# bigai-nlco/VideoTGB

Measured on AMD Instinct MI355X. Metric: clips/sec end-to-end VideoQA (96->8 frames), higher is better.
Workload: dtype bf16; 1 GPU; InstructBLIP-Vicuna-7B + TGB, T=96->8 of 32 frames, 224x224, greedy 16 new tokens (BASELINE.json configs[2]); inputs=resident in HBM when the timed region starts, global_batch=124, parallelism=clip-parallel x1 (no data-path collective), streams=1, weights=seeded N(0,0.02) random init

## Files before the change

include/vtgb.h:

```cpp
#ifndef VTGB_H
#define VTGB_H

#include <stddef.h>
#include <stdint.h>

#ifdef __cplusplus
extern "C" {
#endif

typedef struct ihipStream_t* vtgb_stream_t;

#define VTGB_VERSION 601

#define VTGB_OK 0
#define VTGB_EINVAL (-1)
#define VTGB_EWORKSPACE (-2)
#define VTGB_EHIP (-3)
#define VTGB_EUNSUPPORTED (-4)

#define VTGB_F32 0
#define VTGB_BF16 1
#define VTGB_BF16X3 2
#define VTGB_F16C8 3

// ... 40 lines not shown
} vtgb_preprocess_args;
int vtgb_preprocess_frames(const vtgb_preprocess_args* a, vtgb_stream_t stream);

typedef struct {
    const int64_t* input_ids;
    const int64_t* input_atts;
    const int64_t* output_ids;
    const int64_t* output_atts;
    int64_t* llm_ids;
    int64_t* llm_atts;
    int64_t* input_len;
    int64_t* labels;
    int64_t pad_id;
    int32_t B, Li, Lo, prefix_len;
} vtgb_concat_text_io_args;
int vtgb_concat_text_io(const vtgb_concat_text_io_args* a, vtgb_stream_t stream);

typedef struct {
    int32_t dtype, B, S, V;
    const void* logits;
    const int64_t* labels;
    float* lse;
    float* row_loss;
    float* loss;
    const float* grad_out;
    void* dlogits;
} vtgb_shifted_ce_args;
int vtgb_shifted_ce_forward(const vtgb_shifted_ce_args* a, vtgb_stream_t stream);
int vtgb_shifted_ce_backward(const vtgb_shifted_ce_args* a, vtgb_stream_t stream);

#define VTGB_VIT_NW_GLOBAL 6
#define VTGB_VIT_NW_LAYER 18
typedef struct {
    int32_t dtype, n_frames, image, patch, hidden, heads, mlp, layers;
    float eps;
    const float* pixel_values;
    const void* const* weights;
    float* out_f32;
    void* out_act;
    void* workspace;
    size_t workspace_bytes;
} vtgb_vit_args;
int32_t vtgb_vit_patch_kpad(int32_t dtype, int32_t patch);
size_t vtgb_vit_workspace_bytes(const vtgb_vit_args* a);
int vtgb_vit_forward(const vtgb_vit_args* a, vtgb_stream_t stream);

#define VTGB_QF_NW_GLOBAL 4
#define VTGB_QF_NW_LAYER 32
typedef struct {
    int32_t dtype, n_frames, n_query, n_text, hidden, heads, ffn, layers, cross_freq;
    int32_t enc_tokens, enc_hidden, has_text;
    float eps;
    const void* image_embeds;
    const float* query_tokens;
    const int64_t* text_ids;
    const int64_t* text_mask;
    const int64_t* image_mask;
    const void* const* weights;
    float* out_f32;
    void* workspace;
    size_t workspace_bytes;
} vtgb_qformer_args;
size_t vtgb_qformer_workspace_bytes(const vtgb_qformer_args* a);
int vtgb_qformer_forward(const vtgb_qformer_args* a, vtgb_stream_t stream);

#define VTGB_POOL_MEAN 0
#define VTGB_POOL_CONCAT 1
typedef struct {
    int32_t dtype, n_clips, n_query, hidden, out_dim, mode;
    const float* query_out;
    const int32_t* widths;
    const void* proj_w;
    const float* proj_b;
    float* out;
    void* workspace;
    size_t workspace_bytes;
} vtgb_pool_project_args;
size_t vtgb_pool_project_workspace_bytes(const vtgb_pool_project_args* a);
int vtgb_pool_project(const vtgb_pool_project_args* a, vtgb_stream_t stream);

#define VTGB_TGB_NW_GLOBAL 17
#define VTGB_TGB_NW_LAYER 26
#define VTGB_TGB_MODE_TEXT 0
#define VTGB_TGB_MODE_FUSION 1
#define VTGB_TGB_MODE_MULTIMODAL 2
typedef struct {
    int32_t dtype, B, L, n_text, hidden, heads, ffn, layers, fusion_layer, mode, image, patch;
    float eps;
    const float* of;
    const int64_t* of_mask;
    const int64_t* text_ids;
    const int64_t* text_mask;
    const void* const* weights;
    float* seq_out;
    float* logits;
    void* workspace;
    size_t workspace_bytes;
} vtgb_tgb_args;
size_t vtgb_tgb_workspace_bytes(const vtgb_tgb_args* a);
int vtgb_tgb_forward(const vtgb_tgb_args* a, vtgb_stream_t stream);

typedef struct {
    int32_t dtype, B, L, n_text, hidden, heads, ffn, layers, fusion_layer, mode, image, patch;
    float eps;
    const float* of;
    const int64_t* of_mask;
    const int64_t* text_ids;
    const int64_t* text_mask;
    const void* const* weights;
    float* trunk;
    void* trunk_act;
    float* seq_out;
    float* logits;
    void* workspace;
    size_t workspace_bytes;
} vtgb_tgb_split_args;
size_t vtgb_tgb_trunk_workspace_bytes(const vtgb_tgb_split_args* a);
int vtgb_tgb_trunk(const vtgb_tgb_split_args* a, vtgb_stream_t stream);
size_t vtgb_tgb_resume_workspace_bytes(const vtgb_tgb_split_args* a);
int vtgb_tgb_resume(const vtgb_tgb_split_args* a, vtgb_stream_t stream);

#define VTGB_EPI_STORE 0
#define VTGB_EPI_GELU 1
#define VTGB_EPI_RESID_F32 2
#define VTGB_EPI_STORE_F32 3
typedef struct {
    int32_t dtype, M, N, K, epilogue;
    const void* A;
    int64_t lda;
    const void* W;
    int64_t ldw;
    const float* bias;
    const float* resid;
    void* out;
    int64_t ldo;
} vtgb_gemm_args;
int vtgb_gemm(const vtgb_gemm_args* a, vtgb_stream_t stream);

typedef struct {
    int32_t dtype, batch, heads, head_dim, s_q, s_kv;
    const void* q;
    const void* k;
    const void* v;
    int64_t q_tok_stride, kv_tok_stride;
    int64_t q_batch_stride, kv_batch_stride;
    const float* key_mask;
    const float* rope_q;
    const float* rope_k;
    float scale;
    void* out;
    int64_t out_tok_stride, out_batch_stride;
    int32_t causal;
} vtgb_attention_args;
int vtgb_attention(const vtgb_attention_args* a, vtgb_stream_t stream);

typedef struct {
    int32_t batch, heads, kv_heads, head_dim, s_q, s_kv;
    const void* q;
    const void* k;
    const void* v;
    int64_t q_tok_stride, kv_tok_stride;
    int64_t q_batch_stride, kv_batch_stride;
    const float* key_mask;
    float scale;
    int32_t causal;
    void* out;
    int64_t out_tok_stride, out_batch_stride;
} vtgb_attention_tiled_args;
int vtgb_attention_tiled(const vtgb_attention_tiled_args* a, vtgb_stream_t stream);

typedef struct {
    int32_t batch, heads, kv_heads, head_dim, s_q;
    int32_t q0;
    int32_t tmax;
    float scale;
    const void* q;
    const void* kc;
    const void* vc;
    const float* ks;
    const float* vs;
    const uint8_t* key_valid;
    int64_t q_tok_stride, q_batch_stride;
    void* out;
    int64_t out_tok_stride, out_batch_stride;
} vtgb_attention_cached_args;
int vtgb_attention_cached(const vtgb_attention_cached_args* a, vtgb_stream_t stream);

typedef struct {
    int32_t dtype, M, D;
    float eps;
    const float* x;
    const float* gamma;
    const float* beta;
    float* out_f32;
    void* out_act;
} vtgb_layernorm_args;
int vtgb_layernorm(const vtgb_layernorm_args* a, vtgb_stream_t stream);

#define VTGB_RAFT_NW 30
typedef struct {
    int32_t dtype, n_pairs, H8, W8, iters;
    const float* net;
    const float* inp;
    const void* corr[4];
    const void* const* weights;
    float* flow_up;
    void* workspace;
    size_t workspace_bytes;
    int32_t corr_f16;
    const float* cnet_nhwc;
    const float* flow_init;
} vtgb_raft_update_args;
size_t vtgb_raft_update_workspace_bytes(const vtgb_raft_update_args* a);
int vtgb_raft_update(const vtgb_raft_update_args* a, vtgb_stream_t stream);

int vtgb_pair_pack(int32_t fmt, const float* x, void* out, int64_t M, int32_t C, int32_t ld_pair, vtgb_stream_t stream);
typedef struct {
    int32_t M, N, H, W, KH, KW, C1;
    const void* a;
    const void* a2;
    const void* weights;
    const int32_t* scale;
    const float* bias;
    int32_t act;
    int32_t out_fmt;
    void* out;
    int32_t ld_out;
} vtgb_pair_conv_args;
int vtgb_pair_conv(const vtgb_pair_conv_args* a, vtgb_stream_t stream);
typedef struct {
    vtgb_pair_conv_args conv;
    const void* resid;
    int32_t ld_resid;
    const float* tail_w;
    float* tail_out;
    float* out_f32;
    int32_t ld_f32;
} vtgb_pair_conv_ex_args;
int vtgb_pair_conv_ex(const vtgb_pair_conv_ex_args* a, vtgb_stream_t stream);

typedef struct {
    int32_t n_pairs, H8, W8;
    int32_t variant;
    const float* corr[4];
    const float* flow;
    const void* weights;
    const int32_t* scale;
    const float* bias;
    void* out;
    int32_t* occupancy;
} vtgb_raft_lookup_convc1_args;
int vtgb_raft_lookup_convc1(const vtgb_raft_lookup_convc1_args* a, vtgb_stream_t stream);

typedef struct {
    int32_t fmt;
    int32_t n_images, H8, W8;
    int32_t half;
    int32_t stage;
    const void* h;
    void* h_q;
    const void* x;
    void* rh;
    float* z;
    const float* start_zr;
    const float* start_q;
    const void* w_zr;
    const void* w_q;
    const int32_t* scale_zr;
    const int32_t* scale_q;
} vtgb_raft_gru_half_args;
int vtgb_raft_gru_half(const vtgb_raft_gru_half_args* a, vtgb_stream_t stream);

#define VTGB_CONV_OUT_F32 0
#define VTGB_CONV_OUT_PAIR_BF16 1
#define VTGB_CONV_OUT_PAIR_F16C8 2
#define VTGB_CONV_OUT_BF16 3
typedef struct {
    int32_t dtype;
    int32_t out_kind;
    int32_t site;
    int32_t n_images, H, W;
    int32_t KH, KW, stride;
    int32_t Hi, Wi;
    int32_t C1, C2;
    int32_t N;
    int32_t act;
    int32_t post_relu;
    float out_scale;
    const void* a;
    const void* a2;
    const void* weights;
    const float* bias;
    void* out;
    int64_t ld_out;
    float* moments;
    float* stats_part;
    int64_t stats_part_floats;
    const void* resid;
    int64_t ld_resid;
    const void* tail_w;
    float* tail_out;
} vtgb_conv_launch_args;
int vtgb_conv_launch(const vtgb_conv_launch_args* a, vtgb_stream_t stream);

typedef struct {
    int32_t dtype, n_pairs, H8, W8, dim;
    int32_t pairs_per_clip, frames_per_clip, first_off, second_off, n_images;
    float scale;
    const float* fmap;
    void* levels[4];
    void* workspace;
    size_t workspace_bytes;
} vtgb_raft_corr_args;
size_t vtgb_raft_corr_workspace_bytes(const vtgb_raft_corr_args* a);
int vtgb_raft_corr(const vtgb_raft_corr_args* a, vtgb_stream_t stream);

#define VTGB_RAFT_ENC_NW 40
typedef struct {
    int32_t dtype, n_images, H, W, norm;
    const float* images;
    const void* const* weights;
    float* out;
    void* workspace;
    size_t workspace_bytes;
} vtgb_raft_encoder_args;
size_t vtgb_raft_encoder_workspace_bytes(const vtgb_raft_encoder_args* a);
int vtgb_raft_encoder(const vtgb_raft_encoder_args* a, vtgb_stream_t stream);

int vtgb_llm_rmsnorm(int dtype, void* x, const void* delta, const void* w, void* h, int64_t rows, int32_t H, float eps,
                     vtgb_stream_t stream);
int vtgb_llm_rope_cache(int dtype, const void* qkv, void* q_out, void* kc, void* vc, const void* cos_t, const void* sin_t,
                        const int64_t* pos, int32_t B, int32_t nq, int32_t nkv, int32_t hd, int32_t tmax, vtgb_stream_t stream);
int vtgb_llm_rope_cache_prefill(int dtype, void* qkv, void* kc, void* vc, const void* cos_t, const void* sin_t, int32_t B, int32_t S, int32_t nq,
                                int32_t nkv, int32_t hd, int32_t tmax, vtgb_stream_t stream);
int vtgb_llm_decode_attention(int dtype, const void* q, const void* kc, const void* vc, void* out, const int64_t* pos, int32_t B,
                              int32_t nq, int32_t nkv, int32_t hd, int32_t tmax, float scale, vtgb_stream_t stream);
int vtgb_llm_silu_mul(int dtype, const void* gu, void* act, int64_t rows, int32_t I, vtgb_stream_t stream);

typedef struct {
    int32_t dtype, rows, heads, head_dim, rows_per_batch, n_keys, t_pad;
    float scale;
    const void* q;   int64_t q_row;
    const void* k;   const void* v;   int64_t kv_batch, kv_head, kv_tok;
    const void* bias; int64_t bias_pos, bias_head;
    const int64_t* pos;
    void* out;       int64_t o_row;
} vtgb_llm_attn_rows_args;
int vtgb_llm_attention_rows(const vtgb_llm_attn_rows_args* a, vtgb_stream_t stream);
int vtgb_llm_gated_act(int dtype, const void* gu, void* act, int64_t rows, int32_t I, int32_t kind, int32_t gated, vtgb_stream_t stream);

typedef struct {
    int32_t M, N, K, n_splits;
    const void* x; int64_t ldx;
    const void* w; int64_t ldw;
    void* out; int64_t ldo;
    int32_t out_dtype;
    int32_t w_tiled;
    void* workspace;
    size_t workspace_bytes;
    int32_t defer_reduce;
} vtgb_gemm_skinny_args;
int32_t vtgb_gemm_skinny_splits(const vtgb_gemm_skinny_args* a);
int vtgb_llm_rmsnorm_parts(int dtype, void* x, const float* part, int32_t n_splits, const void* w, void* h, int64_t rows, int32_t H, float eps,
                           vtgb_stream_t stream);
int vtgb_llm_rope_cache_parts(int dtype, const float* part, int32_t n_splits, void* q_out, void* kc, void* vc, const void* cos_t, const void* sin_t,
                              const int64_t* pos, int32_t B, int32_t nq, int32_t nkv, int32_t hd, int32_t tmax, vtgb_stream_t stream);

int vtgb_llm_rope_cache_pos(int dtype, const void* qkv, void* q_out, void* kc, void* vc, const void* cos_t, const void* sin_t,
                            const int64_t* pos, const int64_t* rope_off, int32_t B, int32_t nq, int32_t nkv, int32_t hd, int32_t tmax,
                            vtgb_stream_t stream);
int vtgb_llm_rope_cache_parts_pos(int dtype, const float* part, int32_t n_splits, void* q_out, void* kc, void* vc, const void* cos_t,
                                  const void* sin_t, const int64_t* pos, const int64_t* rope_off, int32_t B, int32_t nq, int32_t nkv, int32_t hd,
                                  int32_t tmax, vtgb_stream_t stream);
int vtgb_llm_rope_cache_prefill_pos(int dtype, void* qkv, void* kc, void* vc, const void* cos_t, const void* sin_t, const int64_t* pos_ids,
                                    int32_t B, int32_t S, int32_t nq, int32_t nkv, int32_t hd, int32_t tmax, vtgb_stream_t stream);
int vtgb_llm_decode_attention_masked(int dtype, const void* q, const void* kc, const void* vc, void* out, const int64_t* pos,
                                     const uint8_t* key_valid, int32_t B, int32_t nq, int32_t nkv, int32_t hd, int32_t tmax, float scale,
                                     vtgb_stream_t stream);
int vtgb_llm_attention_rows_masked(const vtgb_llm_attn_rows_args* a, const uint8_t* key_valid, int64_t key_valid_batch_stride,
                                   vtgb_stream_t stream);

int64_t vtgb_llm_decode_attention_split_workspace_bytes(int32_t B, int32_t nq, int32_t hd, int32_t tmax);
int vtgb_llm_decode_attention_split(int dtype, const void* q, const void* kc, const void* vc, void* out, const int64_t* pos,
                                    const uint8_t* key_valid , void* workspace, int32_t B, int32_t nq, int32_t nkv, int32_t hd,
                                    int32_t tmax, float scale, vtgb_stream_t stream);

typedef struct {
    int32_t dtype;
    int32_t B, nq, nkv, hd, tmax;
    int32_t n_splits;
    const void* qkv;
    const float* part;
    void* q_out;
    uint8_t* kc8; uint8_t* vc8;
    float* ks; float* vs;
    const void* cos_t; const void* sin_t;
    const int64_t* pos;
    const int64_t* rope_off;
} vtgb_llm_rope_cache_fp8_args;
int vtgb_llm_rope_cache_fp8(const vtgb_llm_rope_cache_fp8_args* a, vtgb_stream_t stream);
int vtgb_llm_rope_cache_prefill_fp8(int dtype, void* qkv, uint8_t* kc8, uint8_t* vc8, float* ks, float* vs, const void* cos_t, const void* sin_t,
                                    const int64_t* pos_ids , int32_t B, int32_t S, int32_t nq, int32_t nkv, int32_t hd, int32_t tmax,
                                    vtgb_stream_t stream);
int vtgb_llm_decode_attention_split_fp8(int dtype, const void* q, const uint8_t* kc8, const uint8_t* vc8, const float* ks, const float* vs, void* out,
                                        const int64_t* pos, const uint8_t* key_valid , void* workspace, int32_t B, int32_t nq,
                                        int32_t nkv, int32_t hd, int32_t tmax, float scale, vtgb_stream_t stream);

typedef struct {
    int32_t dtype;
    int32_t R, K, nq, nkv, hd, tmax_p, tmax_g;
    float scale;
    const void* q;
    const void* kp; const void* vp;
    const void* kg; const void* vg;
    const int32_t* src_row;
    void* out;
    const int64_t* n_prompt;
    const int64_t* pos;
    const uint8_t* key_valid;
    void* workspace;
} vtgb_llm_decode_attention_beam_args;
int vtgb_llm_decode_attention_beam(const vtgb_llm_decode_attention_beam_args* a, vtgb_stream_t stream);
typedef struct {
    int32_t dtype;
    int32_t R, K, nq, nkv, hd, tmax_p, tmax_g;
    float scale;
    const void* q;
    const uint8_t* kp8; const uint8_t* vp8;
    const float* kps; const float* vps;
    const uint8_t* kg8; const uint8_t* vg8;
    const float* kgs; const float* vgs;
    const int32_t* src_row;
    void* out;
    const int64_t* n_prompt;
    const int64_t* pos;
    const uint8_t* key_valid;
    void* workspace;
} vtgb_llm_decode_attention_beam_fp8_args;
int vtgb_llm_decode_attention_beam_fp8(const vtgb_llm_decode_attention_beam_fp8_args* a, vtgb_stream_t stream);
typedef struct {
    int32_t dtype;
    int32_t R, K, V, N;
    int32_t eos;
    int32_t min_new;
    float penalty;
    const void* logits;
    const int64_t* seq;
    const int64_t* step;
    const float* running;
    float* cand_score;
    int32_t* cand_idx;
    void* workspace;
    size_t workspace_bytes;
} vtgb_llm_beam_candidates_args;
int vtgb_llm_beam_candidates(const vtgb_llm_beam_candidates_args* a, vtgb_stream_t stream);

#define VTGB_LLM_ATTN_ROWS_BEAM_MAX_T 1920
int vtgb_llm_attention_rows_beam(const vtgb_llm_attn_rows_args* a, const int32_t* src_row, int64_t src_row_stride, int32_t cache_rows,
                                 vtgb_stream_t stream);

#define VTGB_LORA_MAX_SEGMENTS 4
#define VTGB_LORA_MAX_RANK 64
typedef struct {
    const float* A;
    const float* B;
    int32_t r, n, col0;
    float scaling;
} vtgb_llm_lora_seg;
typedef struct {
    int32_t dtype;
    int32_t K, n_cols, n_seg;
    int64_t rows, ldx, ldy;
    const void* x;
    void* y;
    vtgb_llm_lora_seg seg[VTGB_LORA_MAX_SEGMENTS];
} vtgb_llm_lora_args;
int vtgb_llm_lora(const vtgb_llm_lora_args* a, vtgb_stream_t stream);

size_t vtgb_pack_skinny_weight_bytes(int32_t N, int32_t K);
int vtgb_pack_skinny_weight(const void* w, int64_t ldw, int32_t N, int32_t K, void* dst, vtgb_stream_t stream);
size_t vtgb_gemm_skinny_workspace_bytes(const vtgb_gemm_skinny_args* a);
int vtgb_gemm_skinny(const vtgb_gemm_skinny_args* a, vtgb_stream_t stream);

size_t vtgb_pack_skinny_weight_fp8_bytes(int32_t N, int32_t K);
int vtgb_pack_skinny_weight_fp8(const void* w, int64_t ldw, int32_t N, int32_t K, void* dst, float* scale_out, vtgb_stream_t stream);
int vtgb_gemm_skinny_fp8(const vtgb_gemm_skinny_args* a, const float* w_scale, vtgb_stream_t stream);

int vtgb_gemm_skinny_bias(const vtgb_gemm_skinny_args* a, const float* w_scale , const float* bias ,
                          vtgb_stream_t stream);

size_t vtgb_pack_skinny_weight_mxfp4_bytes(int32_t N, int32_t K);
int vtgb_pack_skinny_weight_mxfp4(const void* w, int64_t ldw, int32_t N, int32_t K, void* dst, vtgb_stream_t stream);
int vtgb_gemm_skinny_mxfp4(const vtgb_gemm_skinny_args* a, const float* bias , vtgb_stream_t stream);

typedef struct {
    int32_t batch, heads, head_dim, s_q, s_kv;
    const float* q;
    const float* k;
    const float* v;
    int64_t q_tok, kv_tok, q_batch, kv_batch;
    const float* key_mask;
    const float* drop;
    float scale;
    float* out;
    int64_t o_tok, o_batch;
    float* lse;
    const float* dout;
    float* dq;
    float* dk;
    float* dv;
    float* delta;
} vtgb_attn_train_args;
int vtgb_attn_train_forward(const vtgb_attn_train_args* a, vtgb_stream_t stream);
int vtgb_attn_train_backward(const vtgb_attn_train_args* a, vtgb_stream_t stream);

typedef struct {
    int32_t compute, M, N, K;
    const void* a;
    int64_t lda;
    int32_t a_dtype, a_kmajor;
    const void* b;
    int64_t ldb;
    int32_t b_dtype, b_kmajor;
    const float* bias;
    float* out;
    int64_t ldo;
    void* workspace;
    size_t workspace_bytes;
} vtgb_gemm_train_args;
size_t vtgb_gemm_train_workspace_bytes(const vtgb_gemm_train_args* a);
int vtgb_gemm_train(const vtgb_gemm_train_args* a, vtgb_stream_t stream);
int32_t vtgb_col_sum_parts(int32_t M);
int vtgb_col_sum_f32(const float* x, int64_t ldx, int32_t M, int32_t N, float* out, float* partial, vtgb_stream_t stream);
typedef struct {
    int32_t rows, D;
    float eps;
    const float* x;
    const float* mask;
    const float* resid;
    const float* gamma;
    const float* beta;
    float* sum;
    float* y;
    float* mean;
    float* rstd;
    const float* dy;
    float* ds;
    float* dx;
    float* dgamma;
    float* dbeta;
    float* partial;
} vtgb_layernorm_train_args;
int32_t vtgb_layernorm_train_partials(int32_t rows);
int vtgb_layernorm_train_forward(const vtgb_layernorm_train_args* a, vtgb_stream_t stream);
int vtgb_layernorm_train_backward(const vtgb_layernorm_train_args* a, vtgb_stream_t stream);
int vtgb_gelu_forward(const float* x, float* y, int64_t n, vtgb_stream_t stream);
int vtgb_gelu_backward(const float* x, const float* dy, float* dx, int64_t n, vtgb_stream_t stream);

#define VTGB_COMM_ID_BYTES 128
typedef struct vtgb_comm vtgb_comm;
int vtgb_comm_unique_id(void* id_out );
int vtgb_comm_init(vtgb_comm** comm, const void* unique_id , int32_t rank, int32_t world);
int vtgb_comm_destroy(vtgb_comm* comm);
int vtgb_allreduce_f32(vtgb_comm* comm, float* buf, size_t count, int32_t average, vtgb_stream_t stream);

#define VTGB_PROF_GEMM 0
#define VTGB_PROF_ATTN 1
#define VTGB_PROF_CONV 2
void vtgb_prof_enable(int on);
void vtgb_prof_reset(void);
int vtgb_prof_summary(int kind, int64_t* launches, double* ms, double* flops);
int vtgb_prof_executed_flops(int kind, double* flops);

#ifdef __cplusplus
}
#endif
#endif
```

videotgb_amd/_lib.py:

```python
from __future__ import annotations

import ctypes as C
import os

import torch

HERE = os.path.dirname(os.path.abspath(__file__))
LIB_PATH = os.environ.get("VTGB_LIB") or os.path.join(HERE, "libvtgb.so")

F32, BF16 = 0, 1
BF16X3 = 2
F16C8 = 3
MAP_A, MAP_B = 0, 1
POOL_MEAN, POOL_CONCAT = 0, 1
TGB_MODE = {"text": 0, "vision": 0, "fusion": 1, "multi_modal": 2}
EPI_STORE, EPI_GELU, EPI_RESID_F32, EPI_STORE_F32 = 0, 1, 2, 3
VIT_NW_GLOBAL, VIT_NW_LAYER = 6, 18
QF_NW_GLOBAL, QF_NW_LAYER = 4, 32
TGB_NW_GLOBAL, TGB_NW_LAYER = 17, 26

EXPORTS = [
    "vtgb_version", "vtgb_last_error", "vtgb_pack_bf16", "vtgb_span_select", "vtgb_span_to_frames",
    "vtgb_gather_frames", "vtgb_vit_patch_kpad", "vtgb_vit_workspace_bytes", "vtgb_vit_forward",
    "vtgb_qformer_workspace_bytes", "vtgb_qformer_forward", "vtgb_pool_project_workspace_bytes",
    "vtgb_pool_project", "vtgb_tgb_workspace_bytes", "vtgb_tgb_forward", "vtgb_tgb_trunk_workspace_bytes", "vtgb_tgb_trunk",
    "vtgb_tgb_resume_workspace_bytes", "vtgb_tgb_resume", "vtgb_gemm", "vtgb_attention",
    "vtgb_layernorm", "vtgb_prof_enable", "vtgb_prof_reset", "vtgb_prof_summary", "vtgb_prof_executed_flops",
    "vtgb_llm_rmsnorm", "vtgb_llm_rope_cache", "vtgb_llm_rope_cache_prefill", "vtgb_llm_decode_attention", "vtgb_llm_silu_mul",
    "vtgb_llm_attention_rows", "vtgb_llm_gated_act", "vtgb_llm_rmsnorm_parts", "vtgb_llm_rope_cache_parts", "vtgb_gemm_skinny_splits",
    "vtgb_llm_rope_cache_pos", "vtgb_llm_rope_cache_parts_pos", "vtgb_llm_rope_cache_prefill_pos", "vtgb_llm_decode_attention_masked",
    "vtgb_llm_attention_rows_masked",
    "vtgb_gemm_skinny_workspace_bytes", "vtgb_gemm_skinny", "vtgb_pack_skinny_weight_bytes", "vtgb_pack_skinny_weight",
    "vtgb_pack_skinny_weight_fp8_bytes", "vtgb_pack_skinny_weight_fp8", "vtgb_gemm_skinny_fp8", "vtgb_gemm_skinny_bias",
    "vtgb_raft_update_workspace_bytes", "vtgb_raft_update", "vtgb_raft_encoder_workspace_bytes", "vtgb_raft_encoder",
    "vtgb_raft_corr_workspace_bytes", "vtgb_raft_corr", "vtgb_preprocess_frames", "vtgb_concat_text_io", "vtgb_shifted_ce_forward", "vtgb_shifted_ce_backward",
    "vtgb_comm_unique_id", "vtgb_comm_init", "vtgb_comm_destroy", "vtgb_allreduce_f32",
    "vtgb_attn_train_forward", "vtgb_attn_train_backward",
    "vtgb_gemm_train", "vtgb_gemm_train_workspace_bytes", "vtgb_col_sum_parts", "vtgb_col_sum_f32", "vtgb_layernorm_train_partials", "vtgb_layernorm_train_forward", "vtgb_layernorm_train_backward",
    "vtgb_gelu_forward", "vtgb_gelu_backward",
    "vtgb_pair_pack", "vtgb_pair_conv", "vtgb_pair_conv_ex", "vtgb_attention_tiled",
    "vtgb_llm_decode_attention_split_workspace_bytes", "vtgb_llm_decode_attention_split",
    "vtgb_llm_decode_attention_split_fp8", "vtgb_llm_rope_cache_fp8", "vtgb_llm_rope_cache_prefill_fp8",
    "vtgb_raft_lookup_convc1", "vtgb_raft_gru_half", "vtgb_llm_lora", "vtgb_conv_launch", "vtgb_attention_cached",
    "vtgb_llm_decode_attention_beam", "vtgb_llm_beam_candidates", "vtgb_llm_attention_rows_beam", "vtgb_llm_decode_attention_beam_fp8",
    "vtgb_pack_skinny_weight_mxfp4_bytes", "vtgb_pack_skinny_weight_mxfp4", "vtgb_gemm_skinny_mxfp4",
]
COMM_ID_BYTES = 128

i32, i64, f32, vp, sz = C.c_int32, C.c_int64, C.c_float, C.c_void_p, C.c_size_t


class AttnTrainArgs(C.Structure):
    _fields_ = [("batch", i32), ("heads", i32), ("head_dim", i32), ("s_q", i32), ("s_kv", i32), ("q", vp), ("k", vp), ("v", vp),
                ("q_tok", i64), ("kv_tok", i64), ("q_batch", i64), ("kv_batch", i64), ("key_mask", vp), ("drop", vp), ("scale", f32),
                ("out", vp), ("o_tok", i64), ("o_batch", i64), ("lse", vp), ("dout", vp), ("dq", vp), ("dk", vp), ("dv", vp), ("delta", vp)]


class GemmTrainArgs(C.Structure):
    _fields_ = [("compute", i32), ("M", i32), ("N", i32), ("K", i32), ("a", vp), ("lda", i64), ("a_dtype", i32), ("a_kmajor", i32),
                ("b", vp), ("ldb", i64), ("b_dtype", i32), ("b_kmajor", i32), ("bias", vp), ("out", vp), ("ldo", i64), ("workspace", vp), ("workspace_bytes", sz)]


class LayerNormTrainArgs(C.Structure):
    _fields_ = [("rows", i32), ("D", i32), ("eps", f32), ("x", vp), ("mask", vp), ("resid", vp), ("gamma", vp), ("beta", vp), ("sum", vp),
                ("y", vp), ("mean", vp), ("rstd", vp), ("dy", vp), ("ds", vp), ("dx", vp), ("dgamma", vp), ("dbeta", vp), ("partial", vp)]


class VtgbError(RuntimeError):
    pass


class SpanSelectArgs(C.Structure):
    _fields_ = [("logits", vp), ("noise", vp), ("idx", vp), ("B", i32), ("L", i32), ("draws", i32), ("tau", f32)]


class SpanToFramesArgs(C.Structure):
    _fields_ = [("sel", vp), ("V", vp), ("frame_idx", vp), ("B", i32), ("draws", i32), ("V_all", i32), ("N", i32),
                ("nframe", i32), ("variant", i32)]


class GatherFramesArgs(C.Structure):
    _fields_ = [("pixel_values", vp), ("frame_idx", vp), ("out", vp), ("B", i32), ("N", i32), ("nframe", i32),
                ("frame_elems", i64)]


class PreprocessArgs(C.Structure):
    _fields_ = [("raw", vp), ("frame_idx", vp), ("out", vp), ("T", i32), ("H0", i32), ("W0", i32), ("n_out", i32), ("size", i32),
                ("mean", f32 * 3), ("std", f32 * 3)]


class ConcatTextIoArgs(C.Structure):
    _fields_ = [("input_ids", vp), ("input_atts", vp), ("output_ids", vp), ("output_atts", vp), ("llm_ids", vp), ("llm_atts", vp),
                ("input_len", vp), ("labels", vp), ("pad_id", i64), ("B", i32), ("Li", i32), ("Lo", i32), ("prefix_len", i32)]


class ShiftedCeArgs(C.Structure):
    _fields_ = [("dtype", i32), ("B", i32), ("S", i32), ("V", i32), ("logits", vp), ("labels", vp), ("lse", vp), ("row_loss", vp),
                ("loss", vp), ("grad_out", vp), ("dlogits", vp)]


class VitArgs(C.Structure):
    _fields_ = [("dtype", i32), ("n_frames", i32), ("image", i32), ("patch", i32), ("hidden", i32), ("heads", i32),
                ("mlp", i32), ("layers", i32), ("eps", f32), ("pixel_values", vp), ("weights", C.POINTER(vp)),
                ("out_f32", vp), ("out_act", vp), ("workspace", vp), ("workspace_bytes", sz)]


class QFormerArgs(C.Structure):
    _fields_ = [("dtype", i32), ("n_frames", i32), ("n_query", i32), ("n_text", i32), ("hidden", i32), ("heads", i32),
                ("ffn", i32), ("layers", i32), ("cross_freq", i32), ("enc_tokens", i32), ("enc_hidden", i32),
                ("has_text", i32), ("eps", f32), ("image_embeds", vp), ("query_tokens", vp), ("text_ids", vp),
                ("text_mask", vp), ("image_mask", vp), ("weights", C.POINTER(vp)), ("out_f32", vp), ("workspace", vp),
                ("workspace_bytes", sz)]


class PoolProjectArgs(C.Structure):
    _fields_ = [("dtype", i32), ("n_clips", i32), ("n_query", i32), ("hidden", i32), ("out_dim", i32), ("mode", i32),
                ("query_out", vp), ("widths", C.POINTER(i32)), ("proj_w", vp), ("proj_b", vp), ("out", vp),
                ("workspace", vp), ("workspace_bytes", sz)]


class TgbArgs(C.Structure):
    _fields_ = [("dtype", i32), ("B", i32), ("L", i32), ("n_text", i32), ("hidden", i32), ("heads", i32), ("ffn", i32),
                ("layers", i32), ("fusion_layer", i32), ("mode", i32), ("image", i32), ("patch", i32), ("eps", f32),
                ("of", vp), ("of_mask", vp), ("text_ids", vp), ("text_mask", vp), ("weights", C.POINTER(vp)),
                ("seq_out", vp), ("logits", vp), ("workspace", vp), ("workspace_bytes", sz)]


class TgbSplitArgs(C.Structure):
    _fields_ = [("dtype", i32), ("B", i32), ("L", i32), ("n_text", i32), ("hidden", i32), ("heads", i32), ("ffn", i32),
                ("layers", i32), ("fusion_layer", i32), ("mode", i32), ("image", i32), ("patch", i32), ("eps", f32),
                ("of", vp), ("of_mask", vp), ("text_ids", vp), ("text_mask", vp), ("weights", C.POINTER(vp)),
                ("trunk", vp), ("trunk_act", vp), ("seq_out", vp), ("logits", vp), ("workspace", vp), ("workspace_bytes", sz)]


class RaftUpdateArgs(C.Structure):
    _fields_ = [("dtype", i32), ("n_pairs", i32), ("H8", i32), ("W8", i32), ("iters", i32), ("net", vp), ("inp", vp), ("corr", vp * 4),
                ("weights", C.POINTER(vp)), ("flow_up", vp), ("workspace", vp), ("workspace_bytes", sz), ("corr_f16", i32), ("cnet_nhwc", vp),
                ("flow_init", vp)]


class PairConvArgs(C.Structure):
    _fields_ = [("M", i32), ("N", i32), ("H", i32), ("W", i32), ("KH", i32), ("KW", i32), ("C1", i32), ("a", vp), ("a2", vp), ("weights", vp), ("scale", vp),
                ("bias", vp), ("act", i32), ("out_fmt", i32), ("out", vp), ("ld_out", i32)]


class PairConvExArgs(C.Structure):
    _fields_ = [("conv", PairConvArgs), ("resid", vp), ("ld_resid", i32), ("tail_w", vp), ("tail_out", vp), ("out_f32", vp), ("ld_f32", i32)]


class RaftLookupConvc1Args(C.Structure):
    _fields_ = [("n_pairs", i32), ("H8", i32), ("W8", i32), ("variant", i32), ("corr", vp * 4), ("flow", vp), ("weights", vp), ("scale", vp), ("bias", vp),
                ("out", vp), ("occupancy", C.POINTER(i32))]


class RaftGruHalfArgs(C.Structure):
    _fields_ = [("fmt", i32), ("n_images", i32), ("H8", i32), ("W8", i32), ("half", i32), ("stage", i32), ("h", vp), ("h_q", vp), ("x", vp), ("rh", vp), ("z", vp),
                ("start_zr", vp), ("start_q", vp), ("w_zr", vp), ("w_q", vp), ("scale_zr", vp), ("scale_q", vp)]


CONV_OUT_F32, CONV_OUT_PAIR_BF16, CONV_OUT_PAIR_F16C8, CONV_OUT_BF16 = 0, 1, 2, 3
CONV_SITE_ENCODER, CONV_SITE_UPDATE = 0, 1


class ConvLaunchArgs(C.Structure):
    _fields_ = [("dtype", i32), ("out_kind", i32), ("site", i32), ("n_images", i32), ("H", i32), ("W", i32), ("KH", i32), ("KW", i32), ("stride", i32),
                ("Hi", i32), ("Wi", i32), ("C1", i32), ("C2", i32), ("N", i32), ("act", i32), ("post_relu", i32), ("out_scale", f32), ("a", vp), ("a2", vp),
                ("weights", vp), ("bias", vp), ("out", vp), ("ld_out", i64), ("moments", vp), ("stats_part", vp), ("stats_part_floats", i64), ("resid", vp),
                ("ld_resid", i64), ("tail_w", vp), ("tail_out", vp)]


class RaftCorrArgs(C.Structure):
    _fields_ = [("dtype", i32), ("n_pairs", i32), ("H8", i32), ("W8", i32), ("dim", i32), ("pairs_per_clip", i32), ("frames_per_clip", i32),
                ("first_off", i32), ("second_off", i32), ("n_images", i32), ("scale", f32), ("fmap", vp), ("levels", vp * 4),
                ("workspace", vp), ("workspace_bytes", sz)]


class RaftEncoderArgs(C.Structure):
    _fields_ = [("dtype", i32), ("n_images", i32), ("H", i32), ("W", i32), ("norm", i32), ("images", vp), ("weights", C.POINTER(vp)), ("out", vp),
                ("workspace", vp), ("workspace_bytes", sz)]


class GemmSkinnyArgs(C.Structure):
    _fields_ = [("M", i32), ("N", i32), ("K", i32), ("n_splits", i32), ("x", vp), ("ldx", i64), ("w", vp), ("ldw", i64), ("out", vp), ("ldo", i64),
                ("out_dtype", i32), ("w_tiled", i32), ("workspace", vp), ("workspace_bytes", sz), ("defer_reduce", i32)]


class LlmLoraSeg(C.Structure):
    _fields_ = [("A", vp), ("B", vp), ("r", i32), ("n", i32), ("col0", i32), ("scaling", f32)]


LORA_MAX_SEGMENTS, LORA_MAX_RANK = 4, 64


class LlmLoraArgs(C.Structure):
    _fields_ = [("dtype", i32), ("K", i32), ("n_cols", i32), ("n_seg", i32), ("rows", i64), ("ldx", i64), ("ldy", i64), ("x", vp), ("y", vp),
                ("seg", LlmLoraSeg * LORA_MAX_SEGMENTS)]


class LlmRopeCacheFp8Args(C.Structure):
    _fields_ = [("dtype", i32), ("B", i32), ("nq", i32), ("nkv", i32), ("hd", i32), ("tmax", i32), ("n_splits", i32), ("qkv", vp), ("part", vp),
                ("q_out", vp), ("kc8", vp), ("vc8", vp), ("ks", vp), ("vs", vp), ("cos_t", vp), ("sin_t", vp), ("pos", vp), ("rope_off", vp)]


class LlmDecodeAttentionBeamArgs(C.Structure):
    _fields_ = [("dtype", i32), ("R", i32), ("K", i32), ("nq", i32), ("nkv", i32), ("hd", i32), ("tmax_p", i32), ("tmax_g", i32), ("scale", f32),
                ("q", vp), ("kp", vp), ("vp", vp), ("kg", vp), ("vg", vp), ("src_row", vp), ("out", vp), ("n_prompt", vp), ("pos", vp),
                ("key_valid", vp), ("workspace", vp)]


class LlmDecodeAttentionBeamFp8Args(C.Structure):
    _fields_ = [("dtype", i32), ("R", i32), ("K", i32), ("nq", i32), ("nkv", i32), ("hd", i32), ("tmax_p", i32), ("tmax_g", i32), ("scale", f32),
                ("q", vp), ("kp8", vp), ("vp8", vp), ("kps", vp), ("vps", vp), ("kg8", vp), ("vg8", vp), ("kgs", vp), ("vgs", vp), ("src_row", vp),
                ("out", vp), ("n_prompt", vp), ("pos", vp), ("key_valid", vp), ("workspace", vp)]


class LlmBeamCandidatesArgs(C.Structure):
    _fields_ = [("dtype", i32), ("R", i32), ("K", i32), ("V", i32), ("N", i32), ("eos", i32), ("min_new", i32), ("penalty", f32), ("logits", vp),
                ("seq", vp), ("step", vp), ("running", vp), ("cand_score", vp), ("cand_idx", vp), ("workspace", vp), ("workspace_bytes", sz)]


class GemmArgs(C.Structure):
    _fields_ = [("dtype", i32), ("M", i32), ("N", i32), ("K", i32), ("epilogue", i32), ("A", vp), ("lda", i64),
                ("W", vp), ("ldw", i64), ("bias", vp), ("resid", vp), ("out", vp), ("ldo", i64)]


class AttentionArgs(C.Structure):
    _fields_ = [("dtype", i32), ("batch", i32), ("heads", i32), ("head_dim", i32), ("s_q", i32), ("s_kv", i32),
                ("q", vp), ("k", vp), ("v", vp), ("q_tok_stride", i64), ("kv_tok_stride", i64), ("q_batch_stride", i64),
                ("kv_batch_stride", i64), ("key_mask", vp), ("rope_q", vp), ("rope_k", vp), ("scale", f32), ("out", vp),
                ("out_tok_stride", i64), ("out_batch_stride", i64), ("causal", i32)]


class AttentionTiledArgs(C.Structure):
    _fields_ = [("batch", i32), ("heads", i32), ("kv_heads", i32), ("head_dim", i32), ("s_q", i32), ("s_kv", i32),
                ("q", vp), ("k", vp), ("v", vp), ("q_tok_stride", i64), ("kv_tok_stride", i64), ("q_batch_stride", i64),
                ("kv_batch_stride", i64), ("key_mask", vp), ("scale", f32), ("causal", i32), ("out", vp),
                ("out_tok_stride", i64), ("out_batch_stride", i64)]


class AttentionCachedArgs(C.Structure):
    _fields_ = [("batch", i32), ("heads", i32), ("kv_heads", i32), ("head_dim", i32), ("s_q", i32), ("q0", i32), ("tmax", i32), ("scale", f32),
                ("q", vp), ("kc", vp), ("vc", vp), ("ks", vp), ("vs", vp), ("key_valid", vp), ("q_tok_stride", i64), ("q_batch_stride", i64),
                ("out", vp), ("out_tok_stride", i64), ("out_batch_stride", i64)]


class LlmAttnRowsArgs(C.Structure):
    _fields_ = [("dtype", i32), ("rows", i32), ("heads", i32), ("head_dim", i32), ("rows_per_batch", i32), ("n_keys", i32), ("t_pad", i32),
                ("scale", f32), ("q", vp), ("q_row", i64), ("k", vp), ("v", vp), ("kv_batch", i64), ("kv_head", i64), ("kv_tok", i64),
                ("bias", vp), ("bias_pos", i64), ("bias_head", i64), ("pos", vp), ("out", vp), ("o_row", i64)]


class LayerNormArgs(C.Structure):
    _fields_ = [("dtype", i32), ("M", i32), ("D", i32), ("eps", f32), ("x", vp), ("gamma", vp), ("beta", vp),
                ("out_f32", vp), ("out_act", vp)]


_lib = None


def lib() -> C.CDLL:
    global _lib
    if _lib is not None:
        return _lib
    if not os.path.exists(LIB_PATH):
        raise VtgbError(f"{LIB_PATH} is missing: build it with `python -m videotgb_amd.build` "
                        "(there is no CPU fallback for the hot path)")
    L = C.CDLL(LIB_PATH)
    L.vtgb_version.restype = C.c_int
    L.vtgb_last_error.restype = C.c_char_p
    L.vtgb_pack_bf16.argtypes = [vp, vp, i64, i64, i64, vp]
    L.vtgb_vit_patch_kpad.argtypes = [i32, i32]
    L.vtgb_vit_patch_kpad.restype = i32
    for name, st in (("span_select", SpanSelectArgs), ("span_to_frames", SpanToFramesArgs),
                     ("gather_frames", GatherFramesArgs), ("vit_forward", VitArgs), ("qformer_forward", QFormerArgs),
                     ("pool_project", PoolProjectArgs), ("tgb_forward", TgbArgs), ("gemm", GemmArgs),
                     ("attention", AttentionArgs), ("attention_tiled", AttentionTiledArgs), ("attention_cached", AttentionCachedArgs),
                     ("layernorm", LayerNormArgs)):
        fn = getattr(L, "vtgb_" + name)
        fn.argtypes = [C.POINTER(st), vp]
        fn.restype = C.c_int
    for name, st in (("vit", VitArgs), ("qformer", QFormerArgs), ("pool_project", PoolProjectArgs), ("tgb", TgbArgs),
                     ("tgb_trunk", TgbSplitArgs), ("tgb_resume", TgbSplitArgs)):
        fn = getattr(L, f"vtgb_{name}_workspace_bytes")
        fn.argtypes = [C.POINTER(st)]
        fn.restype = sz
    for name in ("tgb_trunk", "tgb_resume"):
        fn = getattr(L, "vtgb_" + name)
        fn.argtypes = [C.POINTER(TgbSplitArgs), vp]
        fn.restype = C.c_int
    L.vtgb_pair_pack.argtypes = [i32, vp, vp, i64, i32, i32, vp]
    L.vtgb_pair_pack.restype = C.c_int
    L.vtgb_pair_conv.argtypes = [C.POINTER(PairConvArgs), vp]
    L.vtgb_pair_conv.restype = C.c_int
    L.vtgb_pair_conv_ex.argtypes = [C.POINTER(PairConvExArgs), vp]
    L.vtgb_pair_conv_ex.restype = C.c_int
    L.vtgb_raft_lookup_convc1.argtypes = [C.POINTER(RaftLookupConvc1Args), vp]
    L.vtgb_raft_lookup_convc1.restype = C.c_int
    L.vtgb_raft_gru_half.argtypes = [C.POINTER(RaftGruHalfArgs), vp]
    L.vtgb_raft_gru_half.restype = C.c_int
    L.vtgb_conv_launch.argtypes = [C.POINTER(ConvLaunchArgs), vp]
    L.vtgb_conv_launch.restype = C.c_int
    L.vtgb_raft_update.argtypes = [C.POINTER(RaftUpdateArgs), vp]
    L.vtgb_raft_update.restype = C.c_int
    L.vtgb_raft_update_workspace_bytes.argtypes = [C.POINTER(RaftUpdateArgs)]
    L.vtgb_raft_update_workspace_bytes.restype = sz
    L.vtgb_raft_encoder.argtypes = [C.POINTER(RaftEncoderArgs), vp]
    L.vtgb_raft_encoder.restype = C.c_int
    L.vtgb_raft_encoder_workspace_bytes.argtypes = [C.POINTER(RaftEncoderArgs)]
    L.vtgb_raft_encoder_workspace_bytes.restype = sz
    L.vtgb_raft_corr.argtypes = [C.POINTER(RaftCorrArgs), vp]
    L.vtgb_raft_corr.restype = C.c_int
    L.vtgb_raft_corr_workspace_bytes.argtypes = [C.POINTER(RaftCorrArgs)]
    L.vtgb_raft_corr_workspace_bytes.restype = sz
    L.vtgb_llm_rmsnorm.argtypes = [C.c_int, vp, vp, vp, vp, i64, i32, f32, vp]
    L.vtgb_llm_rope_cache.argtypes = [C.c_int, vp, vp, vp, vp, vp, vp, vp, i32, i32, i32, i32, i32, vp]
    L.vtgb_llm_rope_cache_prefill.argtypes = [C.c_int, vp, vp, vp, vp, vp, i32, i32, i32, i32, i32, i32, vp]
    L.vtgb_llm_decode_attention.argtypes = [C.c_int, vp, vp, vp, vp, vp, i32, i32, i32, i32, i32, f32, vp]
    L.vtgb_llm_silu_mul.argtypes = [C.c_int, vp, vp, i64, i32, vp]
    L.vtgb_llm_attention_rows.argtypes = [C.POINTER(LlmAttnRowsArgs), vp]
    L.vtgb_llm_attention_rows.restype = C.c_int
    L.vtgb_llm_gated_act.argtypes = [C.c_int, vp, vp, i64, i32, i32, i32, vp]
    L.vtgb_llm_gated_act.restype = C.c_int
    L.vtgb_llm_rmsnorm_parts.argtypes = [C.c_int, vp, vp, i32, vp, vp, i64, i32, f32, vp]
    L.vtgb_llm_rmsnorm_parts.restype = C.c_int
    L.vtgb_llm_rope_cache_parts.argtypes = [C.c_int, vp, i32, vp, vp, vp, vp, vp, vp, i32, i32, i32, i32, i32, vp]
    L.vtgb_llm_rope_cache_parts.restype = C.c_int
    L.vtgb_llm_rope_cache_pos.argtypes = [C.c_int, vp, vp, vp, vp, vp, vp, vp, vp, i32, i32, i32, i32, i32, vp]
    L.vtgb_llm_rope_cache_parts_pos.argtypes = [C.c_int, vp, i32, vp, vp, vp, vp, vp, vp, vp, i32, i32, i32, i32, i32, vp]
    L.vtgb_llm_rope_cache_prefill_pos.argtypes = [C.c_int, vp, vp, vp, vp, vp, vp, i32, i32, i32, i32, i32, i32, vp]
    L.vtgb_llm_decode_attention_masked.argtypes = [C.c_int, vp, vp, vp, vp, vp, vp, i32, i32, i32, i32, i32, f32, vp]
    L.vtgb_llm_attention_rows_masked.argtypes = [C.POINTER(LlmAttnRowsArgs), vp, i64, vp]
    for fn in (L.vtgb_llm_rope_cache_pos, L.vtgb_llm_rope_cache_parts_pos, L.vtgb_llm_rope_cache_prefill_pos, L.vtgb_llm_decode_attention_masked,
               L.vtgb_llm_attention_rows_masked):
        fn.restype = C.c_int
    L.vtgb_llm_decode_attention_split_workspace_bytes.argtypes = [i32, i32, i32, i32]
    L.vtgb_llm_decode_attention_split_workspace_bytes.restype = i64
    L.vtgb_llm_decode_attention_split.argtypes = [C.c_int, vp, vp, vp, vp, vp, vp, vp, i32, i32, i32, i32, i32, f32, vp]
    L.vtgb_llm_decode_attention_split.restype = C.c_int
    L.vtgb_llm_decode_attention_split_fp8.argtypes = [C.c_int, vp, vp, vp, vp, vp, vp, vp, vp, vp, i32, i32, i32, i32, i32, f32, vp]
    L.vtgb_llm_decode_attention_split_fp8.restype = C.c_int
    L.vtgb_llm_rope_cache_fp8.argtypes = [C.POINTER(LlmRopeCacheFp8Args), vp]
    L.vtgb_llm_rope_cache_fp8.restype = C.c_int
    L.vtgb_llm_decode_attention_beam.argtypes = [C.POINTER(LlmDecodeAttentionBeamArgs), vp]
    L.vtgb_llm_decode_attention_beam.restype = C.c_int
    L.vtgb_llm_decode_attention_beam_fp8.argtypes = [C.POINTER(LlmDecodeAttentionBeamFp8Args), vp]
    L.vtgb_llm_decode_attention_beam_fp8.restype = C.c_int
    L.vtgb_llm_beam_candidates.argtypes = [C.POINTER(LlmBeamCandidatesArgs), vp]
    L.vtgb_llm_beam_candidates.restype = C.c_int
    L.vtgb_llm_attention_rows_beam.argtypes = [C.POINTER(LlmAttnRowsArgs), vp, i64, i32, vp]
    L.vtgb_llm_attention_rows_beam.restype = C.c_int
    L.vtgb_llm_lora.argtypes = [C.POINTER(LlmLoraArgs), vp]
    L.vtgb_llm_lora.restype = C.c_int
    L.vtgb_llm_rope_cache_prefill_fp8.argtypes = [C.c_int, vp, vp, vp, vp, vp, vp, vp, vp, i32, i32, i32, i32, i32, i32, vp]
    L.vtgb_llm_rope_cache_prefill_fp8.restype = C.c_int
    L.vtgb_gemm_skinny_splits.argtypes = [C.POINTER(GemmSkinnyArgs)]
    L.vtgb_gemm_skinny_splits.restype = i32
    L.vtgb_gemm_skinny.argtypes = [C.POINTER(GemmSkinnyArgs), vp]
    L.vtgb_gemm_skinny.restype = C.c_int
    L.vtgb_gemm_skinny_workspace_bytes.argtypes = [C.POINTER(GemmSkinnyArgs)]
    L.vtgb_gemm_skinny_workspace_bytes.restype = sz
    L.vtgb_pack_skinny_weight_bytes.argtypes = [i32, i32]
    L.vtgb_pack_skinny_weight_bytes.restype = sz
    L.vtgb_pack_skinny_weight.argtypes = [vp, i64, i32, i32, vp, vp]
    L.vtgb_pack_skinny_weight.restype = C.c_int
    L.vtgb_pack_skinny_weight_fp8_bytes.argtypes = [i32, i32]
    L.vtgb_pack_skinny_weight_fp8_bytes.restype = sz
    L.vtgb_pack_skinny_weight_fp8.argtypes = [vp, i64, i32, i32, vp, vp, vp]
    L.vtgb_pack_skinny_weight_fp8.restype = C.c_int
    L.vtgb_gemm_skinny_fp8.argtypes = [C.POINTER(GemmSkinnyArgs), vp, vp]
    L.vtgb_gemm_skinny_fp8.restype = C.c_int
    L.vtgb_gemm_skinny_bias.argtypes = [C.POINTER(GemmSkinnyArgs), vp, vp, vp]
    L.vtgb_gemm_skinny_bias.restype = C.c_int
    L.vtgb_pack_skinny_weight_mxfp4_bytes.argtypes = [i32, i32]
    L.vtgb_pack_skinny_weight_mxfp4_bytes.restype = sz
    L.vtgb_pack_skinny_weight_mxfp4.argtypes = [vp, i64, i32, i32, vp, vp]
    L.vtgb_pack_skinny_weight_mxfp4.restype = C.c_int
    L.vtgb_gemm_skinny_mxfp4.argtypes = [C.POINTER(GemmSkinnyArgs), vp, vp]
    L.vtgb_gemm_skinny_mxfp4.restype = C.c_int
    for fn in (L.vtgb_attn_train_forward, L.vtgb_attn_train_backward):
        fn.argtypes = [C.POINTER(AttnTrainArgs), vp]
        fn.restype = C.c_int
    L.vtgb_gemm_train.argtypes = [C.POINTER(GemmTrainArgs), vp]
    L.vtgb_gemm_train_workspace_bytes.argtypes = [C.POINTER(GemmTrainArgs)]
    L.vtgb_gemm_train_workspace_bytes.restype = sz
    L.vtgb_col_sum_f32.argtypes = [vp, i64, i32, i32, vp, vp, vp]
    L.vtgb_col_sum_parts.argtypes = [i32]
    L.vtgb_col_sum_parts.restype = i32
    L.vtgb_layernorm_train_partials.argtypes = [i32]
    L.vtgb_layernorm_train_partials.restype = i32
    for fn in (L.vtgb_layernorm_train_forward, L.vtgb_layernorm_train_backward):
        fn.argtypes = [C.POINTER(LayerNormTrainArgs), vp]
    L.vtgb_gelu_forward.argtypes = [vp, vp, i64, vp]
    L.vtgb_gelu_backward.argtypes = [vp, vp, vp, i64, vp]
    for fn in (L.vtgb_gemm_train, L.vtgb_col_sum_f32, L.vtgb_layernorm_train_forward, L.vtgb_layernorm_train_backward, L.vtgb_gelu_forward,
               L.vtgb_gelu_backward):
        fn.restype = C.c_int
    L.vtgb_comm_unique_id.argtypes = [vp]
    L.vtgb_comm_init.argtypes = [C.POINTER(vp), vp, i32, i32]
    L.vtgb_comm_destroy.argtypes = [vp]
    L.vtgb_allreduce_f32.argtypes = [vp, vp, sz, i32, vp]
    for fn in (L.vtgb_comm_unique_id, L.vtgb_comm_init, L.vtgb_comm_destroy, L.vtgb_allreduce_f32):
        fn.restype = C.c_int
    L.vtgb_prof_enable.argtypes = [C.c_int]
    L.vtgb_prof_enable.restype = None
    L.vtgb_prof_reset.restype = None
    L.vtgb_prof_summary.argtypes = [C.c_int, C.POINTER(i64), C.POINTER(C.c_double), C.POINTER(C.c_double)]
    L.vtgb_prof_summary.restype = C.c_int
    L.vtgb_prof_executed_flops.argtypes = [C.c_int, C.POINTER(C.c_double)]
    L.vtgb_prof_executed_flops.restype = C.c_int
    _lib = L
    return L


def prof_summary(kind: int):
    n, ms, fl = i64(0), C.c_double(0), C.c_double(0)
    check(lib().vtgb_prof_summary(kind, C.byref(n), C.byref(ms), C.byref(fl)))
    return n.value, ms.value, fl.value


def prof_executed_flops(kind: int) -> float:
    f = C.c_double(0)
    check(lib().vtgb_prof_executed_flops(kind, C.byref(f)))
    return f.value


_ERR = {-1: ValueError, -2: VtgbError, -3: VtgbError, -4: NotImplementedError}


def check(rc: int) -> None:
    if rc != 0:
        msg = lib().vtgb_last_error().decode("utf-8", "replace")
        raise _ERR.get(rc, VtgbError)(f"libvtgb: {msg} (code {rc})")
```

videotgb_amd/csrc/common.h:

```cpp
#pragma once
#include <hip/hip_runtime.h>
#include <stdint.h>
#include <stdio.h>

#include "vtgb.h"

typedef __bf16 bf16_t;
typedef __attribute__((ext_vector_type(8))) __bf16 bf16x8;
typedef __attribute__((ext_vector_type(4))) __bf16 bf16x4;
typedef __attribute__((ext_vector_type(4))) float f32x4;

#if defined(__HIPCC__)
__device__ __forceinline__ float bf16_round(float v) {
    unsigned u = __float_as_uint(v);
    if ((u & 0x7F800000u) != 0x7F800000u) u += 0x7FFFu + ((u >> 16) & 1u);
    return __uint_as_float(u & 0xFFFF0000u);
}
#endif

void vtgb_set_error(const char* fmt, ...);

#define VTGB_REQUIRE(cond, code, ...)  \
    do {                               \
        if (!(cond)) {                 \
            vtgb_set_error(__VA_ARGS__); \
            return (code);             \
        }                              \
    } while (0)

#define VTGB_HIP(expr)                                                              \
    do {                                                                            \
        hipError_t _e = (expr);                                                     \
        if (_e != hipSuccess) {                                                     \
            vtgb_set_error("%s failed: %s (%s:%d)", #expr, hipGetErrorString(_e), __FILE__, __LINE__); \
            return VTGB_EHIP;                                                       \
        }                                                                           \
    } while (0)

#define VTGB_TRY(expr)        \
    do {                      \
        int _r = (expr);      \
        if (_r != VTGB_OK) return _r; \
    } while (0)

struct RowMap {
    int32_t seg_rows;
    int64_t seg_stride;
    int64_t seg_off;
};
static inline RowMap rowmap_identity() { return RowMap{0, 0, 0}; }
static inline RowMap rowmap(int seg_rows, int64_t seg_stride, int64_t seg_off) {
    return RowMap{seg_rows, seg_stride, seg_off};
}
__host__ __device__ static inline int64_t map_row(const RowMap& m, int64_t r) {
    if (m.seg_rows == 0) return r;
    const int32_t r32 = (int32_t)r, seg = r32 / m.seg_rows;
    return (int64_t)seg * m.seg_stride + m.seg_off + (r32 - seg * m.seg_rows);
}

static inline size_t align_up(size_t x, size_t a) { return (x + a - 1) / a * a; }

#include <atomic>
struct DeviceOnce {
    std::atomic<uint64_t> done{0};
    static uint64_t bit() {
        int dev = 0;
        (void)hipGetDevice(&dev);
        return 1ull << (dev & 63);
    }
    bool need() const { return !(done.load(std::memory_order_acquire) & bit()); }
    void mark() { done.fetch_or(bit(), std::memory_order_acq_rel); }
};
#define VTGB_FUNC_LDS_ONCE(flag, kernel, bytes)                                                                              \
    do {                                                                                                                     \
        if ((flag).need()) {                                                                                                 \
            VTGB_HIP(hipFuncSetAttribute(reinterpret_cast<const void*>(kernel), hipFuncAttributeMaxDynamicSharedMemorySize, (int)(bytes))); \
            (flag).mark();                                                                                                   \
        }                                                                                                                    \
    } while (0)
static inline size_t dtype_size(int dtype) { return dtype == VTGB_BF16 ? 2 : 4; }

struct Workspace {
    char* base;
    size_t size, used;
    bool dry;
    Workspace(void* p, size_t n) : base((char*)p), size(n), used(0), dry(p == nullptr) {}
    void* take(size_t bytes) {
        size_t off = align_up(used, 256);
        used = off + bytes;
        return dry ? nullptr : (void*)(base + off);
    }
    bool ok() const { return dry || used <= size; }
};

struct GemmDesc {
    int dtype, M, N, K, epi;
    const void* A;
    int64_t lda;
    RowMap a_map;
    const void* W;
    int64_t ldw;
    const float* bias;
    const float* resid;
    int64_t ldr;
    RowMap r_map;
    void* out;
    int64_t ldo;
    RowMap o_map;
    int act;
    float out_scale;
    int conv_H, conv_W, conv_KH, conv_KW, conv_Cin, conv_split;
    int conv_stride, conv_Hi, conv_Wi;
    const void* A2;
    int64_t lda2;
    const void* zero_page;
    const void* aux;
    int64_t ldaux;
    void* out2;
    int64_t ldo2;
    float* col_stats;
    int stats_rows;
    int gate_from;
    const void* resid_bf16;
    int64_t ldrb;
    int post_relu;
    const void* init_bf16;
    int64_t ldinit;
    int frag_out, init_frag;
    uint32_t div_hw_mul, div_hw_sh, div_w_mul, div_w_sh;
    double algo_flops;
    const void* tail_w;
    float* tail_out;
    int64_t ldtail;
    int conv_wrap, conv_wrap2;
    int split_lo;
    void* ln_xb;
    int64_t ldxb;
    float* ln_part;
    const float* ln_stats;
    const float* ln_cs;
    const float* ln_c;
    int h8_run;
    const int* h8_scale;
    int h8_out_bf16;
    int split_f16c8;
};
int launch_conv_h8(const GemmDesc& d, hipStream_t s);
int launch_ln_fold_stats(const float* part, int nblk, int D, float eps, float* stats, int64_t M, hipStream_t s);
int launch_ln_fold_prepare(const float* x, int64_t ldx, int D, void* xb, float* part, int64_t M, hipStream_t s);
#define VTGB_EPI_GRU 4
#define VTGB_EPI_SPLIT 5
#define VTGB_EPI_X3ZR 6
#define VTGB_EPI_X3Q 7
int launch_gemm(const GemmDesc& d, hipStream_t s);
int launch_conv_gemm(const GemmDesc& d, hipStream_t s);

struct AttnDesc {
    int dtype, batch, heads, head_dim, s_q, s_kv;
    const void *q, *k, *v;
    int64_t q_tok, kv_tok, q_batch, kv_batch;
    const float* key_mask;
    const float* rope_q;
    const float* rope_k;
    float scale;
    void* out;
    int64_t o_tok, o_batch;
    int causal = 0;
};
int launch_attention(const AttnDesc& d, hipStream_t s);

bool stem7x7_supported(int H, int W);
int launch_stem7x7(const float* img, const void* w, const float* bias, float* out_f32, float* stats, float* stats_part, void* out_bf16, int n_img, int H, int W,
                   int relu, hipStream_t s);
size_t conv64_stats_part_floats(int n_img);
int launch_stats_finish_tiles(const float* part, float* stats, int n_img, int HW, int N, int64_t M, hipStream_t s);
int launch_stats_finish_parts(const float* part, float* stats, int n_img, int parts, int C, hipStream_t s);
int cu_count();

bool conv3x3_c64_supported(int H, int W);
int launch_conv3x3_c64(const void* in, const void* w, const float* bias, float* out_f32, float* stats, float* stats_part, void* out_bf16, const void* resid,
                       int n_img, int H, int W, int relu, int post_relu, hipStream_t s);

struct LnDesc {
    int dtype, M, D;
    float eps;
    const float* x;
    int64_t ldx;
    RowMap x_map;
    const float* gamma;
    const float* beta;
    float* out_f32;
    void* out_act;
    int64_t ldo;
    RowMap o_map;
};
int launch_layernorm(const LnDesc& d, hipStream_t s);

int launch_im2col(int dtype, const float* pix, void* out, int n_img, int ch, int image, int patch, int kpad, hipStream_t s);
int launch_vit_cls_rows(const float* cls, const float* pos, float* x, int n_frames, int tokens, int hidden, hipStream_t s);
int launch_cast_act(int dtype, const float* src, void* dst, int64_t n, hipStream_t s);
int launch_mask_to_additive(const int64_t* mask, float* out, int64_t n, float neg, hipStream_t s);
int launch_fill_f32(float* dst, float v, int64_t n, hipStream_t s);
int launch_qformer_embed(const float* query, const int64_t* ids, const float* wemb, const float* pemb, float* x,
                         int n_frames, int n_query, int n_text, int hidden, hipStream_t s);
int launch_tgb_text_embed(const int64_t* ids, const float* wemb, const float* temb, float* x, int64_t rows, int hidden,
                          hipStream_t s);
int launch_flow_reduce(const float* of, const float* fcw, float* red, int n_img, int image, int patch, hipStream_t s);
int launch_flow_assemble(const float* conv, const float* proj_b, const float* fcw, const float* fcb, const float* bos,
                         const float* eos, const float* pos, const int64_t* of_mask, float* x, int B, int L,
                         int hidden, int n_patches, hipStream_t s);
int launch_mean_pool_uniform(const float* q, float* out, int n_clips, int width, int64_t row_elems, hipStream_t s);
int launch_pack_bf16(const float* src, void* dst, int64_t rows, int64_t cols, int64_t cols_pad, hipStream_t s);
int launch_mrc_head(const float* x, const float* w, const float* b, float* logits, int B, int L, int hidden, hipStream_t s);

struct CorrPyr { const void* lvl[4]; int h[4], w[4]; };

struct ProfScope {
    int slot;
    hipStream_t s;
    ProfScope(int kind, double flops, hipStream_t stream, double executed_flops = -1.0);
    ~ProfScope();
};
```

videotgb_amd/csrc/conv64.hip:

```cpp
#include "common.h"

namespace {

constexpr int C64_R = 8, C64_RS = 128;
constexpr int C64_ROW_BYTES = C64_RS * 128;
constexpr int C64_LDS = C64_R * C64_ROW_BYTES + 8 * 32 * 2 * 4 + 64 * 4;
typedef __attribute__((address_space(3))) void* c64_lptr_t;

struct Conv64Params {
    const bf16_t* in;
    const bf16_t* w;
    const float* bias;
    float* out_f32;
    float* stats;
    float* stats_part;
    bf16_t* out_bf16;
    const bf16_t* resid;
    int n_img, H, W, relu, post_relu;
    int parts, rows_per_part;
};

template <int MODE>
__global__ __launch_bounds__(512) void conv3x3_c64_kernel(const Conv64Params p) {
#if defined(__HIP_DEVICE_COMPILE__)
    extern __shared__ __attribute__((aligned(16))) char ring[];
    float* const xch = reinterpret_cast<float*>(ring + C64_R * C64_ROW_BYTES);
    const int tid = threadIdx.x, lane = tid & 63, fr = lane & 15, fg = lane >> 4;
    const int wave = __builtin_amdgcn_readfirstlane(tid >> 6);
    const int wm = wave & 3, wn = wave >> 2;
    const int H = p.H, W = p.W;

    bf16x8 wf[9][2][2];
#pragma unroll
    for (int t = 0; t < 9; t++)
#pragma unroll
        for (int ks = 0; ks < 2; ks++)
#pragma unroll
            for (int i = 0; i < 2; i++)
                wf[t][ks][i] = *reinterpret_cast<const bf16x8*>(p.w + (wn * 32 + i * 16 + fr) * 576 + t * 64 + ks * 32 + fg * 8);
    float* const bias_s = xch + 8 * 32 * 2;
    if (tid < 64) bias_s[tid] = p.bias[tid];

    unsigned dma_off[2];
#pragma unroll
    for (int q = 0; q < 2; q++) {
        const int slot = (wave * 2 + q) * 8 + (lane >> 3), x = slot - 1, c = (lane & 7) ^ ((slot >> 1) & 7);
        dma_off[q] = (x >= 0 && x < W) ? (unsigned)(x * 64 + c * 8) * 2u : 0x80000000u;
    }
    unsigned x_off[3];
    int px[2];
#pragma unroll
    for (int j = 0; j < 2; j++) px[j] = wm * 32 + j * 16 + fr;
#pragma unroll
    for (int kx = 0; kx < 3; kx++) x_off[kx] = (unsigned)((px[0] + kx) * 128 + ((fg ^ (((px[0] + kx) >> 1) & 7)) << 4));

    typedef __attribute__((__vector_size__(4 * sizeof(unsigned)))) unsigned u32x4_t;
    typedef __attribute__((__vector_size__(2 * sizeof(unsigned)))) unsigned u32x2_t;
    constexpr unsigned OOB = 0x80000000u;
    constexpr int ES = MODE == 0 ? 4 : 2;
    unsigned o_off[2][2];
#pragma unroll
    for (int i = 0; i < 2; i++)
#pragma unroll
        for (int j = 0; j < 2; j++) o_off[i][j] = px[j] < W ? (unsigned)(px[j] * 64 + wn * 32 + i * 16 + fg * 4) * ES : OOB;

    const int n_units = p.n_img * p.parts;
    for (int unit = blockIdx.x; unit < n_units; unit += gridDim.x) {
        const int img = unit / p.parts, y0 = (unit - img * p.parts) * p.rows_per_part;
        if (y0 >= H) continue;
        const int y1 = y0 + p.rows_per_part < H ? y0 + p.rows_per_part : H;
        const bf16_t* const ibase = p.in + (int64_t)img * H * W * 64;
        const auto rsrc = __builtin_amdgcn_make_buffer_rsrc(const_cast<bf16_t*>(ibase), 0, H * W * 128, 0x00020000);
        const auto orsrc = __builtin_amdgcn_make_buffer_rsrc(MODE == 0 ? (void*)(p.out_f32 + (int64_t)img * H * W * 64) : (void*)(p.out_bf16 + (int64_t)img * H * W * 64), 0,
                                                             H * W * 64 * ES, 0x00020000);
        const auto rrsrc = __builtin_amdgcn_make_buffer_rsrc(const_cast<bf16_t*>(p.resid ? p.resid + (int64_t)img * H * W * 64 : ibase), 0, H * W * 128, 0x00020000);
#define C64_ISSUE(yy)                                                                                                          \
        {                                                                                                                      \
            const int so_ = ((yy) >= 0 && (yy) < H) ? (yy) * W * 128 : 0x7FFFFF00;        \
            char* const dst_ = ring + ((yy) & (C64_R - 1)) * C64_ROW_BYTES + (wave * 2) * 1024;                                \
            __builtin_amdgcn_raw_ptr_buffer_load_lds(rsrc, (c64_lptr_t)dst_, 16, dma_off[0], so_, 0, 0);                       \
            __builtin_amdgcn_raw_ptr_buffer_load_lds(rsrc, (c64_lptr_t)(dst_ + 1024), 16, dma_off[1], so_, 0, 0);              \
        }
        __builtin_amdgcn_s_waitcnt(0x0F70);
        __builtin_amdgcn_s_barrier();
        C64_ISSUE(y0 - 1)
        C64_ISSUE(y0)
        C64_ISSUE(y0 + 1)
        C64_ISSUE(y0 + 2)
        f32x4 s1[2] = {f32x4{0.f, 0.f, 0.f, 0.f}, f32x4{0.f, 0.f, 0.f, 0.f}}, s2[2] = {s1[0], s1[0]};
        for (int y = y0; y < y1; y += 2) {
            if (y == y0) __builtin_amdgcn_s_waitcnt(0x0F70);
            else __builtin_amdgcn_s_waitcnt(0x0F78);
            __builtin_amdgcn_s_barrier();
            bf16x4 rres[2][2][2];
            if constexpr (MODE == 1) {
                if (p.resid) {
#pragma unroll
                    for (int o = 0; o < 2; o++)
#pragma unroll
                        for (int i = 0; i < 2; i++)
#pragma unroll
                            for (int j = 0; j < 2; j++) {
                                const unsigned off = (y + o < y1 && o_off[i][j] != OOB) ? o_off[i][j] + (unsigned)((y + o) * W * 64 * 2) : OOB;
                                rres[o][i][j] = __builtin_bit_cast(bf16x4, __builtin_amdgcn_raw_buffer_load_b64(rrsrc, off, 0, 0));
                            }
                }
            }
            C64_ISSUE(y + 3)
            C64_ISSUE(y + 4)
            f32x4 acc[2][2][2];
#pragma unroll
            for (int o = 0; o < 2; o++)
#pragma unroll
                for (int i = 0; i < 2; i++)
#pragma unroll
                    for (int j = 0; j < 2; j++) acc[o][i][j] = f32x4{0.f, 0.f, 0.f, 0.f};
#pragma unroll
            for (int rr = 0; rr < 4; rr++) {
                const char* const rowp = ring + ((y + rr - 1) & (C64_R - 1)) * C64_ROW_BYTES;
#pragma unroll
                for (int kx = 0; kx < 3; kx++)
#pragma unroll
                    for (int ks = 0; ks < 2; ks++) {
                        const bf16x8 x0 = *reinterpret_cast<const bf16x8*>(rowp + (x_off[kx] ^ (ks * 64)));
                        const bf16x8 x1 = *reinterpret_cast<const bf16x8*>(rowp + (x_off[kx] ^ (ks * 64)) + 2048);
#pragma unroll
                        for (int o = 0; o < 2; o++) {
                            const int ky = rr - o;
                            if (ky < 0 || ky > 2) continue;
#pragma unroll
                            for (int i = 0; i < 2; i++) {
                                acc[o][i][0] = __builtin_amdgcn_mfma_f32_16x16x32_bf16(wf[ky * 3 + kx][ks][i], x0, acc[o][i][0], 0, 0, 0);
                                acc[o][i][1] = __builtin_amdgcn_mfma_f32_16x16x32_bf16(wf[ky * 3 + kx][ks][i], x1, acc[o][i][1], 0, 0, 0);
                            }
                        }
                    }
            }
            f32x4 b4[2];
#pragma unroll
            for (int i = 0; i < 2; i++) b4[i] = *reinterpret_cast<const f32x4*>(bias_s + wn * 32 + i * 16 + fg * 4);
#pragma unroll
            for (int o = 0; o < 2; o++) {
                const bool row_ok = y + o < y1;
#pragma unroll
                for (int i = 0; i < 2; i++)
#pragma unroll
                    for (int j = 0; j < 2; j++) {
                        const bool ok = row_ok && o_off[i][j] != OOB;
                        const unsigned off = ok ? o_off[i][j] + (unsigned)((y + o) * W * 64 * ES) : OOB;
                        f32x4 v = acc[o][i][j] + b4[i];
                        if constexpr (MODE == 0) {
                            __builtin_amdgcn_raw_buffer_store_b128(__builtin_bit_cast(u32x4_t, v), orsrc, off, 0, 0);
                            const f32x4 vz = {ok ? v[0] : 0.f, ok ? v[1] : 0.f, ok ? v[2] : 0.f, ok ? v[3] : 0.f};
                            s1[i] += vz;
                            s2[i] += vz * vz;
                        } else {
                            if (p.relu) v = f32x4{fmaxf(v[0], 0.f), fmaxf(v[1], 0.f), fmaxf(v[2], 0.f), fmaxf(v[3], 0.f)};
                            if (p.resid) {
                                const bf16x4 r = rres[o][i][j];
                                v += f32x4{(float)r[0], (float)r[1], (float)r[2], (float)r[3]};
                            }
                            if (p.post_relu) v = f32x4{fmaxf(v[0], 0.f), fmaxf(v[1], 0.f), fmaxf(v[2], 0.f), fmaxf(v[3], 0.f)};
                            const bf16x4 pk = {(bf16_t)v[0], (bf16_t)v[1], (bf16_t)v[2], (bf16_t)v[3]};
                            __builtin_amdgcn_raw_buffer_store_b64(__builtin_bit_cast(u32x2_t, pk), orsrc, off, 0, 0);
                        }
                    }
            }
        }
#undef C64_ISSUE
        if constexpr (MODE == 0) {
#pragma unroll
            for (int i = 0; i < 2; i++)
#pragma unroll
                for (int e = 0; e < 4; e++) {
                    float a_ = s1[i][e], b_ = s2[i][e];
#pragma unroll
                    for (int off = 1; off < 16; off <<= 1) { a_ += __shfl_xor(a_, off); b_ += __shfl_xor(b_, off); }
                    s1[i][e] = a_; s2[i][e] = b_;
                }
            __builtin_amdgcn_s_waitcnt(0xC07F);
            __builtin_amdgcn_s_barrier();
            if (fr == 0) {
#pragma unroll
                for (int i = 0; i < 2; i++)
#pragma unroll
                    for (int e = 0; e < 4; e++) {
                        xch[(wave * 32 + i * 16 + fg * 4 + e) * 2] = s1[i][e];
                        xch[(wave * 32 + i * 16 + fg * 4 + e) * 2 + 1] = s2[i][e];
                    }
            }
            __syncthreads();
            if (tid < 128) {
                const int ch = tid >> 1, which = tid & 1, wn_ = ch >> 5, c32 = ch & 31;
                float t = 0.f;
#pragma unroll
                for (int m_ = 0; m_ < 4; m_++) t += xch[((wn_ * 4 + m_) * 32 + c32) * 2 + which];
                if (p.parts == 1) p.stats[((int64_t)img * 64 + ch) * 2 + which] = t;
                else p.stats_part[((int64_t)unit * 64 + ch) * 2 + which] = t;
            }
        }
    }
#endif
}


constexpr int ST_R = 5;
struct StemParams {
    const float* img;
    const bf16_t* w;
    const float* bias;
    float* out_f32;
    float* stats;
    float* stats_part;
    bf16_t* out_bf16;
    int n_img, H, W, relu;
    int parts, rows_per_part;
};

template <int MODE>
__global__ __launch_bounds__(512) void stem7x7_kernel(const StemParams p) {
#if defined(__HIP_DEVICE_COMPILE__)
    extern __shared__ __attribute__((aligned(16))) char ring[];
    const int tid = threadIdx.x, lane = tid & 63, fr = lane & 15, fg = lane >> 4;
    const int wave = __builtin_amdgcn_readfirstlane(tid >> 6);
    const int wm = wave & 3, wn = wave >> 2;
    const int H = p.H, W = p.W, H2 = H >> 1, W2 = W >> 1;
    const int row_bytes = W2 * 256;
    float* const xch = reinterpret_cast<float*>(ring + ST_R * row_bytes);
    float* const bias_s = xch + 8 * 32 * 2;
    if (tid < 64) bias_s[tid] = p.bias[tid];
    for (int i = tid; i < ST_R * W2 * 4; i += 512) {
        const int pxl = i >> 2, X = pxl % W2, c = 6 + (i & 1) + ((i & 2) << 2);
        *reinterpret_cast<uint4*>(ring + pxl * 256 + ((c ^ (X & 15)) << 4)) = make_uint4(0, 0, 0, 0);
    }
    bf16x8 wf[16][2];
#pragma unroll
    for (int s_ = 0; s_ < 16; s_++)
#pragma unroll
        for (int i = 0; i < 2; i++) wf[s_][i] = *reinterpret_cast<const bf16x8*>(p.w + (wn * 32 + i * 16 + fr) * 512 + s_ * 32 + fg * 8);
    const bool builder = tid < W2 * 4;
    const int bX = tid >> 2, bdX = tid & 3, bcol = 2 * (bX + bdX - 2);
    const bool bcol_ok = builder && bcol >= 0 && bcol + 1 < W;
    const int bcol_c = bcol < 0 ? 0 : bcol + 1 < W ? bcol : W - 2;
    unsigned b_off[3];
#pragma unroll
    for (int q = 0; q < 3; q++) {
        const int off = bdX * 24 + q * 8;
        b_off[q] = (unsigned)(bX * 256 + (((off >> 4) ^ (bX & 15)) << 4) + (off & 8));
    }
    int px[2];
    unsigned x_off[2];
#pragma unroll
    for (int j = 0; j < 2; j++) {
        px[j] = wm * 32 + j * 16 + fr;
        const int pc = px[j] < W2 ? px[j] : 0;
        x_off[j] = (unsigned)(pc * 256 + ((fg ^ (pc & 15)) << 4));
    }
    typedef __attribute__((__vector_size__(4 * sizeof(unsigned)))) unsigned u32x4_t;
    typedef __attribute__((__vector_size__(2 * sizeof(unsigned)))) unsigned u32x2_t;
    constexpr unsigned OOB = 0x80000000u;
    constexpr int ES = MODE == 0 ? 4 : 2;
    unsigned o_off[2][2];
#pragma unroll
    for (int i = 0; i < 2; i++)
#pragma unroll
        for (int j = 0; j < 2; j++) o_off[i][j] = px[j] < W2 ? (unsigned)(px[j] * 64 + wn * 32 + i * 16 + fg * 4) * ES : OOB;

    const int n_units = p.n_img * p.parts;
    for (int unit = blockIdx.x; unit < n_units; unit += gridDim.x) {
        const int img = unit / p.parts, y0 = (unit - img * p.parts) * p.rows_per_part;
        if (y0 >= H2) continue;
        const int y1 = y0 + p.rows_per_part < H2 ? y0 + p.rows_per_part : H2;
        const float* const ibase = p.img + (int64_t)img * 3 * H * W;
        const auto orsrc = __builtin_amdgcn_make_buffer_rsrc(MODE == 0 ? (void*)(p.out_f32 + (int64_t)img * H2 * W2 * 64) : (void*)(p.out_bf16 + (int64_t)img * H2 * W2 * 64),
                                                             0, H2 * W2 * 64 * ES, 0x00020000);
        float2 ld[6];
#define ST_LOAD(Yp)       \
        {                                                                                                    \
            const int yc_ = (Yp) < 0 ? 0 : (Yp) >= H2 ? H2 - 1 : (Yp);                                       \
            _Pragma("unroll") for (int py = 0; py < 2; py++)                                                 \
                _Pragma("unroll") for (int c = 0; c < 3; c++)                                                \
                    ld[py * 3 + c] = *reinterpret_cast<const float2*>(ibase + ((int64_t)c * H + 2 * yc_ + py) * W + bcol_c); \
        }
#define ST_WRITE(Yp)                                                                                         \
        if (builder) {                                                                                       \
            const bool in_ = bcol_ok && (Yp) >= 0 && (Yp) < H2;                                              \
            bf16_t hi[12], lo[12];                                                                           \
            _Pragma("unroll") for (int py = 0; py < 2; py++)                                                 \
                _Pragma("unroll") for (int c = 0; c < 3; c++) {                                              \
                    const float d0 = in_ ? ld[py * 3 + c].x - 127.5f : 0.f, d1 = in_ ? ld[py * 3 + c].y - 127.5f : 0.f; \
                    const float h0_ = bf16_round(d0), h1_ = bf16_round(d1);                                  \
                    hi[py * 6 + c] = (bf16_t)h0_; lo[py * 6 + c] = (bf16_t)(d0 - h0_);                       \
                    hi[py * 6 + 3 + c] = (bf16_t)h1_; lo[py * 6 + 3 + c] = (bf16_t)(d1 - h1_);               \
                }                                                                                            \
            char* const rb_ = ring + ((((Yp) % ST_R) + ST_R) % ST_R) * row_bytes;                            \
            _Pragma("unroll") for (int q = 0; q < 3; q++) {                                                  \
                *reinterpret_cast<bf16x4*>(rb_ + b_off[q]) = bf16x4{hi[q * 4], hi[q * 4 + 1], hi[q * 4 + 2], hi[q * 4 + 3]}; \
                *reinterpret_cast<bf16x4*>(rb_ + (b_off[q] ^ 128)) = bf16x4{lo[q * 4], lo[q * 4 + 1], lo[q * 4 + 2], lo[q * 4 + 3]}; \
            }                                                                                                \
        }
        __syncthreads();
        for (int yy = y0 - 2; yy <= y0 + 1; yy++) {
            ST_LOAD(yy)
            ST_WRITE(yy)
        }
        f32x4 s1[2] = {f32x4{0.f, 0.f, 0.f, 0.f}, f32x4{0.f, 0.f, 0.f, 0.f}}, s2[2] = {s1[0], s1[0]};
        for (int y = y0; y < y1; y++) {
            __builtin_amdgcn_sched_barrier(0);
            __builtin_amdgcn_s_waitcnt(0xC07F);
            __builtin_amdgcn_s_barrier();
            __builtin_amdgcn_sched_barrier(0);
            ST_LOAD(y + 2)
            f32x4 acc[2][2];
#pragma unroll
            for (int i = 0; i < 2; i++)
#pragma unroll
                for (int j = 0; j < 2; j++) acc[i][j] = f32x4{0.f, 0.f, 0.f, 0.f};
#pragma unroll
            for (int tY = 0; tY < 4; tY++) {
                const char* const rowp = ring + ((y + tY - 2 + ST_R) % ST_R) * row_bytes;
#pragma unroll
                for (int hl = 0; hl < 2; hl++)
#pragma unroll
                    for (int half = 0; half < 2; half++) {
                        const int s_ = hl * 8 + tY * 2 + half;
                        const unsigned cx = (unsigned)((hl * 8 + half * 4) << 4);
                        const bf16x8 x0 = *reinterpret_cast<const bf16x8*>(rowp + (x_off[0] ^ cx));
                        const bf16x8 x1 = *reinterpret_cast<const bf16x8*>(rowp + (x_off[1] ^ cx));
#pragma unroll
                        for (int i = 0; i < 2; i++) {
                            acc[i][0] = __builtin_amdgcn_mfma_f32_16x16x32_bf16(wf[s_][i], x0, acc[i][0], 0, 0, 0);
                            acc[i][1] = __builtin_amdgcn_mfma_f32_16x16x32_bf16(wf[s_][i], x1, acc[i][1], 0, 0, 0);
                        }
                    }
            }
            f32x4 b4[2];
#pragma unroll
            for (int i = 0; i < 2; i++) b4[i] = *reinterpret_cast<const f32x4*>(bias_s + wn * 32 + i * 16 + fg * 4);
#pragma unroll
            for (int i = 0; i < 2; i++)
#pragma unroll
                for (int j = 0; j < 2; j++) {
                    const bool ok = o_off[i][j] != OOB;
                    const unsigned off = ok ? o_off[i][j] + (unsigned)(y * W2 * 64 * ES) : OOB;
                    f32x4 v = acc[i][j] + b4[i];
                    if constexpr (MODE == 0) {
                        __builtin_amdgcn_raw_buffer_store_b128(__builtin_bit_cast(u32x4_t, v), orsrc, off, 0, 0);
                        const f32x4 vz = {ok ? v[0] : 0.f, ok ? v[1] : 0.f, ok ? v[2] : 0.f, ok ? v[3] : 0.f};
                        s1[i] += vz;
                        s2[i] += vz * vz;
                    } else {
                        if (p.relu) v = f32x4{fmaxf(v[0], 0.f), fmaxf(v[1], 0.f), fmaxf(v[2], 0.f), fmaxf(v[3], 0.f)};
                        const bf16x4 pk = {(bf16_t)v[0], (bf16_t)v[1], (bf16_t)v[2], (bf16_t)v[3]};
                        __builtin_amdgcn_raw_buffer_store_b64(__builtin_bit_cast(u32x2_t, pk), orsrc, off, 0, 0);
                    }
                }
            ST_WRITE(y + 2)
        }
#undef ST_LOAD
#undef ST_WRITE
        if constexpr (MODE == 0) {
#pragma unroll
            for (int i = 0; i < 2; i++)
#pragma unroll
                for (int e = 0; e < 4; e++) {
                    float a_ = s1[i][e], b_ = s2[i][e];
#pragma unroll
                    for (int off = 1; off < 16; off <<= 1) { a_ += __shfl_xor(a_, off); b_ += __shfl_xor(b_, off); }
                    s1[i][e] = a_; s2[i][e] = b_;
                }
            __syncthreads();
            if (fr == 0) {
#pragma unroll
                for (int i = 0; i < 2; i++)
#pragma unroll
                    for (int e = 0; e < 4; e++) {
                        xch[(wave * 32 + i * 16 + fg * 4 + e) * 2] = s1[i][e];
                        xch[(wave * 32 + i * 16 + fg * 4 + e) * 2 + 1] = s2[i][e];
                    }
            }
            __syncthreads();
            if (tid < 128) {
                const int ch = tid >> 1, which = tid & 1, wn_ = ch >> 5, c32 = ch & 31;
                float t = 0.f;
#pragma unroll
                for (int m_ = 0; m_ < 4; m_++) t += xch[((wn_ * 4 + m_) * 32 + c32) * 2 + which];
                if (p.parts == 1) p.stats[((int64_t)img * 64 + ch) * 2 + which] = t;
                else p.stats_part[((int64_t)unit * 64 + ch) * 2 + which] = t;
            }
        }
    }
#endif
}

}

bool conv3x3_c64_supported(int H, int W) { return W >= 16 && W <= C64_RS - 2 && H >= 1; }

size_t conv64_stats_part_floats(int n_img) { return ((size_t)n_img + 4 * (size_t)cu_count()) * 2 * 64 * 2; }

int launch_conv3x3_c64(const void* in, const void* w, const float* bias, float* out_f32, float* stats, float* stats_part, void* out_bf16, const void* resid,
                       int n_img, int H, int W, int relu, int post_relu, hipStream_t s) {
    VTGB_REQUIRE(conv3x3_c64_supported(H, W), VTGB_EUNSUPPORTED, "conv3x3_c64: W=%d outside [16, %d]", W, C64_RS - 2);
    VTGB_REQUIRE((int64_t)H * W * 128 < 0x7FFFFF00ll, VTGB_EUNSUPPORTED, "conv3x3_c64: image too large");
    Conv64Params p;
    p.in = (const bf16_t*)in; p.w = (const bf16_t*)w; p.bias = bias; p.out_f32 = out_f32; p.stats = stats; p.stats_part = stats_part; p.out_bf16 = (bf16_t*)out_bf16;
    p.resid = (const bf16_t*)resid; p.n_img = n_img; p.H = H; p.W = W; p.relu = relu; p.post_relu = post_relu;
    int parts = 1;
    while ((int64_t)n_img * parts < 4 * cu_count() && H / (parts * 2) >= 8) parts *= 2;
    p.rows_per_part = 2 * ((H + 2 * parts - 1) / (2 * parts));
    p.parts = (H + p.rows_per_part - 1) / p.rows_per_part;
    const int64_t units = (int64_t)n_img * p.parts;
    const int grid = units < cu_count() ? (int)units : cu_count();
    if (out_f32 && p.parts > 1) VTGB_REQUIRE(stats_part && (size_t)units * 128 <= conv64_stats_part_floats(n_img), VTGB_EINVAL, "conv3x3_c64: partial-moment scratch missing");
    const double flops = 2.0 * n_img * H * W * 64.0 * 576.0;
    ProfScope prof(VTGB_PROF_CONV, flops, s, flops);
    static DeviceOnce a0, a1;
    if (out_f32) {
        VTGB_REQUIRE(stats, VTGB_EINVAL, "conv3x3_c64: fp32 output needs the moments buffer");
        VTGB_FUNC_LDS_ONCE(a0, conv3x3_c64_kernel<0>, C64_LDS);
        hipLaunchKernelGGL(conv3x3_c64_kernel<0>, dim3(grid), dim3(512), C64_LDS, s, p);
        if (p.parts > 1) VTGB_TRY(launch_stats_finish_parts(stats_part, stats, n_img, p.parts, 64, s));
    } else {
        VTGB_FUNC_LDS_ONCE(a1, conv3x3_c64_kernel<1>, C64_LDS);
        hipLaunchKernelGGL(conv3x3_c64_kernel<1>, dim3(grid), dim3(512), C64_LDS, s, p);
    }
    VTGB_HIP(hipGetLastError());
    return VTGB_OK;
}

bool stem7x7_supported(int H, int W) { return (H % 2) == 0 && (W % 2) == 0 && W / 2 >= 16 && W / 2 <= 112 && H / 2 >= 4; }

int launch_stem7x7(const float* img, const void* w, const float* bias, float* out_f32, float* stats, float* stats_part, void* out_bf16, int n_img, int H, int W,
                   int relu, hipStream_t s) {
    VTGB_REQUIRE(stem7x7_supported(H, W), VTGB_EUNSUPPORTED, "stem7x7: %d x %d unsupported", H, W);
    const int H2 = H / 2, W2 = W / 2;
    StemParams p;
    p.img = img; p.w = (const bf16_t*)w; p.bias = bias; p.out_f32 = out_f32; p.stats = stats; p.stats_part = stats_part; p.out_bf16 = (bf16_t*)out_bf16;
    p.n_img = n_img; p.H = H; p.W = W; p.relu = relu;
    int parts = 1;
    while ((int64_t)n_img * parts < 4 * cu_count() && H2 / (parts * 2) >= 14) parts *= 2;
    p.rows_per_part = (H2 + parts - 1) / parts;
    p.parts = (H2 + p.rows_per_part - 1) / p.rows_per_part;
    const int64_t units = (int64_t)n_img * p.parts;
    const int grid = units < cu_count() ? (int)units : cu_count();
    if (out_f32 && p.parts > 1) VTGB_REQUIRE(stats_part && (size_t)units * 128 <= conv64_stats_part_floats(n_img), VTGB_EINVAL, "stem7x7: partial-moment scratch missing");
    const int lds = ST_R * W2 * 256 + 8 * 32 * 2 * 4 + 64 * 4;
    const double flops = 2.0 * n_img * H2 * W2 * 64.0 * 147.0, exec = 2.0 * n_img * H2 * W2 * 64.0 * 512.0;
    ProfScope prof(VTGB_PROF_CONV, flops, s, exec);
    static DeviceOnce a0, a1;
    if (out_f32) {
        VTGB_REQUIRE(stats, VTGB_EINVAL, "stem7x7: fp32 output needs the moments buffer");
        VTGB_FUNC_LDS_ONCE(a0, stem7x7_kernel<0>, ST_R * 112 * 256 + 8 * 32 * 2 * 4 + 64 * 4);
        hipLaunchKernelGGL(stem7x7_kernel<0>, dim3(grid), dim3(512), lds, s, p);
        if (p.parts > 1) VTGB_TRY(launch_stats_finish_parts(stats_part, stats, n_img, p.parts, 64, s));
    } else {
        VTGB_FUNC_LDS_ONCE(a1, stem7x7_kernel<1>, ST_R * 112 * 256 + 8 * 32 * 2 * 4 + 64 * 4);
        hipLaunchKernelGGL(stem7x7_kernel<1>, dim3(grid), dim3(512), lds, s, p);
    }
    VTGB_HIP(hipGetLastError());
    return VTGB_OK;
}
```

videotgb_amd/csrc/pair_h8.h:

```cpp
#pragma once
#include "common.h"

typedef unsigned h8_u32x2 __attribute__((__vector_size__(2 * sizeof(unsigned))));
typedef _Float16 h8_f16x2 __attribute__((ext_vector_type(2)));
constexpr float H8_LO_SCALE = 2048.0f;
constexpr float H8_MAX = 57344.0f;

#if defined(__HIPCC__)
__device__ __forceinline__ void h8_split4(f32x4 v, h8_u32x2& hi, h8_u32x2& lo) {
#pragma unroll
    for (int e = 0; e < 4; e++) v[e] = __builtin_amdgcn_fmed3f(v[e], -H8_MAX, H8_MAX);
    const h8_f16x2 h01 = {(_Float16)v[0], (_Float16)v[1]}, h23 = {(_Float16)v[2], (_Float16)v[3]};
    const float r0 = (v[0] - (float)h01[0]) * H8_LO_SCALE, r1 = (v[1] - (float)h01[1]) * H8_LO_SCALE;
    const float r2 = (v[2] - (float)h23[0]) * H8_LO_SCALE, r3 = (v[3] - (float)h23[1]) * H8_LO_SCALE;
    hi[0] = __builtin_bit_cast(unsigned, h01);
    hi[1] = __builtin_bit_cast(unsigned, h23);
    int l0 = __builtin_amdgcn_cvt_pk_bf8_f32(r0, r1, 0, false);
    l0 = __builtin_amdgcn_cvt_pk_bf8_f32(r2, r3, l0, true);
    int l1 = __builtin_amdgcn_cvt_pk_bf8_f32(v[0], v[1], 0, false);
    l1 = __builtin_amdgcn_cvt_pk_bf8_f32(v[2], v[3], l1, true);
    lo[0] = (unsigned)l0;
    lo[1] = (unsigned)l1;
}
__device__ __forceinline__ f32x4 h8_join4(const h8_u32x2 hi, const h8_u32x2 lo) {
    typedef _Float16 h8_f16x4 __attribute__((ext_vector_type(4)));
    const f32x4 hv = __builtin_convertvector(__builtin_bit_cast(h8_f16x4, hi), f32x4);
    const int l0 = (int)lo[0];
    const f32x4 lv = {__builtin_amdgcn_cvt_f32_bf8(l0, 0), __builtin_amdgcn_cvt_f32_bf8(l0, 1), __builtin_amdgcn_cvt_f32_bf8(l0, 2), __builtin_amdgcn_cvt_f32_bf8(l0, 3)};
    return lv * (1.0f / H8_LO_SCALE) + hv;
}
__device__ __forceinline__ void h8_split1(float v, unsigned short& hi, unsigned char& lo_r, unsigned char& lo_v) {
    v = __builtin_amdgcn_fmed3f(v, -H8_MAX, H8_MAX);
    const _Float16 h = (_Float16)v;
    hi = __builtin_bit_cast(unsigned short, h);
    const int l = __builtin_amdgcn_cvt_pk_bf8_f32((v - (float)h) * H8_LO_SCALE, v, 0, false);
    lo_r = (unsigned char)(l & 255);
    lo_v = (unsigned char)((l >> 8) & 255);
}
__device__ __forceinline__ int h8_lo_off(int c) { return (c >> 2) * 8 + (c & 3); }
#endif
```

videotgb_amd/csrc/raft_enc.hip:

```cpp
#include <math.h>
#include <string.h>

#include "common.h"
#include "conv_descs.h"

template <typename T>
__global__ __launch_bounds__(256) void raft_stem_pack_kernel(const float* __restrict__ img, T* __restrict__ out, T* __restrict__ pad_page,
                                                             int64_t n_px, int H, int W) {
    constexpr bool PAIR = sizeof(T) == 2;
    constexpr int CP = PAIR ? 128 : 64;
    const int64_t i = (int64_t)blockIdx.x * blockDim.x + threadIdx.x;
    if (i < 64) pad_page[i] = (T)0.f;
    if (i >= n_px * 4) return;
    const int64_t px_i = i >> 2;
    const int dX = (int)(i & 3), W2 = W >> 1, H2 = H >> 1;
    const int X = (int)(px_i % W2), Y = (int)((px_i / W2) % H2);
    const int64_t n = px_i / ((int64_t)W2 * H2);
    T v[12], l[12];
#pragma unroll
    for (int py = 0; py < 2; py++)
#pragma unroll
        for (int pxx = 0; pxx < 2; pxx++) {
            const int col = 2 * (X + dX - 2) + pxx, row = 2 * Y + py;
            const bool ok = (unsigned)col < (unsigned)W;
#pragma unroll
            for (int c = 0; c < 3; c++) {
                const int e = py * 6 + pxx * 3 + c;
                const float raw = ok ? img[((n * 3 + c) * H + row) * W + col] : 0.f;
                if constexpr (PAIR) {
                    const float d = ok ? raw - 127.5f : 0.f;
                    const float hf = bf16_round(d);
                    v[e] = (T)hf;
                    l[e] = (T)(d - hf);
                } else {
                    v[e] = (T)(ok ? 2.0f * (raw / 255.0f) - 1.0f : 0.f);
                }
            }
        }
    typedef T T4 __attribute__((ext_vector_type(4)));
    T* o = out + px_i * CP + dX * 12;
#pragma unroll
    for (int q = 0; q < 3; q++) *reinterpret_cast<T4*>(o + q * 4) = T4{v[q * 4], v[q * 4 + 1], v[q * 4 + 2], v[q * 4 + 3]};
    if constexpr (PAIR) {
#pragma unroll
        for (int q = 0; q < 3; q++) *reinterpret_cast<T4*>(o + 64 + q * 4) = T4{l[q * 4], l[q * 4 + 1], l[q * 4 + 2], l[q * 4 + 3]};
    }
    if (dX == 3) {
        const T4 z = {(T)0.f, (T)0.f, (T)0.f, (T)0.f};
#pragma unroll
        for (int q = 0; q < 4; q++) {
            *reinterpret_cast<T4*>(out + px_i * CP + 48 + q * 4) = z;
            if constexpr (PAIR) *reinterpret_cast<T4*>(out + px_i * CP + 112 + q * 4) = z;
        }
    }
}

__global__ __launch_bounds__(256) void inorm_stats_kernel(const float* __restrict__ x, float* __restrict__ part, int HW, int C, int ldx) {
    __shared__ float s1[256], s2[256];
    const int n = blockIdx.x, tid = threadIdx.x;
    const int c4 = C >> 2, cq = tid % c4, lane_p = tid / c4, np = 256 / c4;
    const int per = (HW + gridDim.y - 1) / gridDim.y, p0 = blockIdx.y * per, p1 = min(HW, p0 + per);
    float a[4] = {0.f, 0.f, 0.f, 0.f}, q[4] = {0.f, 0.f, 0.f, 0.f};
    if (lane_p < np) {
        const float* base = x + (int64_t)n * HW * ldx + cq * 4;
        for (int p = p0 + lane_p; p < p1; p += np) {
            const float4 v = *reinterpret_cast<const float4*>(base + (int64_t)p * ldx);
            a[0] += v.x; a[1] += v.y; a[2] += v.z; a[3] += v.w;
            q[0] = fmaf(v.x, v.x, q[0]); q[1] = fmaf(v.y, v.y, q[1]); q[2] = fmaf(v.z, v.z, q[2]); q[3] = fmaf(v.w, v.w, q[3]);
        }
    }
    for (int e = 0; e < 4; e++) {
        __syncthreads();
        s1[tid] = a[e]; s2[tid] = q[e];
        __syncthreads();
        if (tid < c4) {
            float sa = 0.f, sq = 0.f;
            for (int l = 0; l < np; l++) { sa += s1[l * c4 + tid]; sq += s2[l * c4 + tid]; }
            float* st = part + (((int64_t)n * gridDim.y + blockIdx.y) * C + tid * 4 + e) * 2;
            st[0] = sa;
            st[1] = sq;
        }
    }
}

__global__ void stats_finish_parts_kernel(const float* __restrict__ part, float* __restrict__ stats, int64_t total, int parts, int C2) {
    const int64_t i = (int64_t)blockIdx.x * blockDim.x + threadIdx.x;
    if (i >= total) return;
    const int64_t img = i / C2;
    const int cw = (int)(i - img * C2);
    float t = 0.f;
    for (int pt = 0; pt < parts; pt++) t += part[(img * parts + pt) * C2 + cw];
    stats[i] = t;
}
int launch_stats_finish_parts(const float* part, float* stats, int n_img, int parts, int C, hipStream_t s) {
    const int64_t total = (int64_t)n_img * C * 2;
    hipLaunchKernelGGL(stats_finish_parts_kernel, dim3((unsigned)((total + 255) / 256)), dim3(256), 0, s, part, stats, total, parts, C * 2);
    VTGB_HIP(hipGetLastError());
    return VTGB_OK;
}
__global__ void stats_finish_tiles_kernel(const float* __restrict__ part, float* __restrict__ stats, int n_img, int HW, int N, int64_t M) {
    const int64_t i = (int64_t)blockIdx.x * blockDim.x + threadIdx.x;
    if (i >= (int64_t)n_img * N) return;
    const int img = (int)(i / N), n = (int)(i - (int64_t)img * N);
    const int64_t r0 = (int64_t)img * HW, r1 = r0 + HW;
    const int t0 = (int)(r0 >> 8), t1 = (int)((r1 - 1) >> 8);
    float sa = 0.f, sq = 0.f;
    for (int t = t0; t <= t1; t++) {
        const float4 v = *reinterpret_cast<const float4*>(part + ((int64_t)t * N + n) * 4);
        const int img_a = (int)(((int64_t)t << 8) / HW);
        if (img_a == img) { sa += v.x; sq += v.y; }
        else { sa += v.z; sq += v.w; }
    }
    stats[i * 2] = sa;
    stats[i * 2 + 1] = sq;
}
int launch_stats_finish_tiles(const float* part, float* stats, int n_img, int HW, int N, int64_t M, hipStream_t s) {
    VTGB_REQUIRE(HW >= 256, VTGB_EINVAL, "stats_finish_tiles: images of >= 256 rows");
    const int64_t total = (int64_t)n_img * N;
    hipLaunchKernelGGL(stats_finish_tiles_kernel, dim3((unsigned)((total + 255) / 256)), dim3(256), 0, s, part, stats, n_img, HW, N, M);
    VTGB_HIP(hipGetLastError());
    return VTGB_OK;
}

constexpr int NA_PASS = 4;
template <typename T>
__global__ __launch_bounds__(256) void norm_apply_kernel(const float* __restrict__ x, const float* __restrict__ stats, const T* __restrict__ resid,
                                                         T* __restrict__ out, int HW, int C, int Cpad, int ldx, int relu_inner, int relu_outer) {
    typedef T T4 __attribute__((ext_vector_type(4)));
    const int sh = Cpad == 64 ? 4 : 5, cp4 = 1 << sh, ppb = 256 >> sh;
    const int tid = threadIdx.x, c = (tid & (cp4 - 1)) * 4, pl = tid >> sh;
    const int n = blockIdx.y, p0 = blockIdx.x * (NA_PASS * ppb) + pl;
    const int64_t m0 = (int64_t)n * HW;
    float mean[4] = {0.f, 0.f, 0.f, 0.f}, rstd[4] = {1.f, 1.f, 1.f, 1.f};
    const bool live = c < C;
    if (live && stats) {
        const float inv = 1.0f / (float)HW;
        const float4 s01 = *reinterpret_cast<const float4*>(stats + ((int64_t)n * C + c) * 2);
        const float4 s23 = *reinterpret_cast<const float4*>(stats + ((int64_t)n * C + c) * 2 + 4);
        const float sm[4] = {s01.x, s01.z, s23.x, s23.z}, sq[4] = {s01.y, s01.w, s23.y, s23.w};
#pragma unroll
        for (int e = 0; e < 4; e++) {
            mean[e] = sm[e] * inv;
            rstd[e] = rsqrtf(fmaxf(sq[e] * inv - mean[e] * mean[e], 0.f) + 1e-5f);
        }
    }
    float4 xv[NA_PASS];
    T4 rv[NA_PASS];
#pragma unroll
    for (int j = 0; j < NA_PASS; j++) {
        const int px = p0 + j * ppb;
        const int pc = px < HW ? px : HW - 1;
        xv[j] = live ? *reinterpret_cast<const float4*>(x + (m0 + pc) * ldx + c) : make_float4(0.f, 0.f, 0.f, 0.f);
        if (resid && live) rv[j] = *reinterpret_cast<const T4*>(resid + (m0 + pc) * Cpad + c);
    }
#pragma unroll
    for (int j = 0; j < NA_PASS; j++) {
        const int px = p0 + j * ppb;
        float v[4] = {xv[j].x, xv[j].y, xv[j].z, xv[j].w};
        if (live) {
            if (stats) {
#pragma unroll
                for (int e = 0; e < 4; e++) v[e] = (v[e] - mean[e]) * rstd[e];
            }
            if (relu_inner) {
#pragma unroll
                for (int e = 0; e < 4; e++) v[e] = fmaxf(v[e], 0.f);
            }
            if (resid) {
#pragma unroll
                for (int e = 0; e < 4; e++) v[e] += (float)rv[j][e];
            }
            if (relu_outer) {
#pragma unroll
                for (int e = 0; e < 4; e++) v[e] = fmaxf(v[e], 0.f);
            }
        }
        const T4 o = {(T)v[0], (T)v[1], (T)v[2], (T)v[3]};
        if (px < HW) *reinterpret_cast<T4*>(out + (m0 + px) * Cpad + c) = o;
    }
}

int launch_x3_pair_pass(const float* x, int64_t ldx, const float* stats, int HW, const void* resid, int64_t ldr, int r_lo, void* out, int64_t ldo, int o_lo,
                        int C, int Cpad, int relu_in, int relu_out, int64_t M, hipStream_t s, int h8 = 0, int resid_h8 = 0);

static int enc_impl(const vtgb_raft_encoder_args* a, Workspace& ws, hipStream_t s) {
    VTGB_REQUIRE(a, VTGB_EINVAL, "raft_encoder: NULL args");
    VTGB_REQUIRE(a->n_images > 0 && a->H >= 64 && a->W >= 64 && (a->H % 8) == 0 && (a->W % 8) == 0 && (a->norm == 0 || a->norm == 1), VTGB_EINVAL,
                 "raft_encoder: bad dims n=%d H=%d W=%d", a->n_images, a->H, a->W);
    VTGB_REQUIRE(a->dtype == VTGB_BF16 || a->dtype == VTGB_F32 || a->dtype == VTGB_BF16X3 || a->dtype == VTGB_F16C8, VTGB_EINVAL, "raft_encoder: bad dtype %d", a->dtype);
    const bool h8l1 = a->dtype == VTGB_F16C8;
    const int n = a->n_images, dt = h8l1 ? VTGB_BF16X3 : a->dtype;
    const bool x3 = dt == VTGB_BF16X3;
    const size_t es = x3 ? 4 : dtype_size(dt);
    const int H2 = a->H / 2, W2 = a->W / 2, H4 = a->H / 4, W4 = a->W / 4, H8 = a->H / 8, W8 = a->W / 8;
    const int64_t M2 = (int64_t)n * H2 * W2, M4 = (int64_t)n * H4 * W4, M8 = (int64_t)n * H8 * W8;
    VTGB_REQUIRE(M2 < (1ll << 31), VTGB_EUNSUPPORTED, "raft_encoder: too many pixels per call (chunk the images)");
    float* cf = (float*)ws.take(M2 * 64 * 4);
    float* cf2 = (float*)ws.take(M4 * 128 * 4);
    void* act0 = ws.take(M2 * 64 * es);
    char* act12 = (char*)ws.take(2 * M2 * 64 * es);
    void* act1 = act12;
    void* act2 = act12 + (ws.dry ? 0 : M2 * 64 * es);
    float* stats = (float*)ws.take((int64_t)n * 128 * 2 * 4);
    float* stats2 = (float*)ws.take((int64_t)n * 128 * 2 * 4);
    size_t part_floats = (size_t)(M2 / 256 + 2) * 128 * 4;
    if (conv64_stats_part_floats(n) > part_floats) part_floats = conv64_stats_part_floats(n);
    if ((size_t)n * 16 * 128 * 2 > part_floats) part_floats = (size_t)n * 16 * 128 * 2;
    float* spart = (float*)ws.take(part_floats * 4);
    void* zero = ws.take(256);
    void* pad_page = ws.take(256);
    if (ws.dry) return VTGB_OK;
    VTGB_REQUIRE(ws.ok(), VTGB_EWORKSPACE, "raft_encoder: workspace %zu < %zu bytes", ws.size, ws.used);
    VTGB_REQUIRE(a->images && a->weights && a->out, VTGB_EINVAL, "raft_encoder: NULL operand");
    const void* const* w = a->weights;
    auto F = [](const void* p) { return (const float*)p; };
    const bool inorm = a->norm == 0;
    VTGB_HIP(hipMemsetAsync(zero, 0, 256, s));

    auto norm = [&](const float* x, int64_t M, int HW, int C, int Cpad, int ldx, const void* resid, void* out, int relu_in, int relu_out,
                    float* st, bool fused, int out_h8 = 0, int resid_h8 = 0) -> int {
        if (inorm && !fused) {
            const int splits = HW >= 4096 ? 16 : HW >= 1024 ? 4 : 1;
            hipLaunchKernelGGL(inorm_stats_kernel, dim3(n, splits), dim3(256), 0, s, x, spart, HW, C, ldx);
            VTGB_TRY(launch_stats_finish_parts(spart, st, n, splits, C, s));
        }
        if (x3)
            return launch_x3_pair_pass(x, ldx, inorm ? st : nullptr, HW, resid, 2 * Cpad, Cpad, out, 2 * Cpad, Cpad, C, Cpad, relu_in, relu_out, M, s, out_h8, resid_h8);
        VTGB_REQUIRE(Cpad == 64 || Cpad == 128, VTGB_EUNSUPPORTED, "raft_encoder: normalisation pass over %d padded channels", Cpad);
        const int ppb = 256 / (Cpad / 4);
        VTGB_REQUIRE(M / HW <= 65535, VTGB_EUNSUPPORTED, "raft_encoder: %lld images per call exceed the normalisation pass's grid (chunk the images)", (long long)(M / HW));
        const dim3 grid((unsigned)((HW + NA_PASS * ppb - 1) / (NA_PASS * ppb)), (unsigned)(M / HW));
        if (dt == VTGB_BF16)
            hipLaunchKernelGGL(norm_apply_kernel<bf16_t>, grid, dim3(256), 0, s, x, inorm ? st : nullptr, (const bf16_t*)resid, (bf16_t*)out, HW, C, Cpad, ldx,
                               relu_in, relu_out);
        else
            hipLaunchKernelGGL(norm_apply_kernel<float>, grid, dim3(256), 0, s, x, inorm ? st : nullptr, (const float*)resid, (float*)out, HW, C, Cpad, ldx,
                               relu_in, relu_out);
        VTGB_HIP(hipGetLastError());
        return VTGB_OK;
    };
    auto stats_for = [&](float* st, int HW, int C) -> float* {
        if (!inorm || HW < 256 || dt == VTGB_F32) return nullptr;
        return spart;
    };
    auto conv_stats = [&](const GemmDesc& d, float* st) -> int {
        VTGB_TRY(launch_conv_gemm(d, s));
        if (d.col_stats) VTGB_TRY(launch_stats_finish_tiles(d.col_stats, st, n, d.stats_rows, d.N, d.M, s));
        return VTGB_OK;
    };
#ifdef VTGB_DEBUG_HOOKS
    static const bool stem_on = !(getenv("VTGB_STEM64") && getenv("VTGB_STEM64")[0] == '0');
#else
    constexpr bool stem_on = true;
#endif
    if (stem_on && dt == VTGB_BF16 && stem7x7_supported(a->H, a->W)) {
        if (inorm) {
            VTGB_TRY(launch_stem7x7(a->images, w[0], F(w[1]), cf, stats, spart, nullptr, n, a->H, a->W, 0, s));
            VTGB_TRY(norm(cf, M2, H2 * W2, 64, 64, 64, nullptr, act0, 1, 0, stats, true));
        } else {
            VTGB_TRY(launch_stem7x7(a->images, w[0], F(w[1]), nullptr, nullptr, nullptr, act0, n, a->H, a->W, 1, s));
        }
    } else {
        if (dt != VTGB_F32)
            hipLaunchKernelGGL(raft_stem_pack_kernel<bf16_t>, dim3((unsigned)((M2 * 4 + 255) / 256)), dim3(256), 0, s, a->images, (bf16_t*)act1, (bf16_t*)pad_page, M2,
                               a->H, a->W);
        else
            hipLaunchKernelGGL(raft_stem_pack_kernel<float>, dim3((unsigned)((M2 * 4 + 255) / 256)), dim3(256), 0, s, a->images, (float*)act1, (float*)pad_page, M2,
                               a->H, a->W);
        {
            float* sf = stats_for(stats, H2 * W2, 64);
            const int cp = dt == VTGB_BF16 ? 128 : 64;
            GemmDesc d = enc_stem_conv(dt, (int)M2, 64, H2, W2, cp, act1, w[0], F(w[1]), cf, 64, pad_page, sf);
            if (x3) d.algo_flops = 2.0 * (double)M2 * 64 * 147;
            if (!inorm && !x3) { d.epi = VTGB_EPI_STORE; d.act = 1; d.out = act0; }
            VTGB_TRY(conv_stats(d, stats));
            if (inorm || x3) VTGB_TRY(norm(cf, M2, H2 * W2, 64, 64, 64, nullptr, act0, 1, 0, stats, sf != nullptr, h8l1));
        }
    }
    struct Stage { int C, Cpad, stride, Ho, Wo; };
    const Stage st[6] = {{64, 64, 1, H2, W2}, {64, 64, 1, H2, W2}, {96, 128, 2, H4, W4}, {96, 128, 1, H4, W4}, {128, 128, 2, H8, W8}, {128, 128, 1, H8, W8}};
    void* x = act0;
    void* t1 = act1;
    void* t2 = act2;
    int Cin_pad = 64, Hi = H2, Wi = W2;
    auto conv_bn = [&](int64_t Mo, const Stage& g, int K, int Cin, int stride, int Hi_, int Wi_, const void* A, const void* Wt, const float* bias,
                       int relu, const void* resid, int post_relu, void* out) -> int {
        GemmDesc d = enc_conv(dt, (int)Mo, g.Cpad, g.Ho, g.Wo, K, Cin, stride, Hi_, Wi_, A, Wt, bias, nullptr, g.Cpad, zero, nullptr);
        d.epi = VTGB_EPI_STORE; d.act = relu; d.out = out;
        d.resid_bf16 = resid; d.ldrb = g.Cpad; d.post_relu = post_relu;
        return launch_conv_gemm(d, s);
    };
    for (int b = 0; b < 6; b++) {
        const Stage& g = st[b];
        const void* const* bw = w + 2 + 6 * b;
        const int64_t Mo = (int64_t)n * g.Ho * g.Wo;
        const int HWo = g.Ho * g.Wo;
        if (g.stride != 1) VTGB_REQUIRE(bw[4] && bw[5], VTGB_EINVAL, "raft_encoder: block %d lacks its downsample weights", b);
        void* outb;
#ifdef VTGB_DEBUG_HOOKS
        static const bool c64_on = !(getenv("VTGB_CONV64") && getenv("VTGB_CONV64")[0] == '0');
#else
        constexpr bool c64_on = true;
#endif
        const bool c64 = c64_on && dt == VTGB_BF16 && g.C == 64 && g.Cpad == 64 && Cin_pad == 64 && g.stride == 1 && conv3x3_c64_supported(g.Ho, g.Wo);
        if (c64 && !inorm) {
            VTGB_TRY(launch_conv3x3_c64(x, bw[0], F(bw[1]), nullptr, nullptr, nullptr, t1, nullptr, n, g.Ho, g.Wo, 1, 0, s));
            outb = t2;
            VTGB_TRY(launch_conv3x3_c64(t1, bw[2], F(bw[3]), nullptr, nullptr, nullptr, outb, x, n, g.Ho, g.Wo, 1, 1, s));
        } else if (c64) {
            VTGB_TRY(launch_conv3x3_c64(x, bw[0], F(bw[1]), cf, stats, spart, nullptr, nullptr, n, g.Ho, g.Wo, 0, 0, s));
            VTGB_TRY(norm(cf, Mo, HWo, g.C, g.Cpad, g.Cpad, nullptr, t1, 1, 0, stats, true));
            VTGB_TRY(launch_conv3x3_c64(t1, bw[2], F(bw[3]), cf, stats, spart, nullptr, nullptr, n, g.Ho, g.Wo, 0, 0, s));
            outb = t1;
            VTGB_TRY(norm(cf, Mo, HWo, g.C, g.Cpad, g.Cpad, x, outb, 1, 1, stats, true));
        } else if (!inorm && !x3) {
            VTGB_TRY(conv_bn(Mo, g, 3, Cin_pad, g.stride, Hi, Wi, x, bw[0], F(bw[1]), 1, nullptr, 0, t1));
            const void* res = x;
            outb = t2;
            if (g.stride != 1) {
                VTGB_TRY(conv_bn(Mo, g, 1, Cin_pad, g.stride, Hi, Wi, x, bw[4], F(bw[5]), 0, nullptr, 0, t2));
                res = t2;
                outb = x;
            }
            VTGB_TRY(conv_bn(Mo, g, 3, g.Cpad, 1, g.Ho, g.Wo, t1, bw[2], F(bw[3]), 1, res, 1, outb));
        } else if (h8l1) {
            VTGB_REQUIRE(w[40], VTGB_EINVAL, "raft_encoder: weights[40] (the f16c8 convolutions' scale bytes) is NULL at VTGB_F16C8");
            const int C2 = 2 * g.Cpad;
            const bool s2 = g.stride != 1;
            auto conv_h8 = [&](const void* A, const void* Wt, const float* bias, float* col_stats, int si) -> int {
                GemmDesc d;
                memset(&d, 0, sizeof(d));
                d.dtype = VTGB_BF16; d.M = (int)Mo; d.N = g.C; d.K = 9 * C2; d.epi = VTGB_EPI_STORE_F32;
                d.A = A; d.lda = C2; d.W = Wt; d.ldw = d.K; d.bias = bias; d.out = cf; d.ldo = g.Cpad;
                d.conv_H = g.Ho; d.conv_W = g.Wo; d.conv_KH = 3; d.conv_KW = 3; d.conv_Cin = C2; d.conv_split = C2; d.zero_page = zero;
                d.col_stats = col_stats; d.stats_rows = HWo;
                d.h8_run = 9 * (g.Cpad / 64); d.h8_scale = (const int*)w[40] + si;
                d.algo_flops = 2.0 * Mo * (double)g.C * (9 * g.C);
                VTGB_TRY(launch_conv_h8(d, s));
                if (col_stats) VTGB_TRY(launch_stats_finish_tiles(col_stats, stats, n, HWo, g.C, Mo, s));
                return VTGB_OK;
            };
            auto conv_pair = [&](const void* A, const void* Wt, const float* bias, int si, const void* resid, void* out, int out_bf16) -> int {
                GemmDesc d;
                memset(&d, 0, sizeof(d));
                d.dtype = VTGB_BF16; d.M = (int)Mo; d.N = g.Cpad; d.K = 9 * C2; d.epi = VTGB_EPI_SPLIT; d.act = 1;
                d.A = A; d.lda = C2; d.W = Wt; d.ldw = d.K; d.bias = bias; d.out = out; d.ldo = C2; d.split_lo = g.Cpad;
                d.conv_H = g.Ho; d.conv_W = g.Wo; d.conv_KH = 3; d.conv_KW = 3; d.conv_Cin = C2; d.conv_split = C2; d.zero_page = zero;
                d.resid_bf16 = resid; d.ldrb = C2; d.post_relu = resid != nullptr;
                d.h8_run = 9 * (g.Cpad / 64); d.h8_scale = (const int*)w[40] + si; d.h8_out_bf16 = out_bf16;
                d.algo_flops = 2.0 * Mo * (double)g.C * (9 * g.C);
                return launch_conv_h8(d, s);
            };
            const int out_h8 = (b & 1) == 0;
            if (!inorm) {
                auto split_conv = [&](int K, const void* Wt, const float* bias, int relu, void* out) -> int {
                    GemmDesc d = enc_conv(dt, (int)Mo, g.Cpad, g.Ho, g.Wo, K, Cin_pad, g.stride, Hi, Wi, x, Wt, bias, nullptr, C2, zero, nullptr);
                    d.epi = VTGB_EPI_SPLIT; d.act = relu; d.out = out; d.split_lo = g.Cpad; d.split_f16c8 = 1;
                    d.algo_flops = 2.0 * Mo * (double)g.C * (K * K * Cin_pad);
                    return launch_conv_gemm(d, s);
                };
                if (s2) VTGB_TRY(split_conv(3, bw[0], F(bw[1]), 1, t1));
                else VTGB_TRY(conv_pair(x, bw[0], F(bw[1]), 2 * b, nullptr, t1, 0));
                const void* res = x;
                outb = t2;
                if (s2) {
                    VTGB_TRY(split_conv(1, bw[4], F(bw[5]), 0, t2));
                    res = t2;
                    outb = x;
                }
                VTGB_TRY(conv_pair(t1, bw[2], F(bw[3]), 2 * b + 1, res, outb, !out_h8));
            } else {
                float* sf = stats_for(stats, HWo, g.C);
                if (s2) VTGB_TRY(conv_stats(enc_conv(dt, (int)Mo, g.C, g.Ho, g.Wo, 3, Cin_pad, g.stride, Hi, Wi, x, bw[0], F(bw[1]), cf, g.Cpad, zero, sf), stats));
                else VTGB_TRY(conv_h8(x, bw[0], F(bw[1]), sf, 2 * b));
                VTGB_TRY(norm(cf, Mo, HWo, g.C, g.Cpad, g.Cpad, nullptr, t1, 1, 0, stats, sf != nullptr, 1));
                sf = stats_for(stats, HWo, g.C);
                VTGB_TRY(conv_h8(t1, bw[2], F(bw[3]), sf, 2 * b + 1));
                const void* res = x;
                if (s2) {
                    float* sf2 = stats_for(stats2, HWo, g.C);
                    VTGB_TRY(conv_stats(enc_conv(dt, (int)Mo, g.C, g.Ho, g.Wo, 1, Cin_pad, g.stride, Hi, Wi, x, bw[4], F(bw[5]), cf2, g.Cpad, zero, sf2), stats2));
                    VTGB_TRY(norm(cf2, Mo, HWo, g.C, g.Cpad, g.Cpad, nullptr, t2, 0, 0, stats2, sf2 != nullptr));
                    res = t2;
                }
                outb = t1;
                VTGB_TRY(norm(cf, Mo, HWo, g.C, g.Cpad, g.Cpad, res, outb, 1, 1, stats, sf != nullptr, out_h8, !s2));
            }
        } else if (x3 && !inorm && g.Cpad == 128) {
            auto split_conv = [&](int K, int Cin, int stride, int Hi_, int Wi_, const void* A, const void* Wt, const float* bias, int relu, void* out) -> int {
                GemmDesc d = enc_conv(dt, (int)Mo, g.Cpad, g.Ho, g.Wo, K, Cin, stride, Hi_, Wi_, A, Wt, bias, nullptr, 2 * g.Cpad, zero, nullptr);
                d.epi = VTGB_EPI_SPLIT; d.act = relu; d.out = out; d.split_lo = g.Cpad;
                d.algo_flops = 2.0 * Mo * (double)g.C * (K * K * Cin);
                return launch_conv_gemm(d, s);
            };
            VTGB_TRY(split_conv(3, Cin_pad, g.stride, Hi, Wi, x, bw[0], F(bw[1]), 1, t1));
            VTGB_TRY(launch_conv_gemm(enc_conv(dt, (int)Mo, g.C, g.Ho, g.Wo, 3, g.Cpad, 1, g.Ho, g.Wo, t1, bw[2], F(bw[3]), cf, g.Cpad, zero, nullptr), s));
            const void* res = x;
            outb = t1;
            if (g.stride != 1) {
                VTGB_TRY(split_conv(1, Cin_pad, g.stride, Hi, Wi, x, bw[4], F(bw[5]), 0, t2));
                res = t2;
            }
            VTGB_TRY(norm(cf, Mo, HWo, g.C, g.Cpad, g.Cpad, res, outb, 1, 1, stats, false));
        } else {
            float* sf = stats_for(stats, HWo, g.C);
            VTGB_TRY(conv_stats(enc_conv(dt, (int)Mo, g.C, g.Ho, g.Wo, 3, Cin_pad, g.stride, Hi, Wi, x, bw[0], F(bw[1]), cf, g.Cpad, zero, sf), stats));
            VTGB_TRY(norm(cf, Mo, HWo, g.C, g.Cpad, g.Cpad, nullptr, t1, 1, 0, stats, sf != nullptr));
            sf = stats_for(stats, HWo, g.C);
            VTGB_TRY(conv_stats(enc_conv(dt, (int)Mo, g.C, g.Ho, g.Wo, 3, g.Cpad, 1, g.Ho, g.Wo, t1, bw[2], F(bw[3]), cf, g.Cpad, zero, sf), stats));
            const void* res = x;
            if (g.stride != 1) {
                float* sf2 = stats_for(stats2, HWo, g.C);
                VTGB_TRY(conv_stats(enc_conv(dt, (int)Mo, g.C, g.Ho, g.Wo, 1, Cin_pad, g.stride, Hi, Wi, x, bw[4], F(bw[5]), cf2, g.Cpad, zero, sf2), stats2));
                VTGB_TRY(norm(cf2, Mo, HWo, g.C, g.Cpad, g.Cpad, nullptr, t2, 0, 0, stats2, sf2 != nullptr));
                res = t2;
            }
            outb = t1;
            VTGB_TRY(norm(cf, Mo, HWo, g.C, g.Cpad, g.Cpad, res, outb, 1, 1, stats, sf != nullptr));
        }
        void* all3[3] = {x, t1, t2};
        void* rest[2];
        int k = 0;
        for (int i = 0; i < 3; i++) if (all3[i] != outb) rest[k++] = all3[i];
        x = outb; t1 = rest[0]; t2 = rest[1];
        Cin_pad = g.Cpad; Hi = g.Ho; Wi = g.Wo;
    }
    {
        GemmDesc d;
        memset(&d, 0, sizeof(d));
        d.dtype = dt; d.M = (int)M8; d.N = 256; d.K = 128; d.epi = VTGB_EPI_STORE_F32;
        d.A = x; d.lda = 128; d.W = w[38]; d.ldw = 128; d.bias = F(w[39]); d.out = a->out; d.ldo = 256;
        if (x3) d = enc_conv(dt, (int)M8, 256, H8, W8, 1, 128, 1, H8, W8, x, w[38], F(w[39]), a->out, 256, zero, nullptr);
        VTGB_TRY(launch_conv_gemm(d, s));
    }
    return VTGB_OK;
}

extern "C" size_t vtgb_raft_encoder_workspace_bytes(const vtgb_raft_encoder_args* a) {
    Workspace ws(nullptr, 0);
    if (enc_impl(a, ws, nullptr) != VTGB_OK) return 0;
    return align_up(ws.used, 256);
}
extern "C" int vtgb_raft_encoder(const vtgb_raft_encoder_args* a, vtgb_stream_t stream) {
    VTGB_REQUIRE(a && a->workspace, VTGB_EWORKSPACE, "raft_encoder: workspace is NULL");
    Workspace ws(a->workspace, a->workspace_bytes);
    return enc_impl(a, ws, stream);
}
```

videotgb_amd/csrc/raft_x3.hip:

```cpp
#include <math.h>
#include <string.h>

#include "common.h"
#include "conv_descs.h"
#include "pair_h8.h"

int raft_launch_lookup_pair(const CorrPyr& pyr, const float* flow, void* out_pair, int64_t M, int H8, int W8, int h8, hipStream_t s);
int raft_lkc1_h8_variant();
int raft_lkc1_h8_pack(const void* w, void* packed, int variant, hipStream_t s);
size_t raft_lkc1_h8_pack_bytes();
int raft_launch_lookup_convc1_h8(const CorrPyr& pyr, const float* flow, const void* wpk, const int* scale, const float* bias, void* c1, int64_t M, int H8, int W8,
                                 int variant, int* occupancy, hipStream_t s);
int raft_launch_flow_head2(const float* P2, const float* bias, float* flow, int n_pairs, int H8, int W8, hipStream_t s);
int raft_launch_upsample(const float* flow, const float* mask, float* flow_up, int n_pairs, int H8, int W8, hipStream_t s);

__device__ __forceinline__ void pair_split4(const f32x4 v, bf16x4& hi, bf16x4& lo) {
#pragma unroll
    for (int e = 0; e < 4; e++) {
        const float hf = bf16_round(v[e]);
        hi[e] = (bf16_t)hf;
        lo[e] = (bf16_t)(v[e] - hf);
    }
}
__device__ __forceinline__ f32x4 pair_join4(const bf16x4 hi, const bf16x4 lo) {
    return f32x4{(float)hi[0] + (float)lo[0], (float)hi[1] + (float)lo[1], (float)hi[2] + (float)lo[2], (float)hi[3] + (float)lo[3]};
}
__device__ __forceinline__ float tanh_f(float x) { return 1.0f - 2.0f * __frcp_rn(__expf(2.0f * x) + 1.0f); }

struct PairPass {
    const float* x; int64_t ldx;
    const float* stats; int HW;
    const bf16_t* resid; int64_t ldr; int r_lo;
    bf16_t* out; int64_t ldo; int o_lo;
    int C, Cpad, relu_in, relu_out;
    int64_t M;
    int h8;
    int resid_h8;
};
__global__ __launch_bounds__(256) void x3_pair_pass_kernel(const PairPass p) {
    const int g = p.Cpad >> 2;
    const int64_t i = (int64_t)blockIdx.x * 256 + threadIdx.x;
    if (i >= p.M * g) return;
    const int64_t m = i / g;
    const int c = (int)(i - m * g) * 4;
    f32x4 v = {0.f, 0.f, 0.f, 0.f};
    if (c < p.C) {
        v = *reinterpret_cast<const f32x4*>(p.x + m * p.ldx + c);
        if (p.stats) {
            const int64_t n = m / p.HW;
            const float inv = 1.0f / (float)p.HW;
            const f32x4 s01 = *reinterpret_cast<const f32x4*>(p.stats + (n * p.C + c) * 2), s23 = *reinterpret_cast<const f32x4*>(p.stats + (n * p.C + c) * 2 + 4);
            const float sm[4] = {s01[0], s01[2], s23[0], s23[2]}, sq[4] = {s01[1], s01[3], s23[1], s23[3]};
#pragma unroll
            for (int e = 0; e < 4; e++) {
                const float mean = sm[e] * inv;
                const float rstd = rsqrtf(fmaxf(sq[e] * inv - mean * mean, 0.f) + 1e-5f);
                v[e] = (v[e] - mean) * rstd;
            }
        }
        if (p.relu_in) {
#pragma unroll
            for (int e = 0; e < 4; e++) v[e] = fmaxf(v[e], 0.f);
        }
        if (p.resid) {
            const bf16_t* r = p.resid + m * p.ldr + c;
            if (p.resid_h8) v += h8_join4(*reinterpret_cast<const h8_u32x2*>(r), *reinterpret_cast<const h8_u32x2*>(r + p.r_lo));
            else v += pair_join4(*reinterpret_cast<const bf16x4*>(r), *reinterpret_cast<const bf16x4*>(r + p.r_lo));
        }
        if (p.relu_out) {
#pragma unroll
            for (int e = 0; e < 4; e++) v[e] = fmaxf(v[e], 0.f);
        }
    }
    bf16_t* o = p.out + m * p.ldo + c;
    if (p.h8) {
        h8_u32x2 hu, lu;
        h8_split4(v, hu, lu);
        *reinterpret_cast<h8_u32x2*>(o) = hu;
        *reinterpret_cast<h8_u32x2*>(o + p.o_lo) = lu;
        return;
    }
    bf16x4 hi, lo;
    pair_split4(v, hi, lo);
    *reinterpret_cast<bf16x4*>(o) = hi;
    *reinterpret_cast<bf16x4*>(o + p.o_lo) = lo;
}
int launch_x3_pair_pass(const float* x, int64_t ldx, const float* stats, int HW, const void* resid, int64_t ldr, int r_lo, void* out, int64_t ldo, int o_lo,
                        int C, int Cpad, int relu_in, int relu_out, int64_t M, hipStream_t s, int h8, int resid_h8) {
    VTGB_REQUIRE((C & 3) == 0 && (Cpad & 3) == 0 && (ldx & 3) == 0 && (ldo & 3) == 0 && (o_lo & 3) == 0 && (ldr & 3) == 0 && (r_lo & 3) == 0, VTGB_EINVAL,
                 "pair pass: 4-aligned rows");
    PairPass p{x, ldx, stats, HW, (const bf16_t*)resid, ldr, r_lo, (bf16_t*)out, ldo, o_lo, C, Cpad, relu_in, relu_out, M, h8, resid_h8};
    const int64_t n = M * (Cpad >> 2);
    hipLaunchKernelGGL(x3_pair_pass_kernel, dim3((unsigned)((n + 255) / 256)), dim3(256), 0, s, p);
    VTGB_HIP(hipGetLastError());
    return VTGB_OK;
}

__device__ __forceinline__ void x3_put_flow(bf16_t* __restrict__ X, int64_t m, int i, float f, int h8) {
    if (h8) {
        unsigned short hi; unsigned char lr, lv;
        h8_split1(f, hi, lr, lv);
        reinterpret_cast<unsigned short*>(X)[m * 256 + 126 + i] = hi;
        unsigned char* lo = reinterpret_cast<unsigned char*>(X) + m * 512 + 256 + h8_lo_off(126 + i);
        lo[0] = lr; lo[4] = lv;
    } else {
        const float fh = bf16_round(f);
        X[m * 256 + 126 + i] = (bf16_t)fh;
        X[m * 256 + 254 + i] = (bf16_t)(f - fh);
    }
}

__global__ __launch_bounds__(256) void x3_init_kernel(const float* __restrict__ net, const float* __restrict__ inp, const float* __restrict__ cnet,
                                                      bf16_t* __restrict__ hb, bf16_t* __restrict__ INP, bf16_t* __restrict__ X, float* __restrict__ flow,
                                                      const float* __restrict__ flow_init, int64_t M, int HW, int h8) {
    const int64_t i = (int64_t)blockIdx.x * 256 + threadIdx.x;
    if (i >= M * 32) return;
    const int64_t m = i >> 5;
    const int c = (int)(i & 31) * 4;
    f32x4 hv, iv;
    if (cnet) {
        const f32x4 nv = *reinterpret_cast<const f32x4*>(cnet + m * 256 + c);
        iv = *reinterpret_cast<const f32x4*>(cnet + m * 256 + 128 + c);
#pragma unroll
        for (int e = 0; e < 4; e++) { hv[e] = tanh_f(nv[e]); iv[e] = fmaxf(iv[e], 0.f); }
    } else {
        const int64_t n = m / HW, pp = m - n * HW;
#pragma unroll
        for (int e = 0; e < 4; e++) { hv[e] = net[(n * 128 + c + e) * HW + pp]; iv[e] = inp[(n * 128 + c + e) * HW + pp]; }
    }
    bf16x4 hi, lo;
    if (h8) {
        h8_u32x2 hu, lu;
        h8_split4(hv, hu, lu);
        *reinterpret_cast<h8_u32x2*>(hb + m * 256 + c) = hu;
        *reinterpret_cast<h8_u32x2*>(hb + m * 256 + 128 + c) = lu;
    } else {
        pair_split4(hv, hi, lo);
        *reinterpret_cast<bf16x4*>(hb + m * 256 + c) = hi;
        *reinterpret_cast<bf16x4*>(hb + m * 256 + 128 + c) = lo;
    }
    pair_split4(iv, hi, lo);
    *reinterpret_cast<bf16x4*>(INP + m * 256 + c) = hi;
    *reinterpret_cast<bf16x4*>(INP + m * 256 + 128 + c) = lo;
    if (c == 0) {
        float f0 = 0.f, f1 = 0.f;
        if (flow_init) {
            const int64_t n = m / HW, pp = m - n * HW;
            f0 = flow_init[(n * 2) * HW + pp];
            f1 = flow_init[(n * 2 + 1) * HW + pp];
        }
        flow[m * 2] = f0;
        flow[m * 2 + 1] = f1;
        x3_put_flow(X, m, 0, f0, h8);
        x3_put_flow(X, m, 1, f1, h8);
    }
}

constexpr int CF1_PX = 64, CF1_LDW = 65, CF1_KS = 25;
__global__ __launch_bounds__(256) void x3_convf1_kernel(const float* __restrict__ flow, const float* __restrict__ wt, const float* __restrict__ b,
                                                        bf16_t* __restrict__ f1, bf16_t* __restrict__ X, int64_t M, int H8, int W8, int h8) {
    __shared__ float win[4 * CF1_KS][CF1_LDW];
    const int tid = threadIdx.x, HW = H8 * W8;
    const int lane = tid & 63, wave = __builtin_amdgcn_readfirstlane(tid >> 6);
    const int fr = lane & 15, fg = lane >> 4;
    const int64_t n_tiles = (M + CF1_PX - 1) / CF1_PX;
    float wa[CF1_KS][2];
#pragma unroll
    for (int s_ = 0; s_ < CF1_KS; s_++) {
        const int k = 4 * s_ + fg;
#pragma unroll
        for (int i = 0; i < 2; i++) wa[s_][i] = k < 98 ? wt[k * 128 + wave * 32 + i * 16 + fr] : 0.f;
    }
    f32x4 bias4[2];
#pragma unroll
    for (int i = 0; i < 2; i++) bias4[i] = *reinterpret_cast<const f32x4*>(b + wave * 32 + i * 16 + fg * 4);
    for (int64_t tile = blockIdx.x; tile < n_tiles; tile += gridDim.x) {
    const int64_t m0 = tile * CF1_PX;
    {
        const int px = tid & 63, part = tid >> 6;
        const int64_t m = m0 + px;
        const bool live = m < M;
        const int p0 = __builtin_amdgcn_readfirstlane((int)(m0 % HW));
        int pix = p0 + px;
        pix = pix >= HW ? pix - HW : pix;
        const int y0 = pix / W8, x0 = pix - y0 * W8;
        const auto frs = __builtin_amdgcn_make_buffer_rsrc(const_cast<float*>(flow), 0, (int)(M * 8), 0x00020000);
        typedef unsigned cf1_u32x2 __attribute__((__vector_size__(2 * sizeof(unsigned))));
        cf1_u32x2 v[13];
#pragma unroll
        for (int i = 0; i < 13; i++) {
            const int t = part + 4 * i, tt = t < 49 ? t : 48;
            const int ky = tt / 7, kx = tt - ky * 7, y = y0 + ky - 3, x = x0 + kx - 3;
            const bool ok = live && t < 49 && (unsigned)y < (unsigned)H8 && (unsigned)x < (unsigned)W8;
            const unsigned off = ok ? (unsigned)((int)m + (ky - 3) * W8 + (kx - 3)) * 8u : 0xFFFFFFF0u;
            v[i] = __builtin_amdgcn_raw_buffer_load_b64(frs, off, 0, 0);
        }
#pragma unroll
        for (int i = 0; i < 13; i++) {
            const int t = part + 4 * i;
            if (t < 49) {
                win[t][px] = __uint_as_float(v[i][0]);
                win[49 + t][px] = __uint_as_float(v[i][1]);
            }
        }
        if (tid < 2 * CF1_PX) win[98 + (tid >> 6)][tid & 63] = 0.f;
    }
    f32x4 acc[2][4];
#pragma unroll
    for (int i = 0; i < 2; i++)
#pragma unroll
        for (int j = 0; j < 4; j++) acc[i][j] = bias4[i];
    __syncthreads();
#pragma unroll
    for (int s_ = 0; s_ < CF1_KS; s_++) {
        float xb[4];
#pragma unroll
        for (int j = 0; j < 4; j++) xb[j] = win[4 * s_ + fg][j * 16 + fr];
#pragma unroll
        for (int i = 0; i < 2; i++)
#pragma unroll
            for (int j = 0; j < 4; j++) acc[i][j] = __builtin_amdgcn_mfma_f32_16x16x4f32(wa[s_][i], xb[j], acc[i][j], 0, 0, 0);
    }
#pragma unroll
    for (int j = 0; j < 4; j++) {
        const int64_t m = m0 + j * 16 + fr;
        if (m >= M) continue;
#pragma unroll
        for (int i = 0; i < 2; i++) {
            f32x4 v = acc[i][j];
#pragma unroll
            for (int e = 0; e < 4; e++) v[e] = fmaxf(v[e], 0.f);
            bf16_t* o = f1 + m * 256 + wave * 32 + i * 16 + fg * 4;
            if (h8) {
                h8_u32x2 hu, lu;
                h8_split4(v, hu, lu);
                *reinterpret_cast<h8_u32x2*>(o) = hu;
                *reinterpret_cast<h8_u32x2*>(o + 128) = lu;
            } else {
                bf16x4 hi, lo;
                pair_split4(v, hi, lo);
                *reinterpret_cast<bf16x4*>(o) = hi;
                *reinterpret_cast<bf16x4*>(o + 128) = lo;
            }
        }
    }
    if (tid < 2 * CF1_PX) {
        const int64_t m = m0 + (tid >> 1);
        if (m < M) x3_put_flow(X, m, tid & 1, flow[m * 2 + (tid & 1)], h8);
    }
    __syncthreads();
    }
}

static GemmDesc h8_conv(int M, int N, int H, int W, int KH, int KW, const void* A, int C1, const void* A2, int C2, const void* Wt, const float* bias, int epi,
                        int act, void* out, int64_t ldo, int split_lo, const void* zero, const int* scale, int out_bf16 = 0) {
    GemmDesc d;
    memset(&d, 0, sizeof(d));
    const int Cin = 2 * (C1 + C2);
    d.dtype = VTGB_BF16; d.M = M; d.N = N; d.K = KH * KW * Cin; d.epi = epi; d.act = act;
    d.A = A; d.lda = 2 * C1; d.A2 = A2; d.lda2 = 2 * C2; d.W = Wt; d.ldw = d.K; d.bias = bias; d.out = out; d.ldo = ldo; d.split_lo = split_lo;
    d.conv_H = H; d.conv_W = W; d.conv_KH = KH; d.conv_KW = KW; d.conv_Cin = Cin; d.conv_split = 2 * C1;
    d.zero_page = zero;
    d.h8_run = KH * KW * (C1 / 64); d.h8_scale = scale; d.h8_out_bf16 = out_bf16;
    d.algo_flops = 2.0 * M * (double)N * (KH * KW * (C1 + C2));
    return d;
}

struct GruHalf {
    int M, H8, W8, half, h8;
    const void* h; void* hq; const void* X; void* RH; float* Z;
    const float* start_zr; const float* start_q;
    const void* w_zr; const void* w_q;
    const int* s_zr; const int* s_q;
    const void* zero;
};
static int x3_gru_half(const GruHalf& g, int stage, hipStream_t s) {
    const int kh = g.half == 0 ? 1 : 5, kw = g.half == 0 ? 5 : 1;
    auto conv = [&](int N, const void* A, const void* Wt, const int* scale, int epi, void* out, int64_t ldo) {
        return g.h8 ? h8_conv(g.M, N, g.H8, g.W8, kh, kw, A, 128, g.X, 128, Wt, nullptr, epi, 0, out, ldo, 128, g.zero, scale)
                    : x3_conv(g.M, N, g.H8, g.W8, kh, kw, A, 128, g.X, 128, Wt, nullptr, epi, 0, out, ldo, 128, g.zero);
    };
    auto run = [&](const GemmDesc& d) { return g.h8 ? launch_conv_h8(d, s) : launch_conv_gemm(d, s); };
    if (stage != 1) {
        GemmDesc zr = conv(256, g.h, g.w_zr, g.s_zr, VTGB_EPI_X3ZR, g.Z, 128);
        zr.resid = g.start_zr; zr.ldr = 256; zr.aux = g.h; zr.ldaux = 256; zr.out2 = g.RH; zr.ldo2 = 256;
        zr.algo_flops = 2.0 * g.M * 256.0 * (5 * 384);
        VTGB_TRY(run(zr));
    }
    if (stage != 0) {
        GemmDesc q = conv(128, g.RH, g.w_q, g.s_q, VTGB_EPI_X3Q, g.hq, 256);
        q.resid = g.start_q; q.ldr = 128; q.aux = g.Z; q.ldaux = 128;
        q.algo_flops = 2.0 * g.M * 128.0 * (5 * 384);
        VTGB_TRY(run(q));
    }
    return VTGB_OK;
}

int raft_x3_impl(const vtgb_raft_update_args* a, Workspace& ws, hipStream_t s) {
    VTGB_REQUIRE(a->n_pairs > 0 && a->H8 >= 8 && a->W8 >= 8 && a->iters > 0, VTGB_EINVAL, "raft_update: bad dims n=%d H8=%d W8=%d iters=%d", a->n_pairs, a->H8,
                 a->W8, a->iters);
    const int H8 = a->H8, W8 = a->W8, HW = H8 * W8;
    const int64_t M = (int64_t)a->n_pairs * HW;
    VTGB_REQUIRE(M < (1ll << 28), VTGB_EUNSUPPORTED, "raft_update: too many pixels (the flow field is addressed through one 32-bit buffer range)");
    bf16_t* hb = (bf16_t*)ws.take(M * 256 * 2);
    bf16_t* X = (bf16_t*)ws.take(M * 256 * 2);
    bf16_t* INP = (bf16_t*)ws.take(M * 256 * 2);
    float* ZRI[2] = {(float*)ws.take(M * 256 * 4), (float*)ws.take(M * 256 * 4)};
    float* QI[2] = {(float*)ws.take(M * 128 * 4), (float*)ws.take(M * 128 * 4)};
    const int h8 = a->dtype == VTGB_F16C8;
    bf16_t* corrf = h8 ? nullptr : (bf16_t*)ws.take(M * 768 * 2);
    bf16_t* c1 = (bf16_t*)ws.take(M * 512 * 2);
    bf16_t* CF = (bf16_t*)ws.take(M * 512 * 2);
    bf16_t* f1 = (bf16_t*)ws.take(M * 256 * 2);
    bf16_t* RH = (bf16_t*)ws.take(M * 256 * 2);
    bf16_t* FH = (bf16_t*)ws.take(M * 512 * 2);
    float* ZR = (float*)ws.take(M * 256 * 4);
    float* Q = (float*)ws.take(M * 128 * 4);
    float* flow = (float*)ws.take(M * 2 * 4);
    float* mask = (float*)ws.take(M * 576 * 4);
    float* P2 = mask;
    void* zero = ws.take(256);
    void* w1pk = h8 ? ws.take(raft_lkc1_h8_pack_bytes()) : nullptr;
    if (ws.dry) return VTGB_OK;
    VTGB_REQUIRE(ws.ok(), VTGB_EWORKSPACE, "raft_update: workspace %zu < %zu bytes", ws.size, ws.used);
    VTGB_REQUIRE(((a->net && a->inp) || a->cnet_nhwc) && a->weights && a->flow_up, VTGB_EINVAL, "raft_update: NULL operand");
    VTGB_REQUIRE(!a->corr_f16, VTGB_EINVAL, "raft_update: the bf16x3 / f16c8 modes take an fp32 correlation pyramid");
// ... 229 lines not shown
```

videotgb_amd/ops.py:

```python
from __future__ import annotations

import ctypes as C
import logging
import math
from typing import Dict, List, Optional, Sequence, Tuple

import torch

from . import _lib as L
from ._lib import BF16, BF16X3, F16C8, F32

_log = logging.getLogger("videotgb_amd")
_ws_logged = set()


def _log_workspace(what: str, need: int, detail: str) -> None:
    key = (what, need >> 30)
    if key in _ws_logged:
        return
    _ws_logged.add(key)
    _log.log(logging.WARNING if need > (64 << 30) else logging.INFO, "%s: %.2f GB of workspace (%s)", what, need / 2 ** 30, detail)

Tensor = torch.Tensor

# ... 999 lines not shown
    torch.cuda.current_stream().synchronize()
    return tail_out if tail_w is not None else f32 if out_f32 else out


def raft_lookup_convc1(pyramid: Sequence[Tensor], flow: Tensor, w: Tensor, bias: Tensor, H8: int, W8: int, variant: int = 1,
                       want_occupancy: bool = False):
    _need_cuda(flow, *pyramid)
    M = flow.shape[0]
    assert M % (H8 * W8) == 0 and flow.shape == (M, 2) and w.shape == (256, 324) and len(pyramid) == 4
    lv = [p.contiguous().float() for p in pyramid]
    for l, p in enumerate(lv):
        assert p.numel() == M * (H8 >> l) * (W8 >> l)
    wk = torch.zeros(256, 1, 1, 384, dtype=torch.float32, device=flow.device)
    wk[:, 0, 0, :324] = w.to(flow.device).float()
    sw, byte = h8_weight_scale(wk)
    packed = h8_conv_pack(wk, sw)
    scale = torch.tensor([byte], dtype=torch.int32, device=flow.device)
    fl, bias_t = flow.contiguous().float(), bias.to(flow.device).contiguous().float()
    out = torch.zeros(M, 512, dtype=torch.int16, device=flow.device)
    occ = L.i32(0)
    args = L.RaftLookupConvc1Args(M // (H8 * W8), H8, W8, variant, (L.vp * 4)(*[p.data_ptr() for p in lv]), fl.data_ptr(), packed.data_ptr(), scale.data_ptr(),
                                  bias_t.data_ptr(), out.data_ptr(), C.pointer(occ) if want_occupancy else None)
    L.check(L.lib().vtgb_raft_lookup_convc1(C.byref(args), _stream()))
    torch.cuda.current_stream().synchronize()
    return (out, occ.value) if want_occupancy else out


def raft_gru_half(fmt: int, h: Tensor, x: Tensor, start_zr: Optional[Tensor], start_q: Optional[Tensor], w_zr: Optional[Tensor], w_q: Optional[Tensor],
                  H8: int, W8: int, half: int, stage: int = 2, rh: Optional[Tensor] = None, z: Optional[Tensor] = None, h_q: Optional[Tensor] = None):
    _need_cuda(h, x)
    M, dev = h.shape[0], h.device
    assert M % (H8 * W8) == 0 and h.shape == (M, 256) and x.shape == (M, 256) and h.dtype == torch.int16 and x.dtype == torch.int16
    assert h.is_contiguous() and x.is_contiguous()
    kh, kw = (1, 5) if half == 0 else (5, 1)
    keep = []

    def pack(w, co):
        if w is None:
            return None, None
        assert tuple(w.shape) == (co, kh, kw, 256)
        w = w.to(dev).float()
        if fmt == F16C8:
            sw, byte = h8_weight_scale(w)
            keep.append(torch.tensor([byte], dtype=torch.int32, device=dev))
            keep.append(h8_conv_pack(w, sw, [128, 128]))
            return keep[-1], keep[-2]
        keep.append(_bf16_exact(conv_k_order(split3(w, [128, 128]))))
        return keep[-1], None

    pzr, szr = pack(w_zr, 256)
    pq, sq = pack(w_q, 128)
    rh = torch.zeros(M, 256, dtype=torch.int16, device=dev) if rh is None else rh
    z = torch.zeros(M, 128, dtype=torch.float32, device=dev) if z is None else z
    h_q = h if h_q is None else h_q
    for t, shape, dt in ((rh, (M, 256), torch.int16), (z, (M, 128), torch.float32), (h_q, (M, 256), torch.int16), (start_zr, (M, 256), torch.float32),
                         (start_q, (M, 128), torch.float32)):
        assert t is None or (tuple(t.shape) == shape and t.dtype == dt and t.is_contiguous() and t.device == dev)
    args = L.RaftGruHalfArgs(fmt, M // (H8 * W8), H8, W8, half, stage, h.data_ptr(), h_q.data_ptr(), x.data_ptr(), rh.data_ptr(), z.data_ptr(), _ptr(start_zr),
                             _ptr(start_q), _ptr(pzr), _ptr(pq), _ptr(szr), _ptr(sq))
    L.check(L.lib().vtgb_raft_gru_half(C.byref(args), _stream()))
    torch.cuda.current_stream().synchronize()
    return z, rh, h_q


def conv_launch(code: int, a: Tensor, w: Tensor, n_images: int, H: int, W: int, a2: Optional[Tensor] = None, bias: Optional[Tensor] = None, act: int = 0,
                stride: int = 1, in_hw: Optional[Tuple[int, int]] = None, site: int = L.CONV_SITE_UPDATE, out_kind: int = L.CONV_OUT_F32,
                ld_out: Optional[int] = None, out: Optional[Tensor] = None, moments: bool = False, resid: Optional[Tensor] = None, post_relu: bool = False,
                tail_w: Optional[Tensor] = None, out_scale: float = 0.0):
    _need_cuda(a, a2)
    dev = a.device
    co, kh, kw, ci = w.shape
    width = {BF16X3: 2, BF16: 1, F32: 1}[code]
    adt = {BF16X3: torch.int16, BF16: torch.bfloat16, F32: torch.float32}[code]
    C1 = a.shape[1] // width
    C2 = 0 if a2 is None else a2.shape[1] // width
    Hi, Wi = in_hw or (H, W)
    M = n_images * H * W
    for t in (a, a2):
        assert t is None or (t.dtype == adt and t.is_contiguous() and t.shape[0] == n_images * Hi * Wi)
    assert ci == C1 + C2
    w = w.to(dev).float()
    if code == BF16X3:
        packed = _bf16_exact(conv_k_order(split3(w, [C1, C2] if a2 is not None else None)))
    else:
        packed = conv_k_order(w).to(act_dtype(code)).contiguous()
    bias_t = None if bias is None else bias.to(dev).contiguous().float()
    pair = out_kind in (L.CONV_OUT_PAIR_BF16, L.CONV_OUT_PAIR_F16C8)
    if out is None:
        ld = ld_out or ((co + 7) // 8 * 8)
        odt = torch.int16 if pair else torch.bfloat16 if out_kind == L.CONV_OUT_BF16 else torch.float32
        out = torch.zeros(M, (2 if pair else 1) * ld, dtype=odt, device=dev)
    else:
        assert out.dim() == 2 and out.shape[0] == M and out.stride(1) == 1 and out.shape[1] >= co and not pair
        ld = out.stride(0)
    mom = part = None
    if moments:
        mom = torch.zeros(n_images, co, 2, dtype=torch.float32, device=dev)
        part = torch.zeros((M // 256 + 2) * 128 * 4, dtype=torch.float32, device=dev)
    tail_p = tail_out = None
    if tail_w is not None:
        tail_p = tail_w.to(dev).to(torch.bfloat16).contiguous()
        assert tuple(tail_p.shape) == (32, 256)
        tail_out = torch.zeros(M, 32, dtype=torch.float32, device=dev)
    if resid is not None:
        assert resid.dtype == torch.bfloat16 and resid.dim() == 2 and resid.shape[0] == M and resid.stride(1) == 1
    args = L.ConvLaunchArgs(code, out_kind, site, n_images, H, W, kh, kw, stride, Hi, Wi, C1, C2, co, act, 1 if post_relu else 0, out_scale, a.data_ptr(),
                            _ptr(a2), packed.data_ptr(), _ptr(bias_t), out.data_ptr(), ld, _ptr(mom), _ptr(part), 0 if part is None else part.numel(),
                            _ptr(resid), 0 if resid is None else resid.stride(0), _ptr(tail_p), _ptr(tail_out))
    L.check(L.lib().vtgb_conv_launch(C.byref(args), _stream()))
    torch.cuda.current_stream().synchronize()
    res = tail_out if tail_w is not None else out
    return (res, mom) if moments else res


class RaftWeights(_WeightTable):

    def __init__(self, sd: Dict[str, Tensor], prefix: str = "update_block.", code: int = BF16, hoist_inp: Optional[bool] = None):
        super().__init__(code)
        p = prefix
        if code in (BF16X3, F16C8):
            self._init_x3(sd, p, h8=(code == F16C8))
            return
        self.hoist_inp = (code == BF16) if hoist_inp is None else (hoist_inp and code == BF16)

        def conv(name, cin_pad=None, channels=None):
            w = sd[p + name + ".weight"].float()
            if channels is not None:
                w = w[:, channels]
            co, ci, kh, kw = w.shape
            w = w.permute(0, 2, 3, 1)
            if cin_pad and cin_pad != ci:
                w = torch.nn.functional.pad(w, (0, cin_pad - ci))
            return conv_k_order(w)

        def add_conv(name, cin_pad=None):
            self.add(conv(name, cin_pad), True)
            self.add(sd[p + name + ".bias"])

        add_conv("encoder.convc1", 384)
        add_conv("encoder.convc2")
        if code == BF16:
            wf = sd[p + "encoder.convf1.weight"].float().reshape(128, 2, 49).permute(0, 2, 1)
            wf = torch.nn.functional.pad(torch.cat([wf, wf], 2), (0, 0, 0, 7))
            self.add(wf.reshape(128, 224).contiguous(), True)
        else:
            self.add(sd[p + "encoder.convf1.weight"].float().reshape(128, 98).t().contiguous(), True)
        self.add(sd[p + "encoder.convf1.bias"])
        add_conv("encoder.convf2")
        add_conv("encoder.conv")
        dyn = (list(range(0, 128)) + list(range(256, 384))) if self.hoist_inp else None
        for sfx in ("1", "2"):
            self.add(torch.cat([conv("gru.convz" + sfx, channels=dyn), conv("gru.convr" + sfx, channels=dyn)], 0), True)
            self.add(torch.cat([sd[p + "gru.convz" + sfx + ".bias"], sd[p + "gru.convr" + sfx + ".bias"]], 0))
            self.add(conv("gru.convq" + sfx, channels=dyn), True)
            self.add(sd[p + "gru.convq" + sfx + ".bias"])
        add_conv("flow_head.conv1")
        w2 = sd[p + "flow_head.conv2.weight"].float().permute(2, 3, 0, 1).reshape(18, 256)
        self.add(torch.nn.functional.pad(w2, (0, 0, 0, 14)).contiguous(), True)
        self.add(sd[p + "flow_head.conv2.bias"])
        add_conv("mask.0")
        add_conv("mask.2")
        inp = list(range(128, 256))
        for sfx in ("1", "2"):
            if self.hoist_inp:
                self.add(torch.cat([conv("gru.convz" + sfx, channels=inp), conv("gru.convr" + sfx, channels=inp)], 0), True)
                self.add(conv("gru.convq" + sfx, channels=inp), True)
            else:
                self.add(None); self.add(None)
        self.finish()

    def _init_x3(self, sd: Dict[str, Tensor], p: str, h8: bool = False) -> None:
        self.hoist_inp = True
        scales = []

        def raw(name, cin_pad=None, scale=1.0, channels=None):
            w = sd[p + name + ".weight"].float() * scale
            if channels is not None:
                w = w[:, channels]
            co, ci, kh, kw = w.shape
            w = w.permute(0, 2, 3, 1)
            if cin_pad and cin_pad != ci:
                w = torch.nn.functional.pad(w, (0, cin_pad - ci))
            return w

        def conv(name, cin_pad=None, sources=None, scale=1.0, channels=None):
            return _bf16_exact(conv_k_order(split3(raw(name, cin_pad, scale, channels), sources)))

        def big(ws, sources=None):
            if not h8:
                return torch.cat([_bf16_exact(conv_k_order(split3(w, sources))) for w in ws], 0).contiguous()
            sw, byte = h8_weight_scale(torch.cat([w.reshape(-1) for w in ws]))
            scales.append(byte)
            return torch.cat([h8_conv_pack(w, sw, sources) for w in ws], 0).contiguous()

        def add_big(name, cin_pad=None):
            self.tensors.append(big([raw(name, cin_pad)]))
            self.add(sd[p + name + ".bias"].float())

        def add_conv(name, cin_pad=None, scale=1.0):
            self.tensors.append(conv(name, cin_pad, scale=scale))
            self.add(sd[p + name + ".bias"].float() * scale)

        add_big("encoder.convc1", 384)
        add_big("encoder.convc2")
        self.add(sd[p + "encoder.convf1.weight"].float().reshape(128, 98).t().contiguous())
        self.add(sd[p + "encoder.convf1.bias"])
        late_scales = []
        if h8:
            wf2 = raw("encoder.convf2")
            sw, byte = h8_weight_scale(wf2)
            late_scales.append(byte)
            self.tensors.append(h8_conv_pack(wf2, sw))
            self.add(sd[p + "encoder.convf2.bias"].float())
        else:
            add_conv("encoder.convf2")
        add_big("encoder.conv")
        dyn = list(range(0, 128)) + list(range(256, 384))
        for sfx in ("1", "2"):
            self.tensors.append(big([raw("gru.convz" + sfx, channels=dyn), raw("gru.convr" + sfx, channels=dyn)], sources=[128, 128]))
            self.add(torch.cat([sd[p + "gru.convz" + sfx + ".bias"], sd[p + "gru.convr" + sfx + ".bias"]], 0))
            self.tensors.append(big([raw("gru.convq" + sfx, channels=dyn)], sources=[128, 128]))
            self.add(sd[p + "gru.convq" + sfx + ".bias"])
        add_big("flow_head.conv1")
        w2 = sd[p + "flow_head.conv2.weight"].float().permute(2, 3, 0, 1).reshape(18, 256)
        w2 = torch.nn.functional.pad(w2, (0, 0, 0, 14)).reshape(32, 1, 1, 256)
        if h8:
            self.add(flow_tail_pack(w2.reshape(32, 256)))
        else:
            self.tensors.append(_bf16_exact(conv_k_order(split3(w2))))
        self.add(sd[p + "flow_head.conv2.bias"])
        add_big("mask.0")
        add_conv("mask.2", scale=0.25)
        inp = list(range(128, 256))
        for sfx in ("1", "2"):
            self.tensors.append(torch.cat([conv("gru.convz" + sfx, channels=inp), conv("gru.convr" + sfx, channels=inp)], 0).contiguous())
            self.tensors.append(conv("gru.convq" + sfx, channels=inp))
        if h8:
            assert len(scales) == 9
            self.tensors.append(torch.tensor(scales + late_scales, dtype=torch.int32, device=self.tensors[0].device))
        self.finish()


def raft_update(w: RaftWeights, net: Optional[Tensor], inp: Optional[Tensor], pyramid: Sequence[Tensor], iters: int = 20,
                cnet_nhwc: Optional[Tensor] = None, hw: Optional[Tuple[int, int]] = None, flow_init: Optional[Tensor] = None) -> Tensor:
    if cnet_nhwc is not None:
        _need_cuda(cnet_nhwc, *pyramid)
        cnet_nhwc = cnet_nhwc.contiguous().float()
        n, (H8, W8) = cnet_nhwc.shape[0], hw
    else:
        _need_cuda(net, inp, *pyramid)
        net, inp = net.contiguous().float(), inp.contiguous().float()
        n, _, H8, W8 = net.shape
    if len(pyramid) != 4:
        raise ValueError("raft_update: the correlation pyramid has 4 levels")
    half = all(t.dtype == torch.float16 for t in pyramid)
    lv = [t.contiguous() if half else t.contiguous().float() for t in pyramid]
    dev = lv[0].device
    if flow_init is not None:
        flow_init = flow_init.contiguous().float()
    out = torch.empty(n, 2, 8 * H8, 8 * W8, dtype=torch.float32, device=dev)
    a = L.RaftUpdateArgs(w.code, n, H8, W8, iters, None if net is None else net.data_ptr(), None if inp is None else inp.data_ptr(),
                         (C.c_void_p * 4)(*[t.data_ptr() for t in lv]), C.cast(w.array, C.POINTER(C.c_void_p)), out.data_ptr(), None, 0,
                         1 if half else 0, None if cnet_nhwc is None else cnet_nhwc.data_ptr(), _ptr(flow_init))
    need = L.lib().vtgb_raft_update_workspace_bytes(C.byref(a))
    _log_workspace("raft_update", need, f"{n} frame pairs of {H8} x {W8} coarse pixels, dtype code {w.code}; lower flow_clips_per_call to shrink it")
    ws = _ws.get(need, dev)
    a.workspace, a.workspace_bytes = ws.data_ptr(), ws.numel()
    L.check(L.lib().vtgb_raft_update(C.byref(a), _stream()))
    return out


def raft_corr(fmap: Tensor, n_pairs: int, H8: int, W8: int, pairs_per_clip: int, frames_per_clip: int, first_off: int, second_off: int,
              code: int = BF16) -> List[Tensor]:
    _need_cuda(fmap)
    fmap = fmap.contiguous().float()
    n_images = fmap.numel() // (H8 * W8 * 256)
    odt = torch.float16 if code == BF16 else torch.float32
    lv, h, w = [], H8, W8
    for _ in range(4):
        lv.append(torch.empty(n_pairs * H8 * W8, 1, h, w, dtype=odt, device=fmap.device))
        h, w = h // 2, w // 2
    done = 0
    while done < n_pairs:
        per = n_pairs - done
        if per > 65535:
            per = max(65535 // pairs_per_clip, 1) * pairs_per_clip
            if per > 65535:
                raise NotImplementedError("raft_corr: more than 65535 pairs per clip")
        img0 = (done // pairs_per_clip) * frames_per_clip
        fm = fmap.view(n_images, -1)[img0:]
        lvs = [t[done * H8 * W8:] for t in lv]
        a = L.RaftCorrArgs(code, per, H8, W8, 256, pairs_per_clip, frames_per_clip, first_off, second_off, n_images - img0, 1.0 / 16.0,
                           fm.data_ptr(), (C.c_void_p * 4)(*[t.data_ptr() for t in lvs]), None, 0)
        need = L.lib().vtgb_raft_corr_workspace_bytes(C.byref(a))
        if need == 0:
            L.check(L.lib().vtgb_raft_corr(C.byref(a), _stream()))
        ws = _ws.get(need, fmap.device)
        a.workspace, a.workspace_bytes = ws.data_ptr(), ws.numel()
        L.check(L.lib().vtgb_raft_corr(C.byref(a), _stream()))
        done += per
    return lv


class RaftEncoderWeights(_WeightTable):

    def __init__(self, sd: Dict[str, Tensor], prefix: str, batch_norm: bool, code: int = BF16):
        super().__init__(code)
        self.batch_norm = batch_norm
        p = prefix

        def folded(conv, bn):
            w, b = sd[p + conv + ".weight"].float(), sd[p + conv + ".bias"].float()
            if batch_norm:
                g = sd[p + bn + ".weight"].float() / torch.sqrt(sd[p + bn + ".running_var"].float() + 1e-5)
                w = w * g.view(-1, 1, 1, 1)
                b = (b - sd[p + bn + ".running_mean"].float()) * g + sd[p + bn + ".bias"].float()
            return w, b

        x3 = code in (BF16X3, F16C8)
        h8_scales = [0] * 12

        def packed(w, cin_pad, cout_pad=None, h8=None):
            co, ci, kh, kw = w.shape
            w = w.permute(0, 2, 3, 1)
            if cin_pad != ci:
                w = torch.nn.functional.pad(w, (0, cin_pad - ci))
            if h8 is not None:
                if batch_norm and cout_pad and cout_pad != co:
                    w = torch.nn.functional.pad(w, (0, 0, 0, 0, 0, 0, 0, cout_pad - co))
                sw, byte = h8_weight_scale(w)
                h8_scales[h8] = byte
                return h8_conv_pack(w, sw)
            w = conv_k_order(split3(w) if x3 else w)
            if batch_norm and cout_pad and cout_pad != co:
                w = torch.nn.functional.pad(w, (0, 0, 0, cout_pad - co))
            return w

        def pbias(b, cout_pad):
            return torch.nn.functional.pad(b, (0, cout_pad - b.numel())) if batch_norm and cout_pad != b.numel() else b

        w, b = folded("conv1", "norm1")
        if code != F32:
            w = w * (2.0 / 255.0)
        wp = torch.zeros(64, 4, 4, 2, 2, 3, dtype=torch.float32, device=w.device)
        for tY in range(4):
            for py in range(2):
                ky = 2 * tY + py - 1
                if ky < 0:
                    continue
                for dX in range(4):
                    for px in range(2):
                        kx = 2 * dX + px - 1
                        if kx >= 0:
                            wp[:, tY, dX, py, px, :] = w[:, :, ky, kx]
        wp = torch.nn.functional.pad(wp.reshape(64, 4, 48), (0, 16))
        if code == BF16:
            wp = torch.stack([wp, wp], 1)
        if x3:
            wp = conv_k_order(split3(wp.reshape(64, 4, 1, 64)))
        self.add(wp.reshape(64, -1).contiguous(), True); self.add(b)
        cin_pad = 64
        for l, (li, c, cpad) in enumerate((("layer1", 64, 64), ("layer2", 96, 128), ("layer3", 128, 128))):
            for bi in range(2):
                bp = f"{li}.{bi}."
                blk = 2 * l + bi
                w1, b1 = folded(bp + "conv1", bp + "norm1")
                w2, b2 = folded(bp + "conv2", bp + "norm2")
                if code == F16C8 and (l == 0 or bi == 1):
                    self.tensors.append(packed(w1, cin_pad, cpad, 2 * blk)); self.add(pbias(b1, cpad))
                else:
                    self.add(packed(w1, cin_pad, cpad), True); self.add(pbias(b1, cpad))
                if code == F16C8:
                    self.tensors.append(packed(w2, cpad, cpad, 2 * blk + 1)); self.add(pbias(b2, cpad))
                else:
                    self.add(packed(w2, cpad, cpad), True); self.add(pbias(b2, cpad))
                if (p + bp + "downsample.0.weight") in sd:
                    wd, bd = folded(bp + "downsample.0", bp + "norm3")
                    self.add(packed(wd, cin_pad, cpad), True); self.add(pbias(bd, cpad))
                else:
                    self.add(None); self.add(None)
                cin_pad = cpad
        wh = sd[p + "conv2.weight"].float().reshape(256, 128)
        self.add(conv_k_order(split3(wh.reshape(256, 1, 1, 128))) if x3 else wh.contiguous(), True)
        self.add(sd[p + "conv2.bias"])
        if code == F16C8:
            assert len(self.tensors) == 40
            self.tensors.append(torch.tensor(h8_scales, dtype=torch.int32, device=self.tensors[0].device))
        self.finish()


def raft_encoder(w: RaftEncoderWeights, images: Tensor, max_images: int = 384) -> Tensor:
    _need_cuda(images)
    images = images.contiguous().float()
    n, _, H, W = images.shape
    out = torch.empty(n, (H // 8) * (W // 8), 256, dtype=torch.float32, device=images.device)
    if w.code == F32:
        max_images = max(max_images // 2, 1)
    for i0 in range(0, n, max_images):
        chunk = images[i0:i0 + max_images]
        a = L.RaftEncoderArgs(w.code, chunk.shape[0], H, W, 1 if w.batch_norm else 0, chunk.data_ptr(), C.cast(w.array, C.POINTER(C.c_void_p)),
                              out[i0:i0 + max_images].data_ptr(), None, 0)
        need = L.lib().vtgb_raft_encoder_workspace_bytes(C.byref(a))
        _log_workspace("raft_encoder", need, f"{chunk.shape[0]} frames of {H} x {W} per chunk, dtype code {w.code}; max_images sets the chunk")
        ws = _ws.get(need, images.device)
        a.workspace, a.workspace_bytes = ws.data_ptr(), ws.numel()
        L.check(L.lib().vtgb_raft_encoder(C.byref(a), _stream()))
    return out
```

Measured before the change: 35.60 clips/s.

## Fuse split-precision RAFT stem conv with pair-format output and bias epilogue

Extends the 7x7 stem MFMA kernel with a split-precision (x3) variant that consumes three-term bf16 weights and writes hi/lo pair rows (bf16 or h8) directly. For the x3 encoder this replaces the separate stem conv, stats and normalisation passes with one fused kernel. It also adds a standalone raft_stem entry point with a workspace query and moves the stem weight packing into a shared helper. The x3 path issues 1.5x more MFMA work per pixel in exchange for fewer launches and less memory traffic.

```diff
diff --git a/include/vtgb.h b/include/vtgb.h
--- a/include/vtgb.h
+++ b/include/vtgb.h
@@ -366,6 +366,21 @@
     float* tail_out;
 } vtgb_conv_launch_args;
 int vtgb_conv_launch(const vtgb_conv_launch_args* a, vtgb_stream_t stream);
+
+typedef struct {
+    int32_t n_images, H, W;
+    int32_t variant;
+    int32_t out_kind;
+    const float* images;
+    const void* weights;
+    const float* bias;
+    void* out;
+    float* moments;
+    void* workspace;
+    size_t workspace_bytes;
+} vtgb_raft_stem_args;
+size_t vtgb_raft_stem_workspace_bytes(const vtgb_raft_stem_args* a);
+int vtgb_raft_stem(const vtgb_raft_stem_args* a, vtgb_stream_t stream);
 
 typedef struct {
     int32_t dtype, n_pairs, H8, W8, dim;
diff --git a/videotgb_amd/_lib.py b/videotgb_amd/_lib.py
--- a/videotgb_amd/_lib.py
+++ b/videotgb_amd/_lib.py
@@ -44,6 +44,7 @@
     "vtgb_raft_lookup_convc1", "vtgb_raft_gru_half", "vtgb_llm_lora", "vtgb_conv_launch", "vtgb_attention_cached",
     "vtgb_llm_decode_attention_beam", "vtgb_llm_beam_candidates", "vtgb_llm_attention_rows_beam", "vtgb_llm_decode_attention_beam_fp8",
     "vtgb_pack_skinny_weight_mxfp4_bytes", "vtgb_pack_skinny_weight_mxfp4", "vtgb_gemm_skinny_mxfp4",
+    "vtgb_raft_stem_workspace_bytes", "vtgb_raft_stem",
 ]
 COMM_ID_BYTES = 128
 
@@ -167,6 +168,11 @@
                 ("Hi", i32), ("Wi", i32), ("C1", i32), ("C2", i32), ("N", i32), ("act", i32), ("post_relu", i32), ("out_scale", f32), ("a", vp), ("a2", vp),
                 ("weights", vp), ("bias", vp), ("out", vp), ("ld_out", i64), ("moments", vp), ("stats_part", vp), ("stats_part_floats", i64), ("resid", vp),
                 ("ld_resid", i64), ("tail_w", vp), ("tail_out", vp)]
+
+
+class RaftStemArgs(C.Structure):
+    _fields_ = [("n_images", i32), ("H", i32), ("W", i32), ("variant", i32), ("out_kind", i32), ("images", vp), ("weights", vp), ("bias", vp), ("out", vp),
+                ("moments", vp), ("workspace", vp), ("workspace_bytes", sz)]
 
 
 class RaftCorrArgs(C.Structure):
@@ -300,6 +306,10 @@
     L.vtgb_raft_gru_half.restype = C.c_int
     L.vtgb_conv_launch.argtypes = [C.POINTER(ConvLaunchArgs), vp]
     L.vtgb_conv_launch.restype = C.c_int
+    L.vtgb_raft_stem.argtypes = [C.POINTER(RaftStemArgs), vp]
+    L.vtgb_raft_stem.restype = C.c_int
+    L.vtgb_raft_stem_workspace_bytes.argtypes = [C.POINTER(RaftStemArgs)]
+    L.vtgb_raft_stem_workspace_bytes.restype = sz
     L.vtgb_raft_update.argtypes = [C.POINTER(RaftUpdateArgs), vp]
     L.vtgb_raft_update.restype = C.c_int
     L.vtgb_raft_update_workspace_bytes.argtypes = [C.POINTER(RaftUpdateArgs)]
diff --git a/videotgb_amd/csrc/common.h b/videotgb_amd/csrc/common.h
--- a/videotgb_amd/csrc/common.h
+++ b/videotgb_amd/csrc/common.h
@@ -172,6 +172,8 @@
 bool stem7x7_supported(int H, int W);
 int launch_stem7x7(const float* img, const void* w, const float* bias, float* out_f32, float* stats, float* stats_part, void* out_bf16, int n_img, int H, int W,
                    int relu, hipStream_t s);
+int launch_stem7x7_x3(const float* img, const void* w, const float* bias, float* out_f32, float* stats, float* stats_part, void* out_pair, int h8, int n_img, int H,
+                      int W, hipStream_t s);
 size_t conv64_stats_part_floats(int n_img);
 int launch_stats_finish_tiles(const float* part, float* stats, int n_img, int HW, int N, int64_t M, hipStream_t s);
 int launch_stats_finish_parts(const float* part, float* stats, int n_img, int parts, int C, hipStream_t s);
diff --git a/videotgb_amd/csrc/conv64.hip b/videotgb_amd/csrc/conv64.hip
--- a/videotgb_amd/csrc/conv64.hip
+++ b/videotgb_amd/csrc/conv64.hip
@@ -1,4 +1,5 @@
 #include "common.h"
+#include "pair_h8.h"
 
 namespace {
 
@@ -215,10 +216,12 @@
     bf16_t* out_bf16;
     int n_img, H, W, relu;
     int parts, rows_per_part;
+    int h8;
 };
 
-template <int MODE>
+template <int MODE, bool X3>
 __global__ __launch_bounds__(512) void stem7x7_kernel(const StemParams p) {
+    static_assert(X3 ? (MODE == 0 || MODE == 2) : (MODE == 0 || MODE == 1), "stem7x7: bf16 stores fp32 / bf16 rows, the split form fp32 / pair rows");
 #if defined(__HIP_DEVICE_COMPILE__)
     extern __shared__ __attribute__((aligned(16))) char ring[];
     const int tid = threadIdx.x, lane = tid & 63, fr = lane & 15, fg = lane >> 4;
@@ -233,11 +236,13 @@
         const int pxl = i >> 2, X = pxl % W2, c = 6 + (i & 1) + ((i & 2) << 2);
         *reinterpret_cast<uint4*>(ring + pxl * 256 + ((c ^ (X & 15)) << 4)) = make_uint4(0, 0, 0, 0);
     }
+    constexpr int W_LD = X3 ? 768 : 512;
     bf16x8 wf[16][2];
 #pragma unroll
     for (int s_ = 0; s_ < 16; s_++)
 #pragma unroll
-        for (int i = 0; i < 2; i++) wf[s_][i] = *reinterpret_cast<const bf16x8*>(p.w + (wn * 32 + i * 16 + fr) * 512 + s_ * 32 + fg * 8);
+        for (int i = 0; i < 2; i++)
+            wf[s_][i] = *reinterpret_cast<const bf16x8*>(p.w + (wn * 32 + i * 16 + fr) * W_LD + (X3 ? (s_ >> 3) * 512 + (s_ & 7) * 32 : s_ * 32) + fg * 8);
     const bool builder = tid < W2 * 4;
     const int bX = tid >> 2, bdX = tid & 3, bcol = 2 * (bX + bdX - 2);
     const bool bcol_ok = builder && bcol >= 0 && bcol + 1 < W;
@@ -260,11 +265,12 @@
     typedef __attribute__((__vector_size__(2 * sizeof(unsigned)))) unsigned u32x2_t;
     constexpr unsigned OOB = 0x80000000u;
     constexpr int ES = MODE == 0 ? 4 : 2;
+    constexpr int PXU = MODE == 2 ? 128 : 64;
     unsigned o_off[2][2];
 #pragma unroll
     for (int i = 0; i < 2; i++)
 #pragma unroll
-        for (int j = 0; j < 2; j++) o_off[i][j] = px[j] < W2 ? (unsigned)(px[j] * 64 + wn * 32 + i * 16 + fg * 4) * ES : OOB;
+        for (int j = 0; j < 2; j++) o_off[i][j] = px[j] < W2 ? (unsigned)(px[j] * PXU + wn * 32 + i * 16 + fg * 4) * ES : OOB;
 
     const int n_units = p.n_img * p.parts;
     for (int unit = blockIdx.x; unit < n_units; unit += gridDim.x) {
@@ -272,8 +278,8 @@
         if (y0 >= H2) continue;
         const int y1 = y0 + p.rows_per_part < H2 ? y0 + p.rows_per_part : H2;
         const float* const ibase = p.img + (int64_t)img * 3 * H * W;
-        const auto orsrc = __builtin_amdgcn_make_buffer_rsrc(MODE == 0 ? (void*)(p.out_f32 + (int64_t)img * H2 * W2 * 64) : (void*)(p.out_bf16 + (int64_t)img * H2 * W2 * 64),
-                                                             0, H2 * W2 * 64 * ES, 0x00020000);
+        const auto orsrc = __builtin_amdgcn_make_buffer_rsrc(MODE == 0 ? (void*)(p.out_f32 + (int64_t)img * H2 * W2 * 64) : (void*)(p.out_bf16 + (int64_t)img * H2 * W2 * PXU),
+                                                             0, H2 * W2 * PXU * ES, 0x00020000);
         float2 ld[6];
 #define ST_LOAD(Yp)       \
         {                                                                                                    \
@@ -311,44 +317,72 @@
             __builtin_amdgcn_s_barrier();
             __builtin_amdgcn_sched_barrier(0);
             ST_LOAD(y + 2)
-            f32x4 acc[2][2];
-#pragma unroll
-            for (int i = 0; i < 2; i++)
-#pragma unroll
-                for (int j = 0; j < 2; j++) acc[i][j] = f32x4{0.f, 0.f, 0.f, 0.f};
-#pragma unroll
-            for (int tY = 0; tY < 4; tY++) {
-                const char* const rowp = ring + ((y + tY - 2 + ST_R) % ST_R) * row_bytes;
-#pragma unroll
-                for (int hl = 0; hl < 2; hl++)
-#pragma unroll
-                    for (int half = 0; half < 2; half++) {
-                        const int s_ = hl * 8 + tY * 2 + half;
-                        const unsigned cx = (unsigned)((hl * 8 + half * 4) << 4);
-                        const bf16x8 x0 = *reinterpret_cast<const bf16x8*>(rowp + (x_off[0] ^ cx));
-                        const bf16x8 x1 = *reinterpret_cast<const bf16x8*>(rowp + (x_off[1] ^ cx));
-#pragma unroll
-                        for (int i = 0; i < 2; i++) {
-                            acc[i][0] = __builtin_amdgcn_mfma_f32_16x16x32_bf16(wf[s_][i], x0, acc[i][0], 0, 0, 0);
-                            acc[i][1] = __builtin_amdgcn_mfma_f32_16x16x32_bf16(wf[s_][i], x1, acc[i][1], 0, 0, 0);
-                        }
-                    }
-            }
-            f32x4 b4[2];
-#pragma unroll
-            for (int i = 0; i < 2; i++) b4[i] = *reinterpret_cast<const f32x4*>(bias_s + wn * 32 + i * 16 + fg * 4);
+            f32x4 acc[2][2], b4[2];
+#define ST_STEP(tY, hl, half, s_)                                                                            \
+            {                                                                                                \
+                const char* const rowp = ring + ((y + (tY) - 2 + ST_R) % ST_R) * row_bytes;                  \
+                const unsigned cx = (unsigned)(((hl) * 8 + (half) * 4) << 4);       \
+                const bf16x8 x0 = *reinterpret_cast<const bf16x8*>(rowp + (x_off[0] ^ cx));                  \
+                const bf16x8 x1 = *reinterpret_cast<const bf16x8*>(rowp + (x_off[1] ^ cx));                  \
+                _Pragma("unroll") for (int i = 0; i < 2; i++) {                                              \
+                    acc[i][0] = __builtin_amdgcn_mfma_f32_16x16x32_bf16(wf[s_][i], x0, acc[i][0], 0, 0, 0);  \
+                    acc[i][1] = __builtin_amdgcn_mfma_f32_16x16x32_bf16(wf[s_][i], x1, acc[i][1], 0, 0, 0);  \
+                }                                                                                            \
+            }
+            if constexpr (X3) {
+#pragma unroll
+                for (int i = 0; i < 2; i++) b4[i] = *reinterpret_cast<const f32x4*>(bias_s + wn * 32 + i * 16 + fg * 4);
+#pragma unroll
+                for (int i = 0; i < 2; i++)
+#pragma unroll
+                    for (int j = 0; j < 2; j++) acc[i][j] = b4[i] + f32x4{0.f, 0.f, 0.f, 0.f};
+#pragma unroll
+                for (int c = 0; c < 3; c++) {
+#pragma unroll
+                    for (int tY = 0; tY < 4; tY++)
+#pragma unroll
+                        for (int half = 0; half < 2; half++) ST_STEP(tY, c == 1 ? 1 : 0, half, (c == 2 ? 8 : 0) + tY * 2 + half)
+                    if (c < 2) __builtin_amdgcn_sched_barrier(0);
+                }
+            } else {
+#pragma unroll
+                for (int i = 0; i < 2; i++)
+#pragma unroll
+                    for (int j = 0; j < 2; j++) acc[i][j] = f32x4{0.f, 0.f, 0.f, 0.f};
+#pragma unroll
+                for (int tY = 0; tY < 4; tY++)
+#pragma unroll
+                    for (int hl = 0; hl < 2; hl++)
+#pragma unroll
+                        for (int half = 0; half < 2; half++) ST_STEP(tY, hl, half, hl * 8 + tY * 2 + half)
+#pragma unroll
+                for (int i = 0; i < 2; i++) b4[i] = *reinterpret_cast<const f32x4*>(bias_s + wn * 32 + i * 16 + fg * 4);
+            }
+#undef ST_STEP
 #pragma unroll
             for (int i = 0; i < 2; i++)
 #pragma unroll
                 for (int j = 0; j < 2; j++) {
                     const bool ok = o_off[i][j] != OOB;
-                    const unsigned off = ok ? o_off[i][j] + (unsigned)(y * W2 * 64 * ES) : OOB;
-                    f32x4 v = acc[i][j] + b4[i];
+                    const unsigned off = ok ? o_off[i][j] + (unsigned)(y * W2 * PXU * ES) : OOB;
+                    f32x4 v = X3 ? acc[i][j] : acc[i][j] + b4[i];
                     if constexpr (MODE == 0) {
                         __builtin_amdgcn_raw_buffer_store_b128(__builtin_bit_cast(u32x4_t, v), orsrc, off, 0, 0);
                         const f32x4 vz = {ok ? v[0] : 0.f, ok ? v[1] : 0.f, ok ? v[2] : 0.f, ok ? v[3] : 0.f};
                         s1[i] += vz;
                         s2[i] += vz * vz;
+                    } else if constexpr (MODE == 2) {
+                        if (p.relu) v = f32x4{fmaxf(v[0], 0.f), fmaxf(v[1], 0.f), fmaxf(v[2], 0.f), fmaxf(v[3], 0.f)};
+                        u32x2_t hu, lu;
+                        if (p.h8) {
+                            h8_split4(v, hu, lu);
+                        } else {
+                            bf16x4 hi, lo;
+                            pair_split4(v, hi, lo);
+                            hu = __builtin_bit_cast(u32x2_t, hi); lu = __builtin_bit_cast(u32x2_t, lo);
+                        }
+                        __builtin_amdgcn_raw_buffer_store_b64(hu, orsrc, off, 0, 0);
+                        __builtin_amdgcn_raw_buffer_store_b64(lu, orsrc, ok ? off + 128u : OOB, 0, 0);
                     } else {
                         if (p.relu) v = f32x4{fmaxf(v[0], 0.f), fmaxf(v[1], 0.f), fmaxf(v[2], 0.f), fmaxf(v[3], 0.f)};
                         const bf16x4 pk = {(bf16_t)v[0], (bf16_t)v[1], (bf16_t)v[2], (bf16_t)v[3]};
@@ -359,6 +393,9 @@
         }
 #undef ST_LOAD
 #undef ST_WRITE
+        if constexpr (X3) {
+            if (!p.stats) continue;
+        }
         if constexpr (MODE == 0) {
 #pragma unroll
             for (int i = 0; i < 2; i++)
@@ -431,33 +468,54 @@
 
 bool stem7x7_supported(int H, int W) { return (H % 2) == 0 && (W % 2) == 0 && W / 2 >= 16 && W / 2 <= 112 && H / 2 >= 4; }
 
-int launch_stem7x7(const float* img, const void* w, const float* bias, float* out_f32, float* stats, float* stats_part, void* out_bf16, int n_img, int H, int W,
-                   int relu, hipStream_t s) {
+static int stem7x7_launch(bool x3, const float* img, const void* w, const float* bias, float* out_f32, float* stats, float* stats_part, void* out16, int h8, int n_img,
+                          int H, int W, int relu, hipStream_t s) {
     VTGB_REQUIRE(stem7x7_supported(H, W), VTGB_EUNSUPPORTED, "stem7x7: %d x %d unsupported", H, W);
     const int H2 = H / 2, W2 = W / 2;
+    VTGB_REQUIRE((int64_t)H2 * W2 * 256 < 0x7FFFFF00ll, VTGB_EUNSUPPORTED, "stem7x7: image too large");
     StemParams p;
-    p.img = img; p.w = (const bf16_t*)w; p.bias = bias; p.out_f32 = out_f32; p.stats = stats; p.stats_part = stats_part; p.out_bf16 = (bf16_t*)out_bf16;
-    p.n_img = n_img; p.H = H; p.W = W; p.relu = relu;
+    p.img = img; p.w = (const bf16_t*)w; p.bias = bias; p.out_f32 = out_f32; p.stats = stats; p.stats_part = stats_part; p.out_bf16 = (bf16_t*)out16;
+    p.n_img = n_img; p.H = H; p.W = W; p.relu = relu; p.h8 = h8;
     int parts = 1;
     while ((int64_t)n_img * parts < 4 * cu_count() && H2 / (parts * 2) >= 14) parts *= 2;
     p.rows_per_part = (H2 + parts - 1) / parts;
     p.parts = (H2 + p.rows_per_part - 1) / p.rows_per_part;
     const int64_t units = (int64_t)n_img * p.parts;
     const int grid = units < cu_count() ? (int)units : cu_count();
-    if (out_f32 && p.parts > 1) VTGB_REQUIRE(stats_part && (size_t)units * 128 <= conv64_stats_part_floats(n_img), VTGB_EINVAL, "stem7x7: partial-moment scratch missing");
+    if (out_f32 && stats && p.parts > 1)
+        VTGB_REQUIRE(stats_part && (size_t)units * 128 <= conv64_stats_part_floats(n_img), VTGB_EINVAL, "stem7x7: partial-moment scratch missing");
     const int lds = ST_R * W2 * 256 + 8 * 32 * 2 * 4 + 64 * 4;
-    const double flops = 2.0 * n_img * H2 * W2 * 64.0 * 147.0, exec = 2.0 * n_img * H2 * W2 * 64.0 * 512.0;
+    constexpr int lds_max = ST_R * 112 * 256 + 8 * 32 * 2 * 4 + 64 * 4;
+    const double flops = 2.0 * n_img * H2 * W2 * 64.0 * 147.0, exec = 2.0 * n_img * H2 * W2 * 64.0 * (x3 ? 768.0 : 512.0);
     ProfScope prof(VTGB_PROF_CONV, flops, s, exec);
-    static DeviceOnce a0, a1;
+    static DeviceOnce a0, a1, a2, a3;
     if (out_f32) {
-        VTGB_REQUIRE(stats, VTGB_EINVAL, "stem7x7: fp32 output needs the moments buffer");
-        VTGB_FUNC_LDS_ONCE(a0, stem7x7_kernel<0>, ST_R * 112 * 256 + 8 * 32 * 2 * 4 + 64 * 4);
-        hipLaunchKernelGGL(stem7x7_kernel<0>, dim3(grid), dim3(512), lds, s, p);
-        if (p.parts > 1) VTGB_TRY(launch_stats_finish_parts(stats_part, stats, n_img, p.parts, 64, s));
+        VTGB_REQUIRE(stats || x3, VTGB_EINVAL, "stem7x7: fp32 output needs the moments buffer");
+        if (x3) {
+            VTGB_FUNC_LDS_ONCE(a2, (stem7x7_kernel<0, true>), lds_max);
+            hipLaunchKernelGGL((stem7x7_kernel<0, true>), dim3(grid), dim3(512), lds, s, p);
+        } else {
+            VTGB_FUNC_LDS_ONCE(a0, (stem7x7_kernel<0, false>), lds_max);
+            hipLaunchKernelGGL((stem7x7_kernel<0, false>), dim3(grid), dim3(512), lds, s, p);
+        }
+        if (stats && p.parts > 1) VTGB_TRY(launch_stats_finish_parts(stats_part, stats, n_img, p.parts, 64, s));
+    } else if (x3) {
+        VTGB_FUNC_LDS_ONCE(a3, (stem7x7_kernel<2, true>), lds_max);
+        hipLaunchKernelGGL((stem7x7_kernel<2, true>), dim3(grid), dim3(512), lds, s, p);
     } else {
-        VTGB_FUNC_LDS_ONCE(a1, stem7x7_kernel<1>, ST_R * 112 * 256 + 8 * 32 * 2 * 4 + 64 * 4);
-        hipLaunchKernelGGL(stem7x7_kernel<1>, dim3(grid), dim3(512), lds, s, p);
+        VTGB_FUNC_LDS_ONCE(a1, (stem7x7_kernel<1, false>), lds_max);
+        hipLaunchKernelGGL((stem7x7_kernel<1, false>), dim3(grid), dim3(512), lds, s, p);
     }
     VTGB_HIP(hipGetLastError());
     return VTGB_OK;
 }
+
+int launch_stem7x7(const float* img, const void* w, const float* bias, float* out_f32, float* stats, float* stats_part, void* out_bf16, int n_img, int H, int W,
+                   int relu, hipStream_t s) {
+    return stem7x7_launch(false, img, w, bias, out_f32, stats, stats_part, out_bf16, 0, n_img, H, W, relu, s);
+}
+int launch_stem7x7_x3(const float* img, const void* w, const float* bias, float* out_f32, float* stats, float* stats_part, void* out_pair, int h8, int n_img, int H,
+                      int W, hipStream_t s) {
+    VTGB_REQUIRE((out_f32 != nullptr) != (out_pair != nullptr), VTGB_EINVAL, "stem7x7 x3: exactly one of the fp32 rows and the pair rows");
+    return stem7x7_launch(true, img, w, bias, out_f32, stats, stats_part, out_pair, h8, n_img, H, W, out_pair ? 1 : 0, s);
+}
diff --git a/videotgb_amd/csrc/pair_h8.h b/videotgb_amd/csrc/pair_h8.h
--- a/videotgb_amd/csrc/pair_h8.h
+++ b/videotgb_amd/csrc/pair_h8.h
@@ -7,6 +7,14 @@
 constexpr float H8_MAX = 57344.0f;
 
 #if defined(__HIPCC__)
+__device__ __forceinline__ void pair_split4(const f32x4 v, bf16x4& hi, bf16x4& lo) {
+#pragma unroll
+    for (int e = 0; e < 4; e++) {
+        const float hf = bf16_round(v[e]);
+        hi[e] = (bf16_t)hf;
+        lo[e] = (bf16_t)(v[e] - hf);
+    }
+}
 __device__ __forceinline__ void h8_split4(f32x4 v, h8_u32x2& hi, h8_u32x2& lo) {
 #pragma unroll
     for (int e = 0; e < 4; e++) v[e] = __builtin_amdgcn_fmed3f(v[e], -H8_MAX, H8_MAX);
diff --git a/videotgb_amd/csrc/raft_enc.hip b/videotgb_amd/csrc/raft_enc.hip
--- a/videotgb_amd/csrc/raft_enc.hip
+++ b/videotgb_amd/csrc/raft_enc.hip
@@ -120,6 +120,48 @@
     hipLaunchKernelGGL(stats_finish_tiles_kernel, dim3((unsigned)((total + 255) / 256)), dim3(256), 0, s, part, stats, n_img, HW, N, M);
     VTGB_HIP(hipGetLastError());
     return VTGB_OK;
+}
+
+__global__ __launch_bounds__(512) void stats_tiles_c64_kernel(const float* __restrict__ x, float* __restrict__ part, int M, int stats_rows) {
+    __shared__ f32x4 pr[8][64];
+    const int tid = threadIdx.x, lane = tid & 63, wm = tid >> 6, rl = lane >> 4, cl = lane & 15;
+    const int mt = blockIdx.x, m0 = mt * 256;
+    const int img_a = m0 / stats_rows, m_b = (img_a + 1) * stats_rows;
+    f32x4 sa = {0.f, 0.f, 0.f, 0.f}, qa = sa, sb = sa, qb = sa;
+    f32x4 vv[8];
+#pragma unroll
+    for (int rr = 0; rr < 8; rr++) {
+        const int m = m0 + wm * 32 + rr * 4 + rl;
+        vv[rr] = m < M ? *reinterpret_cast<const f32x4*>(x + (int64_t)m * 64 + cl * 4) : f32x4{0.f, 0.f, 0.f, 0.f};
+    }
+#pragma unroll
+    for (int rr = 0; rr < 8; rr++) {
+        const f32x4 v = vv[rr];
+        const int m = m0 + wm * 32 + rr * 4 + rl;
+        if (m < M) {
+            if (m < m_b) { sa += v; qa += v * v; }
+            else { sb += v; qb += v * v; }
+        }
+    }
+#pragma unroll
+    for (int e = 0; e < 4; e++) {
+        sa[e] += __shfl_xor(sa[e], 16); sa[e] += __shfl_xor(sa[e], 32);
+        qa[e] += __shfl_xor(qa[e], 16); qa[e] += __shfl_xor(qa[e], 32);
+        sb[e] += __shfl_xor(sb[e], 16); sb[e] += __shfl_xor(sb[e], 32);
+        qb[e] += __shfl_xor(qb[e], 16); qb[e] += __shfl_xor(qb[e], 32);
+    }
+    if (rl == 0) { pr[wm][cl] = sa; pr[wm][16 + cl] = qa; pr[wm][32 + cl] = sb; pr[wm][48 + cl] = qb; }
+    __syncthreads();
+    if (tid < 64) {
+        float t[4] = {0.f, 0.f, 0.f, 0.f};
+        for (int wm_ = 0; wm_ < 8; wm_++) {
+            if (m0 + wm_ * 32 >= M) break;
+            const float* w_ = reinterpret_cast<const float*>(pr[wm_]);
+#pragma unroll
+            for (int e = 0; e < 4; e++) t[e] += w_[e * 64 + tid];
+        }
+        *reinterpret_cast<float4*>(part + ((int64_t)mt * 64 + tid) * 4) = make_float4(t[0], t[1], t[2], t[3]);
+    }
 }
 
 constexpr int NA_PASS = 4;
@@ -182,6 +224,36 @@
 
 int launch_x3_pair_pass(const float* x, int64_t ldx, const float* stats, int HW, const void* resid, int64_t ldr, int r_lo, void* out, int64_t ldo, int o_lo,
                         int C, int Cpad, int relu_in, int relu_out, int64_t M, hipStream_t s, int h8 = 0, int resid_h8 = 0);
+
+struct StemX3 {
+    const float* images; const void* w; const float* bias;
+    int n, H, W;
+    float* cf; float* stats; float* spart;
+    void* pair; int h8;
+    void* packed; void* pad_page;
+};
+static int enc_stem_x3(const StemX3& t, int variant, hipStream_t s) {
+    const int H2 = t.H / 2, W2 = t.W / 2, HW = H2 * W2;
+    const int64_t M2 = (int64_t)t.n * HW;
+    if (variant == 1) return launch_stem7x7_x3(t.images, t.w, t.bias, t.pair ? nullptr : t.cf, t.stats, t.spart, t.pair, t.h8, t.n, t.H, t.W, s);
+    if (variant == 2) {
+        VTGB_REQUIRE(!t.pair && HW >= 256, VTGB_EINVAL, "raft_stem: tile-order moments belong to fp32 rows of images of >= 256 pixels");
+        VTGB_TRY(launch_stem7x7_x3(t.images, t.w, t.bias, t.cf, nullptr, nullptr, nullptr, 0, t.n, t.H, t.W, s));
+        hipLaunchKernelGGL(stats_tiles_c64_kernel, dim3((unsigned)((M2 + 255) / 256)), dim3(512), 0, s, t.cf, t.spart, (int)M2, HW);
+        return launch_stats_finish_tiles(t.spart, t.stats, t.n, HW, 64, M2, s);
+    }
+    hipLaunchKernelGGL(raft_stem_pack_kernel<bf16_t>, dim3((unsigned)((M2 * 4 + 255) / 256)), dim3(256), 0, s, t.images, (bf16_t*)t.packed, (bf16_t*)t.pad_page, M2, t.H,
+                       t.W);
+    float* sf = (!t.pair && HW >= 256) ? t.spart : nullptr;
+    GemmDesc d = enc_stem_conv(VTGB_BF16X3, (int)M2, 64, H2, W2, 64, t.packed, t.w, t.bias, t.cf, 64, t.pad_page, sf);
+    d.algo_flops = 2.0 * (double)M2 * 64 * 147;
+    VTGB_TRY(launch_conv_gemm(d, s));
+    if (t.pair) return launch_x3_pair_pass(t.cf, 64, nullptr, HW, nullptr, 128, 64, t.pair, 128, 64, 64, 64, 1, 0, M2, s, t.h8);
+    if (sf) return launch_stats_finish_tiles(sf, t.stats, t.n, HW, 64, M2, s);
+    const int splits = HW >= 4096 ? 16 : HW >= 1024 ? 4 : 1;
+    hipLaunchKernelGGL(inorm_stats_kernel, dim3(t.n, splits), dim3(256), 0, s, t.cf, t.spart, HW, 64, 64);
+    return launch_stats_finish_parts(t.spart, t.stats, t.n, splits, 64, s);
+}
 
 static int enc_impl(const vtgb_raft_encoder_args* a, Workspace& ws, hipStream_t s) {
     VTGB_REQUIRE(a, VTGB_EINVAL, "raft_encoder: NULL args");
@@ -260,6 +332,10 @@
         } else {
             VTGB_TRY(launch_stem7x7(a->images, w[0], F(w[1]), nullptr, nullptr, nullptr, act0, n, a->H, a->W, 1, s));
         }
+    } else if (x3) {
+        const StemX3 t{a->images, w[0], F(w[1]), n, a->H, a->W, cf, stats, spart, inorm ? nullptr : act0, h8l1, act1, pad_page};
+        VTGB_TRY(enc_stem_x3(t, stem_on && stem7x7_supported(a->H, a->W) ? (inorm ? 2 : 1) : 0, s));
+        if (inorm) VTGB_TRY(norm(cf, M2, H2 * W2, 64, 64, 64, nullptr, act0, 1, 0, stats, true, h8l1));
     } else {
         if (dt != VTGB_F32)
             hipLaunchKernelGGL(raft_stem_pack_kernel<bf16_t>, dim3((unsigned)((M2 * 4 + 255) / 256)), dim3(256), 0, s, a->images, (bf16_t*)act1, (bf16_t*)pad_page, M2,
@@ -271,10 +347,9 @@
             float* sf = stats_for(stats, H2 * W2, 64);
             const int cp = dt == VTGB_BF16 ? 128 : 64;
             GemmDesc d = enc_stem_conv(dt, (int)M2, 64, H2, W2, cp, act1, w[0], F(w[1]), cf, 64, pad_page, sf);
-            if (x3) d.algo_flops = 2.0 * (double)M2 * 64 * 147;
-            if (!inorm && !x3) { d.epi = VTGB_EPI_STORE; d.act = 1; d.out = act0; }
+            if (!inorm) { d.epi = VTGB_EPI_STORE; d.act = 1; d.out = act0; }
             VTGB_TRY(conv_stats(d, stats));
-            if (inorm || x3) VTGB_TRY(norm(cf, M2, H2 * W2, 64, 64, 64, nullptr, act0, 1, 0, stats, sf != nullptr, h8l1));
+            if (inorm) VTGB_TRY(norm(cf, M2, H2 * W2, 64, 64, 64, nullptr, act0, 1, 0, stats, sf != nullptr));
         }
     }
     struct Stage { int C, Cpad, stride, Ho, Wo; };
@@ -436,6 +511,51 @@
     return VTGB_OK;
 }
 
+static int stem_unit_impl(const vtgb_raft_stem_args* a, Workspace& ws, hipStream_t s) {
+    VTGB_REQUIRE(a, VTGB_EINVAL, "raft_stem: NULL args");
+    VTGB_REQUIRE(a->n_images > 0 && a->H >= 2 && a->W >= 2 && (a->H % 2) == 0 && (a->W % 2) == 0 && a->variant >= 0 && a->variant <= 2, VTGB_EINVAL,
+                 "raft_stem: bad dims n=%d H=%d W=%d variant=%d", a->n_images, a->H, a->W, a->variant);
+    const int ok = a->out_kind;
+    VTGB_REQUIRE(ok == VTGB_CONV_OUT_F32 || ok == VTGB_CONV_OUT_PAIR_BF16 || ok == VTGB_CONV_OUT_PAIR_F16C8, VTGB_EINVAL,
+                 "raft_stem: bad out_kind %d (VTGB_CONV_OUT_F32, _PAIR_BF16 or _PAIR_F16C8)", ok);
+    VTGB_REQUIRE(a->variant == 0 || stem7x7_supported(a->H, a->W), VTGB_EUNSUPPORTED, "raft_stem: the fused stem does not take %d x %d frames (variant 0 does)", a->H, a->W);
+    const bool pair = ok != VTGB_CONV_OUT_F32;
+    VTGB_REQUIRE(a->variant != 2 || (!pair && (a->H / 2) * (a->W / 2) >= 256), VTGB_EINVAL,
+                 "raft_stem: variant 2 (tile-order moments) belongs to fp32 rows of images of >= 256 half-resolution pixels");
+    const int n = a->n_images;
+    const int64_t M2 = (int64_t)n * (a->H / 2) * (a->W / 2);
+    VTGB_REQUIRE(M2 < (1ll << 31), VTGB_EUNSUPPORTED, "raft_stem: too many pixels per call (chunk the images)");
+    void* packed = a->variant == 0 ? ws.take(M2 * 128 * 2) : nullptr;
+    float* cf = a->variant == 0 && pair ? (float*)ws.take(M2 * 64 * 4) : nullptr;
+    size_t part_floats = (size_t)(M2 / 256 + 2) * 128 * 4;
+    if (conv64_stats_part_floats(n) > part_floats) part_floats = conv64_stats_part_floats(n);
+    if ((size_t)n * 16 * 128 * 2 > part_floats) part_floats = (size_t)n * 16 * 128 * 2;
+    float* spart = pair ? nullptr : (float*)ws.take(part_floats * 4);
+    void* pad_page = ws.take(256);
+    if (ws.dry) return VTGB_OK;
+    VTGB_REQUIRE(ws.ok(), VTGB_EWORKSPACE, "raft_stem: workspace %zu < %zu bytes", ws.size, ws.used);
+    VTGB_REQUIRE(a->images && a->weights && a->bias && a->out && (pair || a->moments), VTGB_EINVAL, "raft_stem: NULL operand (moments belong to the fp32 rows)");
+    auto al16 = [](const void* p) { return ((uintptr_t)p & 15) == 0; };
+    VTGB_REQUIRE(al16(a->images) && al16(a->weights) && al16(a->bias) && al16(a->out) && (pair || al16(a->moments)) && al16(a->workspace), VTGB_EINVAL,
+                 "raft_stem: misaligned operand (16 bytes)");
+    const StemX3 t{a->images, a->weights, a->bias, n, a->H, a->W, pair ? cf : (float*)a->out, a->moments, spart, pair ? a->out : nullptr,
+                   ok == VTGB_CONV_OUT_PAIR_F16C8, packed, pad_page};
+    return enc_stem_x3(t, a->variant, s);
+}
+extern "C" size_t vtgb_raft_stem_workspace_bytes(const vtgb_raft_stem_args* a) {
+    Workspace ws(nullptr, 0);
+    if (stem_unit_impl(a, ws, nullptr) != VTGB_OK) return 0;
+    return align_up(ws.used, 256);
+}
+extern "C" int vtgb_raft_stem(const vtgb_raft_stem_args* a, vtgb_stream_t stream) {
+    VTGB_REQUIRE(a, VTGB_EINVAL, "raft_stem: NULL args");
+    Workspace probe(nullptr, 0);
+    VTGB_TRY(stem_unit_impl(a, probe, nullptr));
+    VTGB_REQUIRE(a->workspace, VTGB_EWORKSPACE, "raft_stem: workspace is NULL (%zu bytes needed)", align_up(probe.used, 256));
+    Workspace ws(a->workspace, a->workspace_bytes);
+    return stem_unit_impl(a, ws, (hipStream_t)stream);
+}
+
 extern "C" size_t vtgb_raft_encoder_workspace_bytes(const vtgb_raft_encoder_args* a) {
     Workspace ws(nullptr, 0);
     if (enc_impl(a, ws, nullptr) != VTGB_OK) return 0;
diff --git a/videotgb_amd/csrc/raft_x3.hip b/videotgb_amd/csrc/raft_x3.hip
--- a/videotgb_amd/csrc/raft_x3.hip
+++ b/videotgb_amd/csrc/raft_x3.hip
@@ -14,14 +14,6 @@
 int raft_launch_flow_head2(const float* P2, const float* bias, float* flow, int n_pairs, int H8, int W8, hipStream_t s);
 int raft_launch_upsample(const float* flow, const float* mask, float* flow_up, int n_pairs, int H8, int W8, hipStream_t s);
 
-__device__ __forceinline__ void pair_split4(const f32x4 v, bf16x4& hi, bf16x4& lo) {
-#pragma unroll
-    for (int e = 0; e < 4; e++) {
-        const float hf = bf16_round(v[e]);
-        hi[e] = (bf16_t)hf;
-        lo[e] = (bf16_t)(v[e] - hf);
-    }
-}
 __device__ __forceinline__ f32x4 pair_join4(const bf16x4 hi, const bf16x4 lo) {
     return f32x4{(float)hi[0] + (float)lo[0], (float)hi[1] + (float)lo[1], (float)hi[2] + (float)lo[2], (float)hi[3] + (float)lo[3]};
 }
diff --git a/videotgb_amd/ops.py b/videotgb_amd/ops.py
--- a/videotgb_amd/ops.py
+++ b/videotgb_amd/ops.py
@@ -1325,6 +1325,55 @@
     return lv
 
 
+def raft_stem_pack(w: Tensor, code: int) -> Tensor:
+    w = w.float()
+    if code != F32:
+        w = w * (2.0 / 255.0)
+    wp = torch.zeros(64, 4, 4, 2, 2, 3, dtype=torch.float32, device=w.device)
+    for tY in range(4):
+        for py in range(2):
+            ky = 2 * tY + py - 1
+            if ky < 0:
+                continue
+            for dX in range(4):
+                for px in range(2):
+                    kx = 2 * dX + px - 1
+                    if kx >= 0:
+                        wp[:, tY, dX, py, px, :] = w[:, :, ky, kx]
+    wp = torch.nn.functional.pad(wp.reshape(64, 4, 48), (0, 16))
+    if code == BF16:
+        wp = torch.stack([wp, wp], 1)
+    if code in (BF16X3, F16C8):
+        wp = conv_k_order(split3(wp.reshape(64, 4, 1, 64)))
+    return wp.reshape(64, -1).contiguous()
+
+
+def raft_stem(images: Tensor, w: Tensor, bias: Tensor, variant: int = 1, out_kind: int = L.CONV_OUT_F32, out: Optional[Tensor] = None,
+              workspace: Optional[Tensor] = None):
+    _need_cuda(images)
+    dev = images.device
+    images = images.contiguous().float()
+    n, _, H, W = images.shape
+    M2 = n * (H // 2) * (W // 2)
+    pair = out_kind != L.CONV_OUT_F32
+    packed = _bf16_exact(raft_stem_pack(w.to(dev), BF16X3))
+    bias_t = bias.to(dev).contiguous().float()
+    if out is None:
+        out = torch.empty(M2, 128, dtype=torch.int16, device=dev) if pair else torch.empty(M2, 64, dtype=torch.float32, device=dev)
+    assert out.is_contiguous() and out.numel() >= M2 * (128 if pair else 64) and out.dtype == (torch.int16 if pair else torch.float32)
+    moments = None if pair else torch.empty(n, 64, 2, dtype=torch.float32, device=dev)
+    a = L.RaftStemArgs(n, H, W, variant, out_kind, images.data_ptr(), packed.data_ptr(), bias_t.data_ptr(), out.data_ptr(), _ptr(moments), None, 0)
+    need = L.lib().vtgb_raft_stem_workspace_bytes(C.byref(a))
+    if need == 0:
+        L.check(L.lib().vtgb_raft_stem(C.byref(a), _stream()))
+    ws = workspace if workspace is not None else _ws.get(need, dev)
+    assert ws.numel() >= need
+    a.workspace, a.workspace_bytes = ws.data_ptr(), ws.numel()
+    L.check(L.lib().vtgb_raft_stem(C.byref(a), _stream()))
+    torch.cuda.current_stream().synchronize()
+    return out if pair else (out, moments)
+
+
 class RaftEncoderWeights(_WeightTable):
 
     def __init__(self, sd: Dict[str, Tensor], prefix: str, batch_norm: bool, code: int = BF16):
@@ -1363,25 +1412,7 @@
             return torch.nn.functional.pad(b, (0, cout_pad - b.numel())) if batch_norm and cout_pad != b.numel() else b
 
         w, b = folded("conv1", "norm1")
-        if code != F32:
-            w = w * (2.0 / 255.0)
-        wp = torch.zeros(64, 4, 4, 2, 2, 3, dtype=torch.float32, device=w.device)
-        for tY in range(4):
-            for py in range(2):
-                ky = 2 * tY + py - 1
-                if ky < 0:
-                    continue
-                for dX in range(4):
-                    for px in range(2):
-                        kx = 2 * dX + px - 1
-                        if kx >= 0:
-                            wp[:, tY, dX, py, px, :] = w[:, :, ky, kx]
-        wp = torch.nn.functional.pad(wp.reshape(64, 4, 48), (0, 16))
-        if code == BF16:
-            wp = torch.stack([wp, wp], 1)
-        if x3:
-            wp = conv_k_order(split3(wp.reshape(64, 4, 1, 64)))
-        self.add(wp.reshape(64, -1).contiguous(), True); self.add(b)
+        self.add(raft_stem_pack(w, code), True); self.add(b)
         cin_pad = 64
         for l, (li, c, cpad) in enumerate((("layer1", 64, 64), ("layer2", 96, 128), ("layer3", 128, 128))):
             for bi in range(2):
```

Measured after the change: 36.15 clips/s, median of 6. 1.02x the previous value.
